# biod/sambamba

Measured on NVIDIA H100. Metric: bam_gb_per_s_depth_base, higher is better.
Workload: dtype u32

## Files before the change

include/bdepth.h:

```cpp
#ifndef BDEPTH_H
#define BDEPTH_H

#include <stddef.h>
#include <stdint.h>

#ifdef __cplusplus
extern "C" {
#endif

typedef struct bdepth bdepth_t;

typedef enum {
    BDEPTH_OK = 0,
    BDEPTH_ERR_IO = -1,
    BDEPTH_ERR_FORMAT = -2,
    BDEPTH_ERR_UNSORTED = -3,
    BDEPTH_ERR_NOINDEX = -4,
    BDEPTH_ERR_CUDA = -5,
    BDEPTH_ERR_NCCL = -6,
    BDEPTH_ERR_ARG = -7,
    BDEPTH_ERR_CALLBACK = -8
} bdepth_status;

typedef struct { uint32_t ref_id, start, end; } bdepth_region;

typedef struct {
    int32_t  ref_id;
    uint32_t start;
    uint32_t len;
    uint32_t stride;
    const uint32_t* counts;
    uint32_t n_samples;
    uint32_t sample_stride;
} bdepth_tile;
enum { BDEPTH_PLANE_A = 0, BDEPTH_PLANE_C, BDEPTH_PLANE_G, BDEPTH_PLANE_T, BDEPTH_PLANE_N, BDEPTH_PLANE_DEL, BDEPTH_PLANE_REFSKIP, BDEPTH_N_PLANES };

typedef int (*bdepth_tile_cb)(void* user, const bdepth_tile* tile);

typedef struct {
    int32_t  ref_id;
    uint32_t start, end;
    uint32_t n_reads;
    uint32_t n_bases;
    const uint32_t* cov_ge;
    int32_t  sample_id;
} bdepth_region_stat;
typedef int (*bdepth_stat_cb)(void* user, const bdepth_region_stat* stat, uint64_t index);

typedef struct {
    uint64_t file_bytes;
    uint64_t n_blocks;
    uint64_t cdata_bytes;
    uint64_t inflated_bytes;
    uint64_t n_records;
    uint64_t n_records_pass;
    uint64_t n_cigar_ops;
    uint64_t seq_bytes;
    uint64_t positions;
    uint64_t covered_positions;
    uint64_t long_reads;
    uint64_t chain_fixups;
    uint32_t gpu_launches;
    uint32_t n_batches;
    float ms_h2d, ms_inflate, ms_scan, ms_coverage, ms_reduce, ms_d2h, ms_total_device;
    double host_wall_ms;
    float ms_span_device;
    float ms_exchange;
    uint64_t own_lo, own_hi;
    uint64_t halo_bytes_sent;
    uint64_t mate_pairs;
    uint64_t mate_pair_columns;
    uint64_t mate_groups;
    float ms_mates;
} bdepth_stats;

int  bdepth_device_count(void);
int  bdepth_open(const char* bam_path, int device, bdepth_t** out);
int  bdepth_open_lazy(const char* bam_path, int device, bdepth_t** out);
int  bdepth_open_memory(const void* bam, size_t bam_len, const void* bai, size_t bai_len, int device, bdepth_t** out);
int  bdepth_add_input(bdepth_t* h, const char* bam_path);
void bdepth_close(bdepth_t* h);
const char* bdepth_last_error(const bdepth_t* h);

int         bdepth_n_ref(const bdepth_t* h);
const char* bdepth_ref_name(const bdepth_t* h, int i);
uint32_t    bdepth_ref_length(const bdepth_t* h, int i);
const char* bdepth_header_text(const bdepth_t* h, size_t* len);
int         bdepth_is_coordinate_sorted(const bdepth_t* h);
int         bdepth_has_index(const bdepth_t* h);
int         bdepth_n_samples(const bdepth_t* h);
const char* bdepth_sample_name(const bdepth_t* h, int i);

int bdepth_set_filter(bdepth_t* h, int mapq_gt, uint32_t flag_reject_mask);
int bdepth_set_filter_query(bdepth_t* h, const char* query);
int bdepth_set_min_baseq(bdepth_t* h, uint32_t min_base_quality);
int bdepth_set_fix_mates(bdepth_t* h, int on);
int bdepth_set_combined(bdepth_t* h, int combined);
int bdepth_set_regions(bdepth_t* h, const bdepth_region* regions, size_t n);
int bdepth_set_shard(bdepth_t* h, int rank, int world, const void* nccl_unique_id);
int bdepth_nccl_unique_id(void* out128);
int bdepth_plan_shards(const char* bam_path, int world, uint64_t* out_voffsets);
long bdepth_plan_region_chunks(const char* bam_path, const bdepth_region* regions, size_t n, uint64_t* out_pairs, size_t cap);
int bdepth_set_tuning(bdepth_t* h, uint64_t batch_inflated_bytes, uint64_t chunk_blocks);

int bdepth_stage(bdepth_t* h);
int bdepth_run_resident(bdepth_t* h);
int bdepth_run_base(bdepth_t* h, bdepth_tile_cb cb, void* user);
int bdepth_run_windows(bdepth_t* h, uint32_t window, uint32_t overlap, const uint32_t* thresholds, size_t n_thresholds, bdepth_stat_cb cb, void* user);
int bdepth_run_regions(bdepth_t* h, const bdepth_region* regions, size_t n, const uint32_t* thresholds, size_t n_thresholds, bdepth_stat_cb cb, void* user);

typedef struct { double min_cov, max_cov; int annotate; } bdepth_text_opts;
typedef int (*bdepth_text_cb)(void* user, const char* text, size_t len);
int bdepth_run_base_text(bdepth_t* h, const bdepth_text_opts* opts, bdepth_text_cb cb, void* user);

int bdepth_get_stats(const bdepth_t* h, bdepth_stats* out);
int bdepth_ref_has_reads(const bdepth_t* h, int ref);

int64_t bdepth_inflate_to_host(bdepth_t* h, void* dst, uint64_t cap);
int64_t bdepth_build_index(bdepth_t* h, void* dst, uint64_t cap);
typedef struct { uint64_t total[2], secondary[2], supplementary[2], duplicates[2], mapped[2], paired[2], read1[2], read2[2],
                 proper_pair[2], both_mapped[2], singletons[2], mate_diff_chr[2], mate_diff_chr_mapq5[2]; } bdepth_flagstat;
int bdepth_run_flagstat(bdepth_t* h, bdepth_flagstat* out);
enum { BDEPTH_VIEW_ALL = 0, BDEPTH_VIEW_BED = 1, BDEPTH_VIEW_POSITIONAL = 2 };
typedef struct {
    uint16_t flag_set, flag_unset;
    const char* query;
    int subsample;
    uint64_t subsample_threshold;
    uint64_t subsampling_seed;
    int regions_from;
    const bdepth_region* regions;
    size_t n_regions;
    uint32_t n_unmapped;
} bdepth_view_opts;
int bdepth_run_view_count(bdepth_t* h, const bdepth_view_opts* opts, uint64_t* count);
#define BDEPTH_VIEW_UNMAPPED 0xFFFFFFFFu
int bdepth_run_view_text(bdepth_t* h, const bdepth_view_opts* opts, bdepth_text_cb cb, void* user);
int64_t bdepth_scan_to_host(bdepth_t* h, uint64_t cap, int32_t* ref_id, int32_t* pos, uint32_t* span, uint16_t* flag, uint8_t* mapq, uint16_t* n_cigar, uint64_t* rec_off);

#ifdef __cplusplus
}
#endif
#endif
```

sambamba_b200/_lib.py:

```python
import ctypes as C
import os
import numpy as np

_HERE = os.path.dirname(os.path.abspath(__file__))


def lib_path():
    return os.path.join(_HERE, "_build", "libbdepth.so")


class BDepthError(RuntimeError):
    def __init__(self, code, msg):
        super().__init__(f"bdepth error {code}: {msg}")
        self.code = code
        self.msg = msg


class Region(C.Structure):
    _fields_ = [("ref_id", C.c_uint32), ("start", C.c_uint32), ("end", C.c_uint32)]


class Tile(C.Structure):
    _fields_ = [("ref_id", C.c_int32), ("start", C.c_uint32), ("len", C.c_uint32), ("stride", C.c_uint32),
                ("counts", C.POINTER(C.c_uint32)), ("n_samples", C.c_uint32), ("sample_stride", C.c_uint32)]


class RegionStat(C.Structure):
    _fields_ = [("ref_id", C.c_int32), ("start", C.c_uint32), ("end", C.c_uint32), ("n_reads", C.c_uint32),
                ("n_bases", C.c_uint32), ("cov_ge", C.POINTER(C.c_uint32)), ("sample_id", C.c_int32)]


class Stats(C.Structure):
    _fields_ = [(n, C.c_uint64) for n in ("file_bytes", "n_blocks", "cdata_bytes", "inflated_bytes", "n_records",
                                          "n_records_pass", "n_cigar_ops", "seq_bytes", "positions",
                                          "covered_positions", "long_reads", "chain_fixups")] + \
               [("gpu_launches", C.c_uint32), ("n_batches", C.c_uint32)] + \
               [(n, C.c_float) for n in ("ms_h2d", "ms_inflate", "ms_scan", "ms_coverage", "ms_reduce", "ms_d2h",
                                         "ms_total_device")] + [("host_wall_ms", C.c_double), ("ms_span_device", C.c_float), ("ms_exchange", C.c_float),
                                                                 ("own_lo", C.c_uint64), ("own_hi", C.c_uint64), ("halo_bytes_sent", C.c_uint64),
                                                                 ("mate_pairs", C.c_uint64), ("mate_pair_columns", C.c_uint64), ("mate_groups", C.c_uint64), ("ms_mates", C.c_float)]

    def as_dict(self):
        return {n: getattr(self, n) for n, _ in self._fields_}


FLAGSTAT_FIELDS = ("total", "secondary", "supplementary", "duplicates", "mapped", "paired", "read1", "read2", "proper_pair", "both_mapped",
                   "singletons", "mate_diff_chr", "mate_diff_chr_mapq5")


class FlagStat(C.Structure):
    _fields_ = [(n, C.c_uint64 * 2) for n in FLAGSTAT_FIELDS]

    def as_dict(self):
        return {n: (getattr(self, n)[0], getattr(self, n)[1]) for n in FLAGSTAT_FIELDS}


class ViewOpts(C.Structure):
    _fields_ = [("flag_set", C.c_uint16), ("flag_unset", C.c_uint16), ("query", C.c_char_p), ("subsample", C.c_int), ("subsample_threshold", C.c_uint64),
                ("subsampling_seed", C.c_uint64), ("regions_from", C.c_int), ("regions", C.POINTER(Region)), ("n_regions", C.c_size_t), ("n_unmapped", C.c_uint32)]


def subsample_threshold(frac):
    t = 4294967296.0 * frac
    if not t >= 0:
        raise ValueError("Conversion negative overflow")
    if t > 18446744073709551616.0:
        raise ValueError("Conversion positive overflow")
    return min(int(t), (1 << 64) - 1)


class TextOpts(C.Structure):
    _fields_ = [("min_cov", C.c_double), ("max_cov", C.c_double), ("annotate", C.c_int)]


TEXT_CB = C.CFUNCTYPE(C.c_int, C.c_void_p, C.c_void_p, C.c_size_t)
TILE_CB = C.CFUNCTYPE(C.c_int, C.c_void_p, C.POINTER(Tile))
STAT_CB = C.CFUNCTYPE(C.c_int, C.c_void_p, C.POINTER(RegionStat), C.c_uint64)

_lib = None


def load_library():
    global _lib
    if _lib is not None:
        return _lib
    p = lib_path()
    if not os.path.exists(p):
        raise ImportError(f"{p} is missing: build it with `python -c 'import __graft_entry__ as g; g.build()'` "
                          "(there is no CPU fallback)")
    L = C.CDLL(p)
    vp = C.c_void_p
    L.bdepth_device_count.restype = C.c_int
    L.bdepth_open.argtypes = [C.c_char_p, C.c_int, C.POINTER(vp)]
    L.bdepth_open_lazy.argtypes = [C.c_char_p, C.c_int, C.POINTER(vp)]
    L.bdepth_open_memory.argtypes = [vp, C.c_size_t, vp, C.c_size_t, C.c_int, C.POINTER(vp)]
    L.bdepth_add_input.argtypes = [vp, C.c_char_p]
    L.bdepth_close.argtypes = [vp]
    L.bdepth_close.restype = None
    L.bdepth_last_error.argtypes = [vp]
    L.bdepth_last_error.restype = C.c_char_p
    L.bdepth_n_ref.argtypes = [vp]
    L.bdepth_ref_name.argtypes = [vp, C.c_int]
    L.bdepth_ref_name.restype = C.c_char_p
    L.bdepth_ref_length.argtypes = [vp, C.c_int]
    L.bdepth_ref_length.restype = C.c_uint32
    L.bdepth_header_text.argtypes = [vp, C.POINTER(C.c_size_t)]
    L.bdepth_header_text.restype = C.c_char_p
    L.bdepth_is_coordinate_sorted.argtypes = [vp]
    L.bdepth_has_index.argtypes = [vp]
    L.bdepth_n_samples.argtypes = [vp]
    L.bdepth_sample_name.argtypes = [vp, C.c_int]
    L.bdepth_sample_name.restype = C.c_char_p
    L.bdepth_set_filter.argtypes = [vp, C.c_int, C.c_uint32]
    L.bdepth_set_filter_query.argtypes = [vp, C.c_char_p]
    L.bdepth_set_min_baseq.argtypes = [vp, C.c_uint32]
    L.bdepth_set_fix_mates.argtypes = [vp, C.c_int]
    L.bdepth_set_combined.argtypes = [vp, C.c_int]
    L.bdepth_set_regions.argtypes = [vp, C.POINTER(Region), C.c_size_t]
    L.bdepth_set_shard.argtypes = [vp, C.c_int, C.c_int, vp]
    L.bdepth_nccl_unique_id.argtypes = [vp]
    L.bdepth_set_tuning.argtypes = [vp, C.c_uint64, C.c_uint64]
    L.bdepth_stage.argtypes = [vp]
    L.bdepth_run_resident.argtypes = [vp]
    L.bdepth_plan_shards.argtypes = [C.c_char_p, C.c_int, C.POINTER(C.c_uint64)]
    L.bdepth_plan_region_chunks.argtypes = [C.c_char_p, C.POINTER(Region), C.c_size_t, C.POINTER(C.c_uint64), C.c_size_t]
    L.bdepth_plan_region_chunks.restype = C.c_long
    L.bdepth_run_base.argtypes = [vp, TILE_CB, vp]
    L.bdepth_run_base_text.argtypes = [vp, C.POINTER(TextOpts), TEXT_CB, vp]
    L.bdepth_run_windows.argtypes = [vp, C.c_uint32, C.c_uint32, C.POINTER(C.c_uint32), C.c_size_t, STAT_CB, vp]
    L.bdepth_run_regions.argtypes = [vp, C.POINTER(Region), C.c_size_t, C.POINTER(C.c_uint32), C.c_size_t, STAT_CB, vp]
    L.bdepth_get_stats.argtypes = [vp, C.POINTER(Stats)]
    L.bdepth_ref_has_reads.argtypes = [vp, C.c_int]
    L.bdepth_inflate_to_host.argtypes = [vp, vp, C.c_uint64]
    L.bdepth_inflate_to_host.restype = C.c_int64
    L.bdepth_scan_to_host.argtypes = [vp, C.c_uint64] + [vp] * 7
    L.bdepth_scan_to_host.restype = C.c_int64
    L.bdepth_build_index.argtypes = [vp, vp, C.c_uint64]
    L.bdepth_build_index.restype = C.c_int64
    L.bdepth_run_flagstat.argtypes = [vp, C.POINTER(FlagStat)]
    L.bdepth_run_view_count.argtypes = [vp, C.POINTER(ViewOpts), C.POINTER(C.c_uint64)]
    L.bdepth_run_view_text.argtypes = [vp, C.POINTER(ViewOpts), TEXT_CB, vp]
    _lib = L
    return L


EXPORTED_SYMBOLS = [
    "bdepth_device_count", "bdepth_open", "bdepth_open_lazy", "bdepth_open_memory", "bdepth_add_input", "bdepth_close", "bdepth_last_error", "bdepth_n_ref",
    "bdepth_ref_name", "bdepth_ref_length", "bdepth_header_text", "bdepth_is_coordinate_sorted", "bdepth_has_index",
    "bdepth_n_samples", "bdepth_sample_name", "bdepth_set_filter", "bdepth_set_filter_query", "bdepth_set_min_baseq", "bdepth_set_fix_mates", "bdepth_set_combined", "bdepth_set_regions",
    "bdepth_set_shard", "bdepth_nccl_unique_id", "bdepth_plan_shards", "bdepth_plan_region_chunks", "bdepth_set_tuning", "bdepth_stage", "bdepth_run_resident", "bdepth_run_base", "bdepth_run_base_text",
    "bdepth_run_windows", "bdepth_run_regions", "bdepth_get_stats", "bdepth_ref_has_reads", "bdepth_inflate_to_host", "bdepth_scan_to_host", "bdepth_build_index",
    "bdepth_run_flagstat", "bdepth_run_view_count", "bdepth_run_view_text",
]


def nccl_unique_id():
    L = load_library()
    buf = (C.c_char * 128)()
    rc = L.bdepth_nccl_unique_id(buf)
    if rc:
        raise BDepthError(rc, L.bdepth_last_error(None).decode())
    return bytes(buf)


def plan_shards(path, world):
    L = load_library()
    out = (C.c_uint64 * max(1, world - 1))()
    rc = L.bdepth_plan_shards(os.fsencode(path), world, out)
    if rc:
        raise BDepthError(rc, L.bdepth_last_error(None).decode())
    return list(out)[:world - 1]


def plan_region_chunks(path, regions):
    L = load_library()
    arr = (Region * max(1, len(regions)))(*[Region(*r) for r in regions])
    n = L.bdepth_plan_region_chunks(os.fsencode(path), arr, len(regions), None, 0)
    if n < 0:
        raise BDepthError(n, L.bdepth_last_error(None).decode())
    out = (C.c_uint64 * max(1, 2 * n))()
    L.bdepth_plan_region_chunks(os.fsencode(path), arr, len(regions), out, n)
    return [(out[2 * i], out[2 * i + 1]) for i in range(n)]


class BDepth:

    def __init__(self, path=None, device=0, memory=None, bai=None, lazy=False):
        self.L = load_library()
        self.h = C.c_void_p()
        if memory is not None:
            self._keep = (memory, bai)
            mp = memory.ctypes.data_as(C.c_void_p)
            bp = bai.ctypes.data_as(C.c_void_p) if bai is not None else None
# ... 245 lines not shown
```

sambamba_b200/csrc/bdepth.cu:

```cuda
#include "launch.cuh"
#include <dlfcn.h>
#include <fcntl.h>
#include <stdarg.h>
#include <stdio.h>
#include <stdlib.h>
#include <sys/mman.h>
#include <sys/stat.h>
#include <unistd.h>
#include <algorithm>
#include <chrono>
#include <map>
#include <string>
#include <vector>

#include "../../include/bdepth.h"
#include "host_bam.hpp"
#include "kernels.cuh"
#include "mates.cuh"
#include "host_filter.hpp"

using namespace bdk;

namespace {

thread_local std::string g_open_error;

struct DevBuf {
    void* p = nullptr; size_t cap = 0;
    cudaError_t ensure(size_t n) {
        if (n <= cap) return cudaSuccess;
        if (p) { cudaFree(p); p = nullptr; cap = 0; }
        size_t want = n + n / 8 + 256;
        cudaError_t e = cudaMalloc(&p, want);
        if (e == cudaSuccess) cap = want;
        return e;
    }
    void release() { if (p) cudaFree(p); p = nullptr; cap = 0; }
    template <class T> T* as() const { return (T*)p; }
};

struct HostScratch {
    uint8_t* hp = nullptr; uint8_t* dp = nullptr; size_t cap = 0, used = 0;
    cudaError_t ensure(size_t n) {
        if (n <= cap) return cudaSuccess;
        if (hp) { cudaDeviceSynchronize(); cudaFreeHost(hp); hp = nullptr; dp = nullptr; cap = 0; }
        cudaError_t e = cudaHostAlloc((void**)&hp, n + n / 4, cudaHostAllocMapped);
        if (e != cudaSuccess) return e;
        e = cudaHostGetDevicePointer((void**)&dp, hp, 0);
        if (e == cudaSuccess) cap = n + n / 4;
        used = 0;
        return e;
    }
    uint8_t* take(size_t n) { size_t a = (used + 15) & ~size_t(15); if (a + n > cap) return nullptr; used = a + n; return hp + a; }
    uint8_t* dev(const void* host) const { return dp + ((const uint8_t*)host - hp); }
    void release() { if (hp) cudaFreeHost(hp); hp = nullptr; dp = nullptr; cap = used = 0; }
};
__global__ void k_copy_words(uint32_t* __restrict__ dst, const uint32_t* __restrict__ src, size_t n) {
    for (size_t i = (size_t)blockIdx.x * blockDim.x + threadIdx.x; i < n; i += (size_t)gridDim.x * blockDim.x) dst[i] = src[i];
}

#ifdef BDEPTH_EMULATE_SHIM
constexpr unsigned COUNT_GRID = 4;
#else
constexpr unsigned COUNT_GRID = 2048;
#endif
constexpr size_t CARRY_MAX = 64ull << 20;
constexpr size_t EMIT_CHUNK = 4ull << 20;
constexpr uint32_t SHARD_EXTRA_BLOCKS = 8;
constexpr uint32_t MATE_ZONE_BLOCKS = 64;

enum RunMode { RUN_FULL = 0, RUN_INFLATE_ONLY = 1, RUN_SCAN_ONLY = 2, RUN_INDEX = 3, RUN_FLAGSTAT = 4, RUN_VIEW_COUNT = 5, RUN_VIEW_TEXT = 6 };
constexpr int RC_RETRY_WINDOW = 1;

struct NcclUid { char b[128]; };
typedef void* NcclComm;
struct NcclApi {
    bool ok = false; std::string err;
    int (*GetUniqueId)(NcclUid*) = nullptr;
    int (*CommInitRank)(NcclComm*, int, NcclUid, int) = nullptr;
    int (*CommDestroy)(NcclComm) = nullptr;
    int (*AllGather)(const void*, void*, size_t, int, NcclComm, cudaStream_t) = nullptr;
    int (*AllReduce)(const void*, void*, size_t, int, int, NcclComm, cudaStream_t) = nullptr;
    int (*Send)(const void*, size_t, int, int, NcclComm, cudaStream_t) = nullptr;
    int (*Recv)(void*, size_t, int, int, NcclComm, cudaStream_t) = nullptr;
    int (*GroupStart)() = nullptr;
    int (*GroupEnd)() = nullptr;
    const char* (*GetErrorString)(int) = nullptr;
};
constexpr int NCCL_UINT32 = 3, NCCL_UINT64 = 5, NCCL_SUM = 0;
NcclApi& nccl() {
    static NcclApi api; static bool tried = false;
    if (tried) return api;
    tried = true;
#ifdef BDEPTH_EMULATE_SHIM
    api.GetUniqueId = [](NcclUid* u) { return emu_ncclGetUniqueId(u->b); };
    api.CommInitRank = [](NcclComm* c, int w, NcclUid u, int r) { return emu_ncclCommInitRank(c, w, u.b, r); };
    api.CommDestroy = emu_ncclCommDestroy; api.AllGather = emu_ncclAllGather; api.AllReduce = emu_ncclAllReduce; api.Send = emu_ncclSend; api.Recv = emu_ncclRecv;
    api.GroupStart = emu_ncclGroupStart; api.GroupEnd = emu_ncclGroupEnd; api.GetErrorString = emu_ncclGetErrorString; api.ok = true;
    return api;
#endif
    void* lib = dlopen("libnccl.so.2", RTLD_NOW | RTLD_GLOBAL);
    if (!lib) lib = dlopen("libnccl.so", RTLD_NOW | RTLD_GLOBAL);
    if (!lib) { api.err = std::string("cannot load libnccl.so.2: ") + dlerror(); return api; }
    bool all = true;
    auto sym = [&](const char* n) { void* p = dlsym(lib, n); if (!p) { all = false; api.err = std::string("missing NCCL symbol ") + n; } return p; };
    api.GetUniqueId = (int (*)(NcclUid*))sym("ncclGetUniqueId");
    api.CommInitRank = (int (*)(NcclComm*, int, NcclUid, int))sym("ncclCommInitRank");
    api.CommDestroy = (int (*)(NcclComm))sym("ncclCommDestroy");
    api.AllGather = (int (*)(const void*, void*, size_t, int, NcclComm, cudaStream_t))sym("ncclAllGather");
    api.AllReduce = (int (*)(const void*, void*, size_t, int, int, NcclComm, cudaStream_t))sym("ncclAllReduce");
    api.Send = (int (*)(const void*, size_t, int, int, NcclComm, cudaStream_t))sym("ncclSend");
    api.Recv = (int (*)(void*, size_t, int, int, NcclComm, cudaStream_t))sym("ncclRecv");
    api.GroupStart = (int (*)())sym("ncclGroupStart");
    api.GroupEnd = (int (*)())sym("ncclGroupEnd");
    api.GetErrorString = (const char* (*)(int))sym("ncclGetErrorString");
    api.ok = all;
    return api;
}

}

struct bdepth {
    const uint8_t* file = nullptr; size_t file_len = 0; bool mapped = false; int fd = -1;
    std::vector<HostBlock> blocks; uint64_t total_u = 0;
    bool lazy = false, framed_all = true; size_t framed_off = 0;
    BamHeader hdr; BaiIndex bai; bool has_index = false;
    int device = 0; int n_sm = 0;
    int mapq_gt = 0; uint32_t flag_reject = 0x600; uint32_t minq = 0;
    std::vector<bdepth_region> regions;
    int rank = 0, world = 1;
    NcclComm comm = nullptr; bool have_uid = false; NcclUid uid{};
    uint64_t own_lo = 0, own_hi = 0;
    bool bai_window_ok = true;
    bool combined = false;
    bool fix_mates = false;
    bool k1lz_v12 = false;
    bool k1lz_flat = false;
    int k1h_variant = -1;
    bool k1_onephase = false;
    bool k3_pre = false;
    bool k3_tile = true;
    bool has_fprog = false; FilterProg fprog; DevBuf fprog_d;
    DevBuf m_hash, m_flag, m_flt, m_ctl;
    uint32_t S = 1;
    DevBuf rg_ids, rg_offs, rg_samp;
    DevBuf text[2], text_tiles, text_offs, text_zero, text_samp, present;
    int coll_pending = 0;
    bool want_presence = false;
    uint64_t batch_u = 6ull << 30;
    uint64_t chunk_blocks = 13 * 32 * 16;
    bool shard_ready = false;
    size_t blk_lo = 0, blk_hi = 0; int64_t entry0 = 0; uint64_t limit_abs_u = 0;
    uint64_t zone_lin_lo = UINT64_MAX;
    uint64_t own_lo_abs_u = 0;
    bool sparse_ok = true;
    bool sparse_on = false;
    std::vector<HostBlock> vblocks; std::vector<int32_t> seg_entry ; std::vector<uint32_t> seg_limit ;
    DevBuf anchors_idx, anchors_val, chunk_limit;
    cudaStream_t s_main = nullptr, s_copy = nullptr, s_d2h = nullptr;
    cudaEvent_t ev[32] = {};
    DevBuf comp2[2];
    cudaStream_t s_k1[16] = {};
    std::vector<cudaEvent_t> chunk_ev[2], k1_ev;
    std::vector<size_t> chunk_end[2];
    bool staged = false; uint64_t staged_file_off = 0;
    DevBuf tok, lits, aux, segi, littab;
    DevBuf comp, descs, status, ubuf, chunk_start, entry, exitb, count, slot_base, slots, rec_base, walk_list;
    DevBuf soa_start, soa_span, soa_meta, soa_off, soa_ncl, soa_lseq, long_list, tile_first, tile_lo, counts, ref_len_d, ref_lin0_d, scan_stats, ref_has, ref_has_all, flt_d, lead_list, misc;
    uint64_t cnt_base = 0, win_len = 0;
    void* pinned = nullptr; size_t pinned_cap = 0;
    HostScratch hs;
    std::vector<uint32_t> ref_has_host;
    struct SegSet { bool on = false; uint32_t n = 0; bool has_min = false, has_u = false; uint64_t ext_max = 0; DevBuf s, e, pmax, id, reads, minstart, bases_reads, mbases, ustart, da, dac, db, dthr, dbases, dcov, dscr; } seg;
    struct IndexSet { DevBuf lin, lin_len, lin_base, lin_cap, n_mapped, n_unmapped, carry, ctl, runs, excs; std::vector<uint32_t> base, cap; std::vector<IndexRun> h_runs; std::vector<IndexExc> h_excs; uint64_t n_lin = 0; } ix;
    std::vector<uint8_t> built_bai;
    DevBuf fs; uint64_t fs_host[FS_WORDS + 1] = {};
    ViewSel vsel{}; DevBuf vc, vc_reg, vc_prog; uint64_t vc_host[2] = {};
    struct ViewText {
        bdepth_text_cb cb = nullptr; void* user = nullptr;
        DevBuf names, len, off, tiles, ctl, cut_r, cut_o, slot[2];
        char* host = nullptr; size_t cap = 0;
        bool pend[2] = {false, false}; size_t pend_len[2] = {0, 0}; int next = 0;
        uint64_t issued = 0;
        float ms_fmt = 0, ms_d2h = 0;
        SamTab tab{};
    } vt;
    std::vector<bdepth*> extra;
    bool accum = false;
    bool force_window = false;
    bdepth_stats st{}; std::string err;
};

namespace {

int fail(bdepth* h, int code, const char* fmt, ...) {
    char buf[1024]; va_list ap; va_start(ap, fmt); vsnprintf(buf, sizeof buf, fmt, ap); va_end(ap);
    if (h) h->err = buf; else g_open_error = buf;
    return code;
}
#define NK(call) do { int r__ = (call); if (r__ != 0) return fail(h, BDEPTH_ERR_NCCL, "NCCL error at %s:%d: %s", __FILE__, __LINE__, nccl().GetErrorString ? nccl().GetErrorString(r__) : "?"); } while (0)
#define CK(call) do { cudaError_t e__ = (call); if (e__ != cudaSuccess) return fail(h, BDEPTH_ERR_CUDA, "CUDA error %s at %s:%d: %s", cudaGetErrorName(e__), __FILE__, __LINE__, cudaGetErrorString(e__)); } while (0)

int ensure_pinned(bdepth* h, size_t n) {
    if (n <= h->pinned_cap) return 0;
    if (h->pinned) cudaFreeHost(h->pinned);
    h->hs.release();
    h->pinned = nullptr; h->pinned_cap = 0;
    CK(cudaMallocHost(&h->pinned, n));
    h->pinned_cap = n;
    return 0;
}

int init_device(bdepth* h) {
    int n = 0; cudaError_t e = cudaGetDeviceCount(&n);
    if (e != cudaSuccess || n <= 0) return fail(h, BDEPTH_ERR_CUDA, "no CUDA device available (%s); libbdepth has no CPU fallback", cudaGetErrorString(e));
    if (h->device < 0 || h->device >= n) return fail(h, BDEPTH_ERR_ARG, "device %d out of range (%d devices)", h->device, n);
    CK(cudaSetDevice(h->device));
    CK(cudaDeviceGetAttribute(&h->n_sm, cudaDevAttrMultiProcessorCount, h->device));
    if (!h->s_main) { CK(cudaStreamCreateWithFlags(&h->s_main, cudaStreamNonBlocking)); CK(cudaStreamCreateWithFlags(&h->s_copy, cudaStreamNonBlocking)); CK(cudaStreamCreateWithFlags(&h->s_d2h, cudaStreamNonBlocking)); for (auto& ks : h->s_k1) CK(cudaStreamCreateWithFlags(&ks, cudaStreamNonBlocking)); for (auto& e2 : h->ev) CK(cudaEventCreate(&e2)); }
    CK(cudaFuncSetAttribute(k1_inflate, cudaFuncAttributeMaxDynamicSharedMemorySize, K1_SMEM));
    CK(cudaFuncSetAttribute(k1_fallback, cudaFuncAttributeMaxDynamicSharedMemorySize, K1_SMEM));
    CK(cudaFuncSetAttribute(k1_huff<false, 4>, cudaFuncAttributePreferredSharedMemoryCarveout, cudaSharedmemCarveoutMaxShared)); CK(cudaFuncSetAttribute(k1_huff<false, 6>, cudaFuncAttributePreferredSharedMemoryCarveout, cudaSharedmemCarveoutMaxShared));
    CK(cudaFuncSetAttribute(k1_huff<true, 5>, cudaFuncAttributePreferredSharedMemoryCarveout, cudaSharedmemCarveoutMaxShared)); CK(cudaFuncSetAttribute(k1_huff<true, 4>, cudaFuncAttributePreferredSharedMemoryCarveout, cudaSharedmemCarveoutMaxShared));
    { const char* e = getenv("BDEPTH_K1H_VARIANT"); h->k1h_variant = e ? atoi(e) : -1; }
    { const char* e = getenv("BDEPTH_K3"); h->k3_tile = !(e && !strcmp(e, "gather")); }
    CK(cudaFuncSetAttribute(k3_tile<false>, cudaFuncAttributeMaxDynamicSharedMemorySize, (int)K3T_SMEM)); CK(cudaFuncSetAttribute(k3_tile<true>, cudaFuncAttributeMaxDynamicSharedMemorySize, (int)K3T_SMEM));
    { const char* e = getenv("BDEPTH_K1LZ"); h->k1lz_flat = e && !strcmp(e, "flat"); h->k1lz_v12 = e && !strcmp(e, "v12"); }
    { const char* e = getenv("BDEPTH_K1_ONEPHASE"); h->k1_onephase = e && atoi(e) == 1; }
    { const char* e = getenv("BDEPTH_K3_PREFETCH"); h->k3_pre = !e || atoi(e) != 0; }
    return 0;
}

int inflate_blocks_to_host(bdepth* h, size_t b0, size_t b1, std::vector<uint8_t>& out) {
    size_t nb = b1 - b0; if (!nb) { out.clear(); return 0; }
    uint64_t f0 = h->blocks[b0].coff & ~3ull, f1 = h->blocks[b1 - 1].coff + h->blocks[b1 - 1].bsize;
    uint64_t ulen = h->blocks[b1 - 1].uoff + h->blocks[b1 - 1].isize - h->blocks[b0].uoff;
    CK(h->comp.ensure(f1 - f0 + 256)); CK(h->descs.ensure(nb * sizeof(BlockDesc))); CK(h->status.ensure(nb * sizeof(int))); CK(h->ubuf.ensure(CARRY_MAX + ulen + 256));
    std::vector<BlockDesc> d(nb);
    for (size_t i = 0; i < nb; i++) { const HostBlock& b = h->blocks[b0 + i]; d[i] = BlockDesc{b.coff + b.cdata_off - f0, b.uoff - h->blocks[b0].uoff, b.csize, b.isize}; }
    CK(cudaMemcpyAsync(h->comp.p, h->file + f0, f1 - f0, cudaMemcpyHostToDevice, h->s_main));
    CK(cudaMemsetAsync((uint8_t*)h->comp.p + (f1 - f0), 0, 128, h->s_main));
    CK(cudaMemcpyAsync(h->descs.p, d.data(), nb * sizeof(BlockDesc), cudaMemcpyHostToDevice, h->s_main));
    BD_LAUNCH((unsigned)((nb + 32 * K1_WARPS - 1) / (32 * K1_WARPS)), 32 * K1_WARPS, K1_SMEM, h->s_main, k1_inflate)(h->comp.as<uint32_t>(), h->descs.as<BlockDesc>(), (uint32_t)nb, h->ubuf.as<uint8_t>() + CARRY_MAX, h->status.as<int>());
    CK(cudaGetLastError());
    std::vector<int> stt(nb); out.resize(ulen);
    CK(cudaMemcpyAsync(stt.data(), h->status.p, nb * sizeof(int), cudaMemcpyDeviceToHost, h->s_main));
    CK(cudaMemcpyAsync(out.data(), h->ubuf.as<uint8_t>() + CARRY_MAX, ulen, cudaMemcpyDeviceToHost, h->s_main));
    CK(cudaStreamSynchronize(h->s_main));
    h->st.gpu_launches += 1;
    for (size_t i = 0; i < nb; i++) if (stt[i]) return fail(h, BDEPTH_ERR_FORMAT, "DEFLATE error %d in BGZF block at offset %llu", stt[i], (unsigned long long)h->blocks[b0 + i].coff);
    return 0;
}

int frame_more(bdepth* h, size_t more) {
    if (h->framed_all) return 0;
    bool eof = false;
    std::string e = frame_bgzf(h->file, h->file_len, &h->framed_off, &h->total_u, more, UINT64_MAX, h->blocks, &eof);
    if (!e.empty()) return fail(h, BDEPTH_ERR_FORMAT, "%s", e.c_str());
    if (eof) h->framed_all = true;
    return 0;
}
int ensure_all_blocks(bdepth* h) { return frame_more(h, SIZE_MAX); }

int finish_open(bdepth* h) {
    h->blocks.clear(); h->total_u = 0; h->framed_off = 0; h->framed_all = false;
    { int rcf = frame_more(h, h->lazy ? 4 : SIZE_MAX); if (rcf) return rcf; }
    if (h->blocks.empty()) return fail(h, BDEPTH_ERR_FORMAT, "Invalid file format: expected BAM\\1");
    int rc = init_device(h); if (rc) return rc;
    size_t nb = std::min<size_t>(4, h->blocks.size());
    for (;;) {
        std::vector<uint8_t> u; rc = inflate_blocks_to_host(h, 0, nb, u); if (rc) return rc;
        std::string perr; int pr = parse_bam_header(u.data(), u.size(), h->hdr, perr);
        if (pr == 0) break;
        if (pr < 0) return fail(h, BDEPTH_ERR_FORMAT, "%s", perr.c_str());
        if (nb == h->blocks.size() && !h->framed_all) { rc = frame_more(h, nb * 3); if (rc) return rc; }
        if (nb == h->blocks.size()) return fail(h, BDEPTH_ERR_FORMAT, "truncated BAM header");
        nb = std::min(h->blocks.size(), nb * 4);
    }
    size_t nref = h->hdr.ref_len.size();
    CK(h->ref_len_d.ensure((nref + 1) * 4)); CK(h->ref_lin0_d.ensure((nref + 1) * 8));
    if (nref) { CK(cudaMemcpy(h->ref_len_d.p, h->hdr.ref_len.data(), nref * 4, cudaMemcpyHostToDevice)); CK(cudaMemcpy(h->ref_lin0_d.p, h->hdr.ref_lin0.data(), nref * 8, cudaMemcpyHostToDevice)); }
    return 0;
}

std::vector<uint64_t> shard_candidates(const BaiIndex& bai) {
    std::vector<uint64_t> vos;
    for (auto& v : bai.ioffsets) for (uint64_t x : v) if (x) vos.push_back(x);
    std::sort(vos.begin(), vos.end()); vos.erase(std::unique(vos.begin(), vos.end()), vos.end());
    return vos;
}
uint64_t shard_cut_voffset(const std::vector<uint64_t>& vos, uint64_t file_len, int k, int world) {
    uint64_t target = (uint64_t)((__uint128_t)file_len * (unsigned)k / (unsigned)world);
    auto it = std::lower_bound(vos.begin(), vos.end(), target << 16);
    return it == vos.end() ? UINT64_MAX : *it;
}

int prepare_shard(bdepth* h) {
    if (h->shard_ready) return 0;
    { int rcf = ensure_all_blocks(h); if (rcf) return rcf; }
    const auto& B = h->blocks;
    auto block_of_u = [&](uint64_t u) { size_t lo = 0, hi = B.size(); while (lo + 1 < hi) { size_t m = (lo + hi) / 2; if (B[m].uoff <= u) lo = m; else hi = m; } return lo; };
    auto block_of_c = [&](uint64_t c) { size_t lo = 0, hi = B.size(); while (lo + 1 < hi) { size_t m = (lo + hi) / 2; if (B[m].coff <= c) lo = m; else hi = m; } return lo; };
    uint64_t start_u = h->hdr.first_rec_off, end_u = h->total_u;
    if (h->world > 1) {
        if (!h->bai.valid) return fail(h, BDEPTH_ERR_NOINDEX, "sharding needs the BAI linear index");
        std::vector<uint64_t> vos = shard_candidates(h->bai);
        auto cut = [&](int k) -> uint64_t {
            if (k <= 0) return h->hdr.first_rec_off;
            if (k >= h->world) return h->total_u;
            uint64_t vo = shard_cut_voffset(vos, h->file_len, k, h->world);
            if (vo == UINT64_MAX) return h->total_u;
            size_t b = block_of_c(vo >> 16);
            if (B[b].coff != (vo >> 16)) return h->total_u;
            uint64_t u = B[b].uoff + (vo & 0xFFFF);
            return u < h->hdr.first_rec_off ? h->hdr.first_rec_off : u;
        };
        start_u = cut(h->rank); end_u = cut(h->rank + 1);
        if (end_u < start_u) end_u = start_u;
    }
    if (start_u >= h->total_u) { h->blk_lo = h->blk_hi = B.size(); h->entry0 = 0; h->limit_abs_u = h->total_u; h->shard_ready = true; return 0; }
    h->blk_lo = block_of_u(start_u); h->entry0 = (int64_t)(start_u - B[h->blk_lo].uoff);
    h->limit_abs_u = end_u; h->own_lo_abs_u = start_u;
    if (end_u >= h->total_u) h->blk_hi = B.size();
    else h->blk_hi = std::min(B.size(), block_of_u(end_u) + 1 + (h->fix_mates ? MATE_ZONE_BLOCKS : SHARD_EXTRA_BLOCKS));
    h->zone_lin_lo = UINT64_MAX;
    if (h->world > 1 && h->rank > 0) {
        std::vector<uint8_t> u; int rc = inflate_blocks_to_host(h, h->blk_lo, std::min(B.size(), h->blk_lo + 2), u); if (rc) return rc;
        const uint64_t o = (uint64_t)h->entry0;
        if (o + 12 <= u.size()) {
            int32_t ref = (int32_t)h_rd32(u.data() + o + 4), pos = (int32_t)h_rd32(u.data() + o + 8);
            if (ref >= 0 && (size_t)ref < h->bai.ioffsets.size() && pos >= 0) {
                const auto& lin = h->bai.ioffsets[ref]; size_t w = (size_t)pos >> 14;
                uint64_t vo = w < lin.size() ? lin[w] : 0;
                if (vo) {
                    size_t b = block_of_c(vo >> 16);
                    if (B[b].coff != (vo >> 16)) return fail(h, BDEPTH_ERR_FORMAT, "fix-mate-overlaps on several ranks: the linear index does not match the file");
                    uint64_t zu = B[b].uoff + (vo & 0xFFFF);
                    if (zu < h->hdr.first_rec_off) zu = h->hdr.first_rec_off;
                    if (zu < start_u) { h->blk_lo = block_of_u(zu); h->entry0 = (int64_t)(zu - B[h->blk_lo].uoff); }
                    h->zone_lin_lo = h->hdr.ref_lin0[ref] + ((uint64_t)w << 14);
                }
            }
        }
    }
    h->shard_ready = true;
    return 0;
}

struct Emitter {
    bdepth* h; bdepth_tile_cb cb; void* user;
    struct Range { uint64_t a, b; };
    std::vector<Range> ranges; size_t ri = 0; uint64_t pos = 0; bool started = false;
    uint64_t lo_clip = 0, hi_clip = UINT64_MAX;
    struct Slot { uint64_t a = 0, b = 0; } slot[2];
    int head = 0, inflight = 0;
    uint64_t d2h_bytes = 0;
    size_t chunk() const { return EMIT_CHUNK / h->S; }
    int issue(int si, uint64_t a, uint64_t b) {
        const int NP = N_PLANES * (int)h->S; const size_t CH = chunk();
        uint32_t* dst = (uint32_t*)h->pinned + (size_t)si * EMIT_CHUNK * N_PLANES;
        uint64_t wa = std::max(a, h->cnt_base), wb = std::min(b, h->cnt_base + h->win_len);
        if (wa >= wb || wa > a || wb < b) for (int pl = 0; pl < NP; pl++) memset(dst + (size_t)pl * CH, 0, (b - a) * 4);
        if (wa < wb) for (int pl = 0; pl < NP; pl++) CK(cudaMemcpyAsync(dst + (size_t)pl * CH + (wa - a), h->counts.as<uint32_t>() + (uint64_t)pl * h->win_len + (wa - h->cnt_base), (wb - wa) * 4, cudaMemcpyDeviceToHost, h->s_d2h));
        CK(cudaEventRecord(h->ev[8 + si], h->s_d2h));
        slot[si].a = a; slot[si].b = b; d2h_bytes += (b - a) * NP * 4;
        return 0;
    }
    int deliver_oldest() {
        int si = (head + 2 - inflight) & 1;
        CK(cudaEventSynchronize(h->ev[8 + si]));
        inflight--;
        if (!cb) return 0;
        const uint32_t* src = (const uint32_t*)h->pinned + (size_t)si * EMIT_CHUNK * N_PLANES;
        uint64_t a = slot[si].a, bnd = slot[si].b; const size_t nref = h->hdr.ref_len.size();
        size_t ref = std::upper_bound(h->hdr.ref_lin0.begin(), h->hdr.ref_lin0.end(), a) - h->hdr.ref_lin0.begin() - 1;
        while (a < bnd && ref < nref) {
            uint64_t rend = h->hdr.ref_lin0[ref] + h->hdr.ref_len[ref];
            if (a >= rend) { ref++; continue; }
            uint64_t e = std::min(bnd, rend);
// ... 191 lines not shown
    uint32_t i = blockIdx.x * blockDim.x + threadIdx.x; if (i < n) dst[idx[i]] = val[i];
}

struct RunOut {
    uint8_t* inflate_dst = nullptr; uint64_t inflate_cap = 0; uint64_t inflate_len = 0;
    uint64_t scan_cap = 0; uint64_t scan_n = 0;
    int32_t* ref_id = nullptr; int32_t* pos = nullptr; uint32_t* span = nullptr; uint16_t* flag = nullptr; uint8_t* mapq = nullptr; uint16_t* n_cigar = nullptr; uint64_t* rec_off = nullptr;
};

__global__ void k_fill_u32(uint32_t* p, uint32_t v, uint64_t n) { uint64_t i = (uint64_t)blockIdx.x * blockDim.x + threadIdx.x; if (i < n) p[i] = v; }

constexpr uint64_t VIEW_TEXT_PIECE = 64ull << 20;
const char* sam_err_msg(unsigned long long c) {
    switch (c) {
        case SAM_ERR_REF: return "a record's reference ID lies outside [-1, n_ref): no RNAME to print (the reference indexes its reference list out of bounds)";
        case SAM_ERR_MATE_REF: return "a record's mate reference ID lies outside [-1, n_ref): no RNEXT to print (the reference indexes its reference list out of bounds)";
        case SAM_ERR_TAG_TYPE: return "unknown tag type in a record's auxiliary data (UnknownTagTypeException)";
        case SAM_ERR_B_TYPE: return "unknown element type of a B array in a record's auxiliary data (UnknownTagTypeException)";
        case SAM_ERR_NO_NUL: return "a Z or H tag value without its terminating NUL";
        default: return "a record's fields, a tag or a B array run past the record's block_size";
    }
}
int view_text_deliver(bdepth* h, int slot) {
    auto& V = h->vt;
    if (!V.pend[slot]) return 0;
    CK(cudaEventSynchronize(h->ev[26 + slot])); V.pend[slot] = false;
    float t = 0; CK(cudaEventElapsedTime(&t, h->ev[28 + slot], h->ev[24 + slot])); V.ms_fmt += t;
    CK(cudaEventElapsedTime(&t, h->ev[24 + slot], h->ev[26 + slot])); V.ms_d2h += t;
    if (V.cb && V.pend_len[slot] && V.cb(V.user, V.host + (size_t)slot * V.cap, V.pend_len[slot])) return fail(h, BDEPTH_ERR_CALLBACK, "text callback aborted");
    return 0;
}
int view_text_flush(bdepth* h) { int rc = view_text_deliver(h, h->vt.next); if (!rc) rc = view_text_deliver(h, h->vt.next ^ 1); return rc; }
int view_text_sub(bdepth* h, const RecordSoA& soa, const uint8_t* u0, uint32_t R, int64_t own_from) {
    auto& V = h->vt; cudaStream_t sm = h->s_main;
    const uint32_t n_tiles = (R + SAM_SCAN_TILE - 1) / SAM_SCAN_TILE;
    const size_t toff_at = ((size_t)n_tiles * 4 + 7) / 8 * 8;
    CK(V.len.ensure((size_t)R * 4)); CK(V.off.ensure((size_t)R * 8)); CK(V.tiles.ensure(toff_at + (size_t)n_tiles * 8)); CK(V.ctl.ensure(32));
    uint32_t* len = V.len.as<uint32_t>(); unsigned long long* off = V.off.as<unsigned long long>();
    uint32_t* tsum = V.tiles.as<uint32_t>(); unsigned long long* toff = (unsigned long long*)(V.tiles.as<uint8_t>() + toff_at);
    SamTab t = V.tab; t.ctl = V.ctl.as<unsigned long long>();
    CK(cudaMemsetAsync(t.ctl, 0, 24, sm));
    CK(cudaEventRecord(h->ev[30], sm));
    BD_LAUNCH((unsigned)std::min<uint64_t>((R + 7) / 8, 8192), 256, 0, sm, k_sam_len)(soa, u0, R, own_from, h->vsel, t, len);
    BD_LAUNCH(n_tiles, 256, 0, sm, k_sam_tile_sum)(len, R, tsum);
    BD_LAUNCH(1, 1024, 0, sm, k_text_scan)(tsum, n_tiles, toff, t.ctl);
    BD_LAUNCH(n_tiles, 256, 0, sm, k_sam_scan_apply)(len, R, toff, off);
    CK(cudaGetLastError()); h->st.gpu_launches += 4;
    CK(cudaEventRecord(h->ev[31], sm));
    unsigned long long c[3]; CK(cudaMemcpyAsync(c, t.ctl, 24, cudaMemcpyDeviceToHost, sm)); CK(cudaStreamSynchronize(sm));
    { float tm = 0; CK(cudaEventElapsedTime(&tm, h->ev[30], h->ev[31])); V.ms_fmt += tm; }
    if (c[2]) return fail(h, BDEPTH_ERR_FORMAT, "%s", sam_err_msg(c[2]));
    const uint64_t total = c[0];
    if (!total) return 0;
    const uint64_t piece = std::max<uint64_t>(1, std::min<uint64_t>(VIEW_TEXT_PIECE, h->batch_u));
    if (piece + c[1] > V.cap) {
        int rc = view_text_flush(h); if (rc) return rc;
        if (V.host) { cudaFreeHost(V.host); V.host = nullptr; }
        V.cap = 0;
        const size_t need = piece + std::max<uint64_t>(c[1], piece);
        CK(cudaMallocHost((void**)&V.host, 2 * need)); CK(V.slot[0].ensure(need)); CK(V.slot[1].ensure(need));
        V.cap = need;
    }
    const uint32_t n_cuts = (uint32_t)((total + piece - 1) / piece) + 1;
    CK(V.cut_r.ensure((size_t)n_cuts * 4)); CK(V.cut_o.ensure((size_t)n_cuts * 8));
    BD_LAUNCH((n_cuts + 255) / 256, 256, 0, sm, k_sam_cut)(off, R, total, piece, n_cuts, V.cut_r.as<uint32_t>(), V.cut_o.as<unsigned long long>());
    CK(cudaGetLastError()); h->st.gpu_launches++;
    std::vector<uint32_t> cr(n_cuts); std::vector<unsigned long long> co(n_cuts);
    CK(cudaMemcpyAsync(cr.data(), V.cut_r.p, (size_t)n_cuts * 4, cudaMemcpyDeviceToHost, sm)); CK(cudaMemcpyAsync(co.data(), V.cut_o.p, (size_t)n_cuts * 8, cudaMemcpyDeviceToHost, sm));
    CK(cudaStreamSynchronize(sm));
    for (uint32_t j = 0; j + 1 < n_cuts; j++) {
        const uint32_t r0 = cr[j], r1 = j + 2 == n_cuts ? R : cr[j + 1];
        const uint64_t bytes = (j + 2 == n_cuts ? total : co[j + 1]) - co[j];
        if (!bytes) continue;
        const int s = V.next;
        int rc = view_text_deliver(h, s); if (rc) return rc;
        CK(cudaEventRecord(h->ev[28 + s], sm));
        BD_LAUNCH((unsigned)std::min<uint64_t>((r1 - r0 + 7) / 8, 8192), 256, 0, sm, k_sam_write)(soa.off, u0, r0, r1, len, off, t, V.slot[s].as<char>());
        CK(cudaGetLastError()); h->st.gpu_launches++;
        CK(cudaEventRecord(h->ev[24 + s], sm));
        CK(cudaStreamWaitEvent(h->s_d2h, h->ev[24 + s], 0));
        CK(cudaMemcpyAsync(V.host + (size_t)s * V.cap, V.slot[s].p, bytes, cudaMemcpyDeviceToHost, h->s_d2h));
        CK(cudaEventRecord(h->ev[26 + s], h->s_d2h));
        V.pend[s] = true; V.pend_len[s] = bytes; V.issued += bytes; V.next = s ^ 1;
        rc = view_text_deliver(h, s ^ 1); if (rc) return rc;
    }
    return 0;
}

int run_pipeline_body(bdepth* h, RunMode mode, RunOut* ro, Emitter* em);
int run_pipeline(bdepth* h, RunMode mode, RunOut* ro, Emitter* em = nullptr) {
    const int rc = run_pipeline_body(h, mode, ro, em);
    if (rc && rc != RC_RETRY_WINDOW) abort_collectives(h);
    return rc;
}
int run_pipeline_body(bdepth* h, RunMode mode, RunOut* ro, Emitter* em) {
    h->coll_pending = 0;
    int rc = init_device(h); if (rc) return rc;
    auto t_host0 = std::chrono::steady_clock::now();
    bdepth_stats& st = h->st; uint32_t launches0 = 0;
    st = bdepth_stats{}; st.gpu_launches = launches0;
    const bool view = mode == RUN_VIEW_COUNT || mode == RUN_VIEW_TEXT;
    if (mode == RUN_VIEW_TEXT) { h->vt.issued = 0; h->vt.ms_fmt = h->vt.ms_d2h = 0; }
    const bool sparse = (mode == RUN_FULL || view) && plan_sparse(h);
    h->coll_pending = (mode == RUN_FULL && h->world > 1 && h->comm) ? (sparse ? 2 : 1) : (mode == RUN_FLAGSTAT && h->world > 1 && h->comm) ? 3 : (view && h->world > 1 && h->comm) ? (sparse ? 2 : 4) : 0;
    if (!sparse) { rc = prepare_shard(h); if (rc) return rc; }
    const bool fix = mode == RUN_FULL && h->fix_mates;
    bool flt_uploaded = false;
    if (fix && h->world > 1 && !h->comm) return fail(h, BDEPTH_ERR_ARG, "fix-mate-overlaps on several ranks needs the boundary exchange (bdepth_set_shard with a NCCL id)");
    const uint64_t eff_batch_u = h->batch_u;
    size_t ghost_b = 0; int64_t ghost_entry = 0; uint64_t ghost_below_abs = 0, prev_s_last = 0, covered_from = 0;
    const std::vector<HostBlock>& B = sparse ? h->vblocks : h->blocks;
    const size_t blk_lo = sparse ? 0 : h->blk_lo, blk_hi = sparse ? B.size() : h->blk_hi;
    const size_t nref = h->hdr.ref_len.size();
    cudaStream_t sm = h->s_main;

    if (mode == RUN_FULL && h->accum) {
    } else if (mode == RUN_FULL) {
        uint64_t lo = 0, hi = h->hdr.total_len;
        if (h->force_window) { lo = h->cnt_base; hi = h->cnt_base + h->win_len; }
        else
        if (h->bai.valid && h->bai_window_ok && h->bai.ioffsets.size() == nref && h->world > 1 && !sparse && !fix && blk_hi > blk_lo) {
            const uint64_t vo_end = blk_hi < B.size() ? (B[blk_hi].coff << 16) : (h->file_len << 16);
            lo = h->rank == 0 ? UINT64_MAX : h->zone_lin_lo; hi = 0;
            for (size_t r = 0; r < nref; r++) {
                const auto& v = h->bai.ioffsets[r];
                for (size_t k = 0; k < v.size(); k++) if (v[k] && v[k] < vo_end) {
                    const uint64_t a = h->hdr.ref_lin0[r] + std::min<uint64_t>((uint64_t)k << 14, h->hdr.ref_len[r]), e = h->hdr.ref_lin0[r] + std::min<uint64_t>((uint64_t)(k + 1) << 14, h->hdr.ref_len[r]);
                    if (h->rank == 0) lo = std::min(lo, a);
                    if (e > hi) hi = e;
                }
            }
            if (lo == UINT64_MAX || lo >= hi) { lo = 0; hi = h->hdr.total_len; }
        } else if (h->bai.valid && h->bai_window_ok && h->bai.ioffsets.size() == nref && h->world == 1) {
            lo = UINT64_MAX; hi = 0;
            for (size_t r = 0; r < nref; r++) {
                const auto& v = h->bai.ioffsets[r]; if (v.empty()) continue;
                size_t k = 0; while (k < v.size() && v[k] == 0) k++;
                if (k == v.size()) continue;
                lo = std::min<uint64_t>(lo, h->hdr.ref_lin0[r] + std::min<uint64_t>((uint64_t)k << 14, h->hdr.ref_len[r]));
                hi = std::max<uint64_t>(hi, h->hdr.ref_lin0[r] + std::min<uint64_t>((uint64_t)v.size() << 14, h->hdr.ref_len[r]));
            }
            if (lo >= hi) { lo = 0; hi = h->hdr.total_len; }
        }
        if (!h->force_window) {
            h->cnt_base = lo / TILE_POS * TILE_POS;
            h->win_len = ((hi - h->cnt_base + TILE_POS - 1) / TILE_POS + 1) * TILE_POS;
        }
        h->S = (h->combined || h->hdr.sample_names.size() <= 1) ? 1u : (uint32_t)h->hdr.sample_names.size();
        if (h->S > 64) return fail(h, BDEPTH_ERR_ARG, "%u samples: per-sample output supports at most 64 (use --combined)", h->S);
        size_t need = (size_t)h->win_len * N_PLANES * 4 * h->S;
        size_t free_b = 0, tot_b = 0; CK(cudaMemGetInfo(&free_b, &tot_b));
        if (need > h->counts.cap && need > free_b + h->counts.cap) return fail(h, BDEPTH_ERR_CUDA, "counter window needs %zu bytes of HBM, %zu free", need, free_b);
        CK(h->counts.ensure(need));
        CK(cudaMemsetAsync(h->counts.p, 0, need, sm));
        if (h->want_presence) { CK(h->present.ensure((h->win_len / 32 + 2) * 4)); CK(cudaMemsetAsync(h->present.p, 0, (h->win_len / 32 + 2) * 4, sm)); }
        CK(h->ref_has.ensure((nref / 32 + 2) * 4)); CK(cudaMemsetAsync(h->ref_has.p, 0, (nref / 32 + 2) * 4, sm));
    }
    CK(h->scan_stats.ensure(sizeof(ScanStats)));
    const FilterProg* d_fprog = nullptr;
    if (h->has_fprog && mode != RUN_FLAGSTAT && !view) { CK(h->fprog_d.ensure(sizeof(FilterProg))); CK(cudaMemcpyAsync(h->fprog_d.p, &h->fprog, sizeof(FilterProg), cudaMemcpyHostToDevice, sm)); CK(cudaStreamSynchronize(sm)); d_fprog = h->fprog_d.as<FilterProg>(); }
    RgTable rgt{nullptr, nullptr, nullptr, 0};
    if (mode == RUN_FULL && (h->S > 1 || (fix && h->hdr.sample_names.size() > 1))) {
        std::vector<uint8_t> ids; std::vector<uint32_t> offs; std::vector<uint8_t> samp;
        for (size_t g = 0; g < h->hdr.rg_ids.size(); g++) { offs.push_back((uint32_t)ids.size()); ids.insert(ids.end(), h->hdr.rg_ids[g].begin(), h->hdr.rg_ids[g].end()); ids.push_back(0); samp.push_back((uint8_t)h->hdr.rg_sample[g]); }
        CK(h->rg_ids.ensure(ids.size() + 8)); CK(h->rg_offs.ensure(offs.size() * 4 + 8)); CK(h->rg_samp.ensure(samp.size() + 8));
        CK(cudaMemcpyAsync(h->rg_ids.p, ids.data(), ids.size(), cudaMemcpyHostToDevice, sm)); CK(cudaMemcpyAsync(h->rg_offs.p, offs.data(), offs.size() * 4, cudaMemcpyHostToDevice, sm)); CK(cudaMemcpyAsync(h->rg_samp.p, samp.data(), samp.size(), cudaMemcpyHostToDevice, sm));
        CK(cudaStreamSynchronize(sm));
        rgt = RgTable{h->rg_ids.as<uint8_t>(), h->rg_offs.as<uint32_t>(), h->rg_samp.as<uint8_t>(), (uint32_t)offs.size()};
    }
    { uint64_t shard_u = blk_hi > blk_lo ? B[blk_hi - 1].uoff + B[blk_hi - 1].isize - B[blk_lo].uoff : 0; CK(h->ubuf.ensure(CARRY_MAX + std::min<uint64_t>(eff_batch_u + 65536, shard_u) + 256)); }
    CK(h->misc.ensure(64));
    HostScratch& hs = h->hs;
    auto up = [&](void* dst_dev, const void* src, size_t bytes) -> int {
        if (!bytes) return 0;
        uint8_t* m = hs.take(bytes); if (!m) return fail(h, BDEPTH_ERR_CUDA, "internal: host scratch exhausted");
        memcpy(m, src, bytes);
        BD_LAUNCH((unsigned)std::min<size_t>((bytes / 4 + 255) / 256, 512), 256, 0, sm, k_copy_words)((uint32_t*)dst_dev, (const uint32_t*)hs.dev(m), bytes / 4);
        st.gpu_launches++;
        return 0;
    };
    auto down = [&](const void* src_dev, size_t bytes) -> uint8_t* {
        uint8_t* m = hs.take(bytes ? bytes : 4); if (!m) return nullptr;
        if (bytes) { BD_LAUNCH((unsigned)std::min<size_t>((bytes / 4 + 255) / 256, 512), 256, 0, sm, k_copy_words)((uint32_t*)hs.dev(m), (const uint32_t*)src_dev, bytes / 4); st.gpu_launches++; }
        return m;
    };
#define UP(dst, src, bytes) do { int rcu_ = up((dst), (src), (bytes)); if (rcu_) return rcu_; } while (0)
#define DOWN(var, type, src, bytes) type* var = (type*)down((src), (bytes)); if (!var) return fail(h, BDEPTH_ERR_CUDA, "internal: host scratch exhausted")

    float ms_h2d = 0, ms_k1 = 0, ms_k2 = 0, ms_k3 = 0;
    uint64_t carry_len = 0; bool first_batch = true;
    bool sparse_bad = false;
    uint64_t shard_min = UINT64_MAX, shard_max = 0;
    if (mode == RUN_INDEX) {
        auto& X = h->ix; X.base.assign(nref + 1, 0); X.cap.assign(nref + 1, 0); uint64_t acc = 0;
        for (size_t r = 0; r < nref; r++) { X.base[r] = (uint32_t)acc; X.cap[r] = (uint32_t)std::min<uint64_t>(32769, ((uint64_t)h->hdr.ref_len[r] >> 14) + 2); acc += X.cap[r]; if (acc > 0xFFFFFFF0ull) return fail(h, BDEPTH_ERR_ARG, "too many references for the linear index tables"); }
        X.n_lin = acc; X.h_runs.clear(); X.h_excs.clear();
        CK(X.lin.ensure((acc + 1) * 8)); CK(X.lin_len.ensure((nref + 1) * 4)); CK(X.lin_base.ensure((nref + 1) * 4)); CK(X.lin_cap.ensure((nref + 1) * 4));
        CK(X.n_mapped.ensure((nref + 1) * 8)); CK(X.n_unmapped.ensure((nref + 1) * 8)); CK(X.carry.ensure(sizeof(IndexCarry))); CK(X.ctl.ensure(sizeof(IndexCtl)));
        CK(cudaMemsetAsync(X.lin.p, 0xFF, (acc + 1) * 8, sm)); CK(cudaMemsetAsync(X.lin_len.p, 0, (nref + 1) * 4, sm)); CK(cudaMemsetAsync(X.n_mapped.p, 0, (nref + 1) * 8, sm)); CK(cudaMemsetAsync(X.n_unmapped.p, 0, (nref + 1) * 8, sm));
        CK(cudaMemsetAsync(X.carry.p, 0, sizeof(IndexCarry), sm));
        CK(cudaMemcpyAsync(X.lin_base.p, X.base.data(), (nref + 1) * 4, cudaMemcpyHostToDevice, sm)); CK(cudaMemcpyAsync(X.lin_cap.p, X.cap.data(), (nref + 1) * 4, cudaMemcpyHostToDevice, sm));
        IndexCtl c0{0, 0, 0, ~0ull, ~0ull, 0, ~0ull, 0};
        CK(cudaMemcpyAsync(X.ctl.p, &c0, sizeof c0, cudaMemcpyHostToDevice, sm)); CK(cudaStreamSynchronize(sm));
    }
    float ms_census = 0;
    if (mode == RUN_FLAGSTAT) { CK(h->fs.ensure((FS_WORDS + 1) * 8)); CK(cudaMemsetAsync(h->fs.p, 0, (FS_WORDS + 1) * 8, sm)); }
    if (view) { CK(h->vc.ensure(16)); CK(cudaMemsetAsync(h->vc.p, 0, 16, sm)); }
    CK(cudaEventRecord(h->ev[10], sm));
    size_t b = blk_lo;
    if (ro) { ro->inflate_len = 0; ro->scan_n = 0; }
    if (!h->staged) {
        uint64_t mx = 0;
        for (size_t bb = blk_lo; bb < blk_hi;) {
            size_t e = bb; uint64_t u = 0, cb = 0; while (e < blk_hi && (e == bb || u + B[e].isize <= eff_batch_u)) { u += B[e].isize; cb += B[e].bsize; e++; }
            mx = std::max<uint64_t>(mx, sparse ? cb + 8 : B[e - 1].coff + B[e - 1].bsize - (B[bb].coff & ~3ull)); bb = e;
        }
        CK(h->comp2[0].ensure(mx + 256)); CK(h->comp2[1].ensure(mx + 256));
    }
    size_t batch_no = 0;
    auto batch_end = [&](size_t bb) { size_t e = bb; uint64_t u = 0; while (e < blk_hi && (e == bb || u + B[e].isize <= eff_batch_u)) { u += B[e].isize; e++; } return e; };
    const size_t H2D_CHUNK_BLOCKS = h->chunk_blocks;
    std::vector<uint64_t> dco[2];
    auto issue_h2d = [&](size_t no, size_t bb, size_t be) -> int {
        int slot = (int)(no & 1);
        uint64_t g0 = B[bb].coff & ~3ull;
        if (no >= 2) CK(cudaStreamWaitEvent(h->s_copy, h->ev[16 + slot], 0));
        CK(cudaEventRecord(h->ev[18 + slot], h->s_copy));
        h->chunk_end[slot].clear();
        dco[slot].resize(be - bb);
        { uint64_t acc = 0; for (size_t i = bb; i < be; i++) { dco[slot][i - bb] = sparse ? acc : B[i].coff - g0; acc += B[i].bsize; } }
        size_t nch = 0;
        for (size_t c0 = bb; c0 < be; c0 += H2D_CHUNK_BLOCKS, nch++) {
            size_t c1 = std::min(be, c0 + H2D_CHUNK_BLOCKS);
            uint64_t dev_end;
            if (!sparse) {
                uint64_t a = c0 == bb ? g0 : B[c0].coff, e = B[c1 - 1].coff + B[c1 - 1].bsize;
                CK(cudaMemcpyAsync((uint8_t*)h->comp2[slot].p + (a - g0), h->file + a, e - a, cudaMemcpyHostToDevice, h->s_copy));
                dev_end = e - g0;
            } else {
                for (size_t r0 = c0; r0 < c1;) {
                    size_t r1 = r0 + 1; while (r1 < c1 && B[r1].coff == B[r1 - 1].coff + B[r1 - 1].bsize) r1++;
                    CK(cudaMemcpyAsync((uint8_t*)h->comp2[slot].p + dco[slot][r0 - bb], h->file + B[r0].coff, B[r1 - 1].coff + B[r1 - 1].bsize - B[r0].coff, cudaMemcpyHostToDevice, h->s_copy));
                    r0 = r1;
                }
                dev_end = dco[slot][c1 - 1 - bb] + B[c1 - 1].bsize;
            }
            if (c1 == be) CK(cudaMemsetAsync((uint8_t*)h->comp2[slot].p + dev_end, 0, 128, h->s_copy));
            if (h->chunk_ev[slot].size() <= nch) { cudaEvent_t ne; CK(cudaEventCreateWithFlags(&ne, cudaEventDisableTiming)); h->chunk_ev[slot].push_back(ne); }
            CK(cudaEventRecord(h->chunk_ev[slot][nch], h->s_copy));
            h->chunk_end[slot].push_back(c1);
        }
        CK(cudaEventRecord(h->ev[14 + slot], h->s_copy));
        return 0;
    };
    while (b < blk_hi) {
        size_t b1 = b; uint64_t ub_new = 0;
        while (b1 < blk_hi && (b1 == b || ub_new + B[b1].isize <= eff_batch_u)) { ub_new += B[b1].isize; b1++; }
        const bool last_batch = b1 == blk_hi;
        st.n_batches++; st.n_blocks += b1 - b; st.inflated_bytes += ub_new;
        const size_t new_b = b;
        const size_t stream_b = (fix && batch_no > 0) ? std::min(ghost_b, b) : b;
        {
        const size_t b = stream_b;
        const size_t nb = b1 - b;
        const uint64_t batch_u0 = B[b].uoff;
        const uint64_t ub = B[b1 - 1].uoff + B[b1 - 1].isize - batch_u0;
        const uint32_t* d_comp;
        cudaEvent_t e0 = h->ev[0], e1 = h->ev[1], e2 = h->ev[2], e3 = h->ev[3], e4 = h->ev[4];
        CK(cudaEventRecord(e0, sm));
        if (h->staged) d_comp = h->comp.as<uint32_t>();
        else {
            if (fix) {
                uint64_t need = 8; if (sparse) for (size_t i = b; i < b1; i++) need += B[i].bsize; else need = B[b1 - 1].coff + B[b1 - 1].bsize - (B[b].coff & ~3ull);
                CK(h->comp2[batch_no & 1].ensure(need + 256));
                int rcp = issue_h2d(batch_no, b, b1); if (rcp) return rcp;
            } else if (batch_no == 0) { int rcp = issue_h2d(0, b, b1); if (rcp) return rcp; }
            d_comp = h->comp2[batch_no & 1].as<uint32_t>();
        }
        std::vector<BlockDesc> d(nb); uint64_t csum = 0, tok_words = 0;
        for (size_t i = 0; i < nb; i++) {
            const HostBlock& hb = B[b + i];
            uint64_t dev_off = h->staged ? hb.coff - h->staged_file_off : dco[batch_no & 1][i];
            d[i] = BlockDesc{dev_off + hb.cdata_off, hb.uoff - batch_u0, hb.csize, hb.isize, tok_words};
            tok_words += tok_cap_of(hb.isize);
            if (b + i >= new_b) { csum += hb.csize; st.file_bytes += hb.bsize; }
        }
        st.cdata_bytes += csum;
        CK(h->descs.ensure(nb * sizeof(BlockDesc))); CK(h->status.ensure(nb * sizeof(int))); CK(h->ubuf.ensure(CARRY_MAX + ub + 256));
        if (!h->k1_onephase) { CK(h->tok.ensure(tok_words * 4 + 64)); CK(h->lits.ensure(ub + 16 * nb + 64)); CK(h->aux.ensure(nb * sizeof(BlockAux))); CK(h->segi.ensure(nb * MAX_SEG * 4)); CK(h->littab.ensure(nb * (size_t)MAX_SEG * 256)); }
        CK(hs.ensure(nb * (sizeof(BlockDesc) + 192) + 16384)); hs.used = 0;
        UP(h->descs.p, d.data(), nb * sizeof(BlockDesc));
        uint8_t* u0 = h->ubuf.as<uint8_t>() + CARRY_MAX;
        CK(cudaEventRecord(e1, sm));
        struct Sub { size_t s0, s1; int ev_lo, ev_hi; };
        std::vector<Sub> subs;
        auto launch_k1 = [&](cudaStream_t ks, size_t c0, uint32_t n) -> int {
            const BlockDesc* dd = h->descs.as<BlockDesc>() + (c0 - b); int* stp = h->status.as<int>() + (c0 - b);
            if (h->k1_onephase) {
                BD_LAUNCH((n + 32 * K1_WARPS - 1) / (32 * K1_WARPS), 32 * K1_WARPS, K1_SMEM, ks, k1_inflate)(d_comp, dd, n, u0, stp);
                CK(cudaGetLastError()); st.gpu_launches++;
                return 0;
            }
            BlockAux* ax = h->aux.as<BlockAux>() + (c0 - b); uint32_t* sgi = h->segi.as<uint32_t>() + (c0 - b) * MAX_SEG; uint8_t* ltb = h->littab.as<uint8_t>() + (c0 - b) * (size_t)MAX_SEG * 256;
            const unsigned hg = (n + 32 * K1H_WARPS - 1) / (32 * K1H_WARPS); const uint32_t blk0 = (uint32_t)(c0 - b);
#define K1H(LIMS, MINB) BD_LAUNCH(hg, 32 * K1H_WARPS, k1h_smem<LIMS>(), ks, k1_huff<LIMS, MINB>)(d_comp, dd, n, blk0, stp, h->tok.as<uint32_t>(), h->lits.as<uint8_t>(), ax, sgi, ltb)
            const int variant = h->k1h_variant >= 0 ? h->k1h_variant : (n > (uint32_t)h->n_sm * 16u * 32u ? 2 : 0);
            switch (variant) { case 1: K1H(false, 6); break; case 2: K1H(true, 5); break; case 3: K1H(true, 4); break; default: K1H(false, 4); }
// ... 84 lines not shown
        int walk_err = *werr;
        for (size_t i = 0; i < nb; i++) if (stt[i]) return fail(h, BDEPTH_ERR_FORMAT, "DEFLATE error %d in BGZF block at offset %llu", stt[i], (unsigned long long)B[b + i].coff);
        int64_t cur = anchor; int64_t tail = (int64_t)ub;
        for (size_t i = 0; i < nb; i++) {
            if (sparse && i && h->seg_entry[b + i] >= 0) cur = cstart[i] + h->seg_entry[b + i];
            int64_t true_e = (cur < cstart[i + 1]) ? cur : ENTRY_NONE;
            if (true_e != ENTRY_NONE && true_e < cstart[i]) return fail(h, BDEPTH_ERR_FORMAT, "internal: record chain went backwards");
            if (ent[i] != true_e) {
                st.chain_fixups++;
                uint32_t ci = (uint32_t)i;
                UP((int64_t*)h->entry.p + i, &true_e, 8);
                UP(h->walk_list.p, &ci, 4);
                BD_LAUNCH(1, 32, 0, sm, k2_walk)(spw, h->chunk_start.as<int64_t>(), (uint32_t)nb, h->entry.as<int64_t>(), h->slot_base.as<uint32_t>(), h->slots.as<uint16_t>(), h->count.as<uint32_t>(), h->exitb.as<int64_t>(), (int*)h->misc.p, h->walk_list.as<uint32_t>(), 1, d_limit);
                CK(cudaGetLastError()); st.gpu_launches++;
                DOWN(fx_ext, int64_t, (int64_t*)h->exitb.p + i, 8); DOWN(fx_cnt, uint32_t, (uint32_t*)h->count.p + i, 4); DOWN(fx_err, int, h->misc.p, 4);
                CK(cudaStreamSynchronize(sm));
                ext[i] = *fx_ext; cnt[i] = *fx_cnt; walk_err = *fx_err;
                ent[i] = true_e;
            }
            if (true_e != ENTRY_NONE) {
                cur = ext[i];
                if (sparse && h->seg_limit[b + i] != UINT32_MAX) {
                    if (ext[i] != (i ? cstart[i] : 0) + (int64_t)h->seg_limit[b + i]) {
                        if (h->world == 1) { if (mode == RUN_VIEW_TEXT && h->vt.issued) return fail(h, BDEPTH_ERR_FORMAT, "the index does not describe this file (a region chunk does not end at a record), found after SAM lines were delivered"); h->sparse_ok = false; CK(cudaDeviceSynchronize()); return run_pipeline(h, mode, ro, em); }
                        sparse_bad = true; break;
                    }
                    cur = INT64_MAX / 2;
                    continue;
                }
                if (ext[i] < cstart[i + 1]) {
                    for (size_t j = i + 1; j < nb; j++) cnt[j] = 0;
                    break;
                }
            }
        }
        if (sparse_bad) break;
        if (walk_err) return fail(h, BDEPTH_ERR_FORMAT, "corrupt BAM record chain (block_size < 32)");
        tail = cur < (int64_t)ub ? cur : (int64_t)ub;
        std::vector<uint32_t> rbase(nb + 1); uint64_t R = 0;
        bool limited = u_limit < (int64_t)ub && !fix;
        std::vector<uint16_t> tmp_slots;
        for (size_t i = 0; i < nb; i++) {
            if (limited && cnt[i]) {
                if (cstart[i] >= u_limit) cnt[i] = 0;
                else if (cstart[i + 1] > u_limit) {
                    tmp_slots.resize(cnt[i]);
                    CK(cudaMemcpy(tmp_slots.data(), (uint16_t*)h->slots.p + sbase[i], cnt[i] * 2, cudaMemcpyDeviceToHost));
                    uint32_t k = 0; while (k < cnt[i] && ((k == 0 || cstart[i] > 0) ? cstart[i] : 0) + tmp_slots[k] < u_limit) k++;
                    cnt[i] = k;
                }
            }
            rbase[i] = (uint32_t)R; R += cnt[i];
        }
        rbase[nb] = (uint32_t)R;
        if (R > 0xFFFFFFF0ull) return fail(h, BDEPTH_ERR_ARG, "batch too large");
        UP(h->count.p, cnt, nb * 4);
        if (limited && last_batch && tail < u_limit && tail < (int64_t)ub && b1 < B.size()) return fail(h, BDEPTH_ERR_FORMAT, "record at the shard boundary spans more than %u BGZF blocks", SHARD_EXTRA_BLOCKS);
        UP(h->rec_base.p, rbase.data(), (nb + 1) * 4);
        st.n_records += R;
        size_t Rc = R ? R : 1;
        CK(h->soa_start.ensure(Rc * 8)); CK(h->soa_span.ensure(Rc * 4)); CK(h->soa_meta.ensure(Rc * 4)); CK(h->soa_off.ensure(Rc * 8)); CK(h->soa_ncl.ensure(Rc * 4)); CK(h->soa_lseq.ensure(Rc * 4)); CK(h->long_list.ensure(Rc * 4));
        RecordSoA soa{h->soa_start.as<uint64_t>(), h->soa_span.as<uint32_t>(), h->soa_meta.as<uint32_t>(), h->soa_off.as<int64_t>(), h->soa_ncl.as<uint32_t>(), h->soa_lseq.as<int32_t>()};
        ScanStats zs{0, 0, 0, 0, ~0ull, 0, 0, ~0ull, 0, 0, ~0ull, 0, ~0ull, ~0ull, 0};
        const int64_t ghost_below = (fix && batch_no > 0) ? (int64_t)ghost_below_abs - (int64_t)batch_u0 : INT64_MIN;
        const int64_t own_lo = (fix && h->world > 1) ? (int64_t)h->own_lo_abs_u - (int64_t)batch_u0 : INT64_MIN;
        const int64_t own_hi = (fix && h->world > 1 && h->limit_abs_u < h->total_u) ? (int64_t)h->limit_abs_u - (int64_t)batch_u0 : INT64_MAX;
        const int64_t zone_below = (!fix && !sparse && h->world > 1) ? (int64_t)h->own_lo_abs_u - (int64_t)batch_u0 : INT64_MIN;
        UP(h->scan_stats.p, &zs, sizeof zs);
        if ((mode == RUN_SCAN_ONLY || mode == RUN_INDEX || mode == RUN_FLAGSTAT || view) && !h->ref_has.p) { CK(h->ref_has.ensure((nref / 32 + 2) * 4)); CK(cudaMemsetAsync(h->ref_has.p, 0, (nref / 32 + 2) * 4, sm)); }
        uint32_t* has_dst = h->ref_has.as<uint32_t>();
        const uint32_t n_flt_k2 = mode == RUN_FULL ? (uint32_t)h->regions.size() : 0u;
        if (n_flt_k2) {
            if (!flt_uploaded) {
                std::vector<uint64_t> fl; fl.reserve(2 * (size_t)n_flt_k2);
                for (auto& g : h->regions) fl.push_back(h->hdr.ref_lin0[g.ref_id] + g.start);
                for (auto& g : h->regions) fl.push_back(h->hdr.ref_lin0[g.ref_id] + g.end);
                CK(h->flt_d.ensure(fl.size() * 8)); CK(cudaMemcpyAsync(h->flt_d.p, fl.data(), fl.size() * 8, cudaMemcpyHostToDevice, sm)); CK(cudaStreamSynchronize(sm));
                CK(h->ref_has_all.ensure((nref / 32 + 2) * 4)); CK(cudaMemsetAsync(h->ref_has_all.p, 0, (nref / 32 + 2) * 4, sm));
                flt_uploaded = true;
            }
            has_dst = h->ref_has_all.as<uint32_t>();
        }
#define K2_DECODE(F, G) BD_LAUNCH((unsigned)((nb * 32 + 255) / 256), 256, 0, sm, k2_decode<F, G>)(sp, h->chunk_start.as<int64_t>(), (uint32_t)nb, h->slot_base.as<uint32_t>(), h->slots.as<uint16_t>(), h->count.as<uint32_t>(), h->rec_base.as<uint32_t>(), soa, h->mapq_gt, h->flag_reject, h->scan_stats.as<ScanStats>(), h->long_list.as<uint32_t>(), has_dst, rgt, d_fprog, ghost_below, own_lo, own_hi, zone_below)
        if (fix) { if (d_fprog) K2_DECODE(true, true); else K2_DECODE(false, true); }
        else if (d_fprog) K2_DECODE(true, false);
        else K2_DECODE(false, false);
#undef K2_DECODE
        CK(cudaGetLastError()); st.gpu_launches++;
        if (R && mode != RUN_INDEX && mode != RUN_SCAN_ONLY && mode != RUN_FLAGSTAT && !view) {
            const bool lead_n_regions = h->seg.on && h->seg.n && !h->seg.has_u && !h->seg.has_min && !fix && h->world == 1;
            LeadNSegs lsg{nullptr, nullptr, nullptr, nullptr, 0u, nullptr, nullptr, 1u, h->minq};
            if (lead_n_regions) lsg = LeadNSegs{h->seg.s.as<uint64_t>(), h->seg.e.as<uint64_t>(), h->seg.pmax.as<uint64_t>(), h->seg.id.as<uint32_t>(), h->seg.n, h->seg.reads.as<uint32_t>(), h->seg.mbases.as<uint32_t>(),
                                                (uint32_t)((h->combined || h->hdr.sample_names.size() <= 1) ? 1 : h->hdr.sample_names.size()), h->minq};
            CK(h->lead_list.ensure(Rc * 4));
            BD_LAUNCH((unsigned)((R + 255) / 256), 256, 0, sm, k2_lead_n_find)(soa, u0, (uint32_t)R, h->lead_list.as<uint32_t>(), h->scan_stats.as<ScanStats>());
            BD_LAUNCH(32, 128, 0, sm, k2_lead_n_fix)(soa, u0, h->lead_list.as<uint32_t>(), h->scan_stats.as<ScanStats>(), (h->seg.on && !lead_n_regions) ? 1 : 0,
                                                    n_flt_k2 ? h->flt_d.as<uint64_t>() : nullptr, n_flt_k2 ? h->flt_d.as<uint64_t>() + n_flt_k2 : nullptr, n_flt_k2, lsg);
            CK(cudaGetLastError()); st.gpu_launches += 2;
        }
        if (n_flt_k2 && R) {
            BD_LAUNCH((unsigned)((R + 255) / 256), 256, 0, sm, k_ref_seen)(soa, (uint32_t)R, h->flt_d.as<uint64_t>(), h->flt_d.as<uint64_t>() + n_flt_k2, n_flt_k2, h->ref_lin0_d.as<uint64_t>(), (uint32_t)nref, h->ref_has.as<uint32_t>());
            CK(cudaGetLastError()); st.gpu_launches++;
        }
        DOWN(ssp, ScanStats, h->scan_stats.p, sizeof(ScanStats));
        CK(cudaEventRecord(e3, sm));
        CK(cudaStreamSynchronize(sm));
        const ScanStats ss = *ssp;
        st.n_records -= ss.n_ghost + ss.n_ghost_right;
        if (ss.bad_rec != ~0ull) return fail(h, BDEPTH_ERR_FORMAT, "corrupt BAM record (#%llu of the batch): its name, CIGAR, sequence and qualities do not fit its block_size", ss.bad_rec);
        if (ss.lead_n != ~0ull) return fail(h, BDEPTH_ERR_FORMAT, "read #%llu of the batch: its CIGAR begins with N%s (pileup.d:180-189): there is no result to reproduce", ss.lead_n,
                                             h->seg.on ? " -- the reference computes region / window statistics of such a read partly from its CIGAR as written and partly from a cursor that skips the leading N" : " and ends in a match -- the reference's pileup cursor runs past the read's sequence on such a read");
        if (ss.rg_err != ~0ull) return fail(h, BDEPTH_ERR_FORMAT, "error in read #%llu of the batch: its read group is not present in the header", ss.rg_err);
        st.n_records_pass += ss.n_pass; st.n_cigar_ops += ss.n_cigar; st.seq_bytes += ss.seq_bytes; st.long_reads += ss.n_long;
        if (ss.n_pass) { shard_min = std::min<uint64_t>(shard_min, ss.min_start); shard_max = std::max<uint64_t>(shard_max, ss.max_end); }
        if (mode == RUN_SCAN_ONLY) {
            if (ro && R) {
                uint64_t n = std::min<uint64_t>(R, ro->scan_cap > ro->scan_n ? ro->scan_cap - ro->scan_n : 0);
                std::vector<uint64_t> hs(n), ho(n); std::vector<uint32_t> hsp(n), hm(n), hn(n);
                CK(cudaMemcpy(hs.data(), soa.start, n * 8, cudaMemcpyDeviceToHost)); CK(cudaMemcpy(ho.data(), soa.off, n * 8, cudaMemcpyDeviceToHost));
                CK(cudaMemcpy(hsp.data(), soa.span, n * 4, cudaMemcpyDeviceToHost)); CK(cudaMemcpy(hm.data(), soa.meta, n * 4, cudaMemcpyDeviceToHost)); CK(cudaMemcpy(hn.data(), soa.ncl, n * 4, cudaMemcpyDeviceToHost));
                for (uint64_t i = 0; i < n; i++) {
                    uint64_t k = ro->scan_n + i; int32_t rid = -1, p = -1;
                    if (hs[i] != START_UNPLACED) { size_t lo = 0, hi = nref; while (lo + 1 < hi) { size_t m = (lo + hi) / 2; if (h->hdr.ref_lin0[m] <= hs[i]) lo = m; else hi = m; } while (lo + 1 < nref && h->hdr.ref_lin0[lo + 1] <= hs[i] && h->hdr.ref_len[lo] == 0) lo++; rid = (int32_t)lo; p = (int32_t)(hs[i] - h->hdr.ref_lin0[lo]); }
                    if (ro->ref_id) ro->ref_id[k] = rid; if (ro->pos) ro->pos[k] = p; if (ro->span) ro->span[k] = hsp[i];
                    if (ro->flag) ro->flag[k] = (uint16_t)(hm[i] >> 16); if (ro->mapq) ro->mapq[k] = (uint8_t)(hm[i] >> 8); if (ro->n_cigar) ro->n_cigar[k] = (uint16_t)(hn[i] >> 8);
                    if (ro->rec_off) ro->rec_off[k] = batch_u0 + ho[i] - 4;
                }
            }
            if (ro) ro->scan_n += R;
        }
        if (mode == RUN_INDEX && R) {
            auto& X = h->ix;
            CK(X.runs.ensure(R * sizeof(IndexRun))); CK(X.excs.ensure(R * sizeof(IndexExc)));
            BD_LAUNCH((unsigned)((R + 255) / 256), 256, 0, sm, k_index_scan)(soa, u0, (uint32_t)R, (unsigned long long)batch_u0, (int)nref, X.lin_base.as<uint32_t>(), X.lin_cap.as<uint32_t>(), X.lin.as<unsigned long long>(), X.lin_len.as<uint32_t>(),
                                                                               X.n_mapped.as<unsigned long long>(), X.n_unmapped.as<unsigned long long>(), X.carry.as<IndexCarry>(), X.runs.as<IndexRun>(), X.excs.as<IndexExc>(), X.ctl.as<IndexCtl>());
            BD_LAUNCH(1, 32, 0, sm, k_index_carry)(soa, u0, (unsigned long long)batch_u0, X.carry.as<IndexCarry>(), X.ctl.as<IndexCtl>());
            CK(cudaGetLastError()); st.gpu_launches += 2;
            DOWN(icp, IndexCtl, X.ctl.p, sizeof(IndexCtl));
            CK(cudaStreamSynchronize(sm));
            const IndexCtl ic = *icp;
            if (ic.bad_ref != ~0ull) return fail(h, BDEPTH_ERR_FORMAT, "record #%llu of the batch names a reference the header does not have", ic.bad_ref);
            if (ic.unsorted != ~0ull) return fail(h, BDEPTH_ERR_FORMAT, "BAM file is not coordinate-sorted (record #%llu of the batch lies before the read in front of it)", ic.unsorted);
            if (ic.past_end) return fail(h, BDEPTH_ERR_FORMAT, "%llu reads reach more than 16 kbp past the end of their reference: no index is built for such a file", ic.past_end);
            if (ic.n_runs) { size_t o = X.h_runs.size(); X.h_runs.resize(o + ic.n_runs); CK(cudaMemcpy(X.h_runs.data() + o, X.runs.p, ic.n_runs * sizeof(IndexRun), cudaMemcpyDeviceToHost)); std::sort(X.h_runs.begin() + o, X.h_runs.end(), [](const IndexRun& a, const IndexRun& b) { return a.start_abs < b.start_abs; }); }
            if (ic.n_exc) { size_t o = X.h_excs.size(); X.h_excs.resize(o + ic.n_exc); CK(cudaMemcpy(X.h_excs.data() + o, X.excs.p, ic.n_exc * sizeof(IndexExc), cudaMemcpyDeviceToHost)); std::sort(X.h_excs.begin() + o, X.h_excs.end(), [](const IndexExc& a, const IndexExc& b) { return a.start_abs < b.start_abs; }); }
            CK(cudaMemsetAsync(X.ctl.p, 0, 16, sm));
        }
        if (mode == RUN_FULL && h->seg.on && h->seg.n && ss.n_pass) {
            if (h->minq) BD_LAUNCH((unsigned)((R + 127) / 128), 128, 0, sm, k_read_segments<true>)(soa, u0, (uint32_t)R, h->seg.s.as<uint64_t>(), h->seg.e.as<uint64_t>(), h->seg.pmax.as<uint64_t>(), h->seg.id.as<uint32_t>(), h->seg.has_min ? h->seg.minstart.as<uint64_t>() : nullptr, h->seg.n, h->seg.reads.as<uint32_t>(), h->minq, h->S, h->seg.has_min ? h->seg.bases_reads.as<uint32_t>() : nullptr);
            else BD_LAUNCH((unsigned)((R + 127) / 128), 128, 0, sm, k_read_segments<false>)(soa, u0, (uint32_t)R, h->seg.s.as<uint64_t>(), h->seg.e.as<uint64_t>(), h->seg.pmax.as<uint64_t>(), h->seg.id.as<uint32_t>(), h->seg.has_min ? h->seg.minstart.as<uint64_t>() : nullptr, h->seg.n, h->seg.reads.as<uint32_t>(), 0, h->S, h->seg.has_min ? h->seg.bases_reads.as<uint32_t>() : nullptr);
            CK(cudaGetLastError()); st.gpu_launches++;
        }
        uint64_t idx_tiles_base = 0; uint32_t idx_n_tiles = 0;
        uint64_t gmin = std::min<uint64_t>(ss.min_start, ss.min_start_all), gmax = ss.max_end;
        if (ss.n_zone_pass && gmin < h->cnt_base) gmin = h->cnt_base;
        if (mode == RUN_FULL && (ss.n_pass || ss.n_zone_pass) && gmax > gmin) {
            if (gmin < h->cnt_base || gmax > h->cnt_base + h->win_len) {
                if (!h->bai_window_ok) return fail(h, BDEPTH_ERR_FORMAT, "read extends past the end of the reference space");
                h->bai_window_ok = false; CK(cudaDeviceSynchronize());
                if (h->force_window || h->accum) return RC_RETRY_WINDOW;
                return run_pipeline(h, mode, ro, em);
            }
            uint64_t t_lo = (gmin - h->cnt_base) / TILE_POS, t_hi = (gmax - h->cnt_base + TILE_POS - 1) / TILE_POS;
            uint64_t n_tiles = t_hi - t_lo; uint64_t tiles_base = h->cnt_base + t_lo * TILE_POS;
            idx_tiles_base = tiles_base; idx_n_tiles = (uint32_t)n_tiles;
            if (t_hi * TILE_POS > h->win_len) return fail(h, BDEPTH_ERR_FORMAT, "read extends past the end of the reference space");
            CK(h->tile_first.ensure((n_tiles + 2) * 4)); CK(h->tile_lo.ensure((n_tiles + 2) * 4));
            BD_LAUNCH((unsigned)((n_tiles + 2 + 255) / 256), 256, 0, sm, k_fill_u32)(h->tile_first.as<uint32_t>(), (uint32_t)R, n_tiles + 2);
            CK(cudaMemsetAsync(h->tile_lo.p, 0xFF, (n_tiles + 2) * 4, sm));
            if (h->want_presence) { BD_LAUNCH((unsigned)((R + 255) / 256), 256, 0, sm, k_presence)(soa, (uint32_t)R, h->cnt_base, h->win_len, h->present.as<uint32_t>()); st.gpu_launches++; }
            BD_LAUNCH((unsigned)((R + 255) / 256), 256, 0, sm, k3_tile_index)(soa, (uint32_t)R, tiles_base, (uint32_t)n_tiles, h->tile_first.as<uint32_t>(), h->tile_lo.as<uint32_t>());
            CK(cudaGetLastError()); st.gpu_launches += 2;
            for (uint32_t si = 0; si < h->S; si++) {
                uint32_t* cnt = h->counts.as<uint32_t>() + (uint64_t)si * N_PLANES * h->win_len; int sel = h->S > 1 ? (int)si : -1;
                if (ss.n_long) {
                    if (h->minq) BD_LAUNCH((unsigned)((ss.n_long * 32 + 255) / 256), 256, 0, sm, k3_scatter_long<true>)(soa, u0, h->long_list.as<uint32_t>(), (uint32_t)ss.n_long, h->cnt_base, h->win_len, cnt, h->minq, sel);
                    else BD_LAUNCH((unsigned)((ss.n_long * 32 + 255) / 256), 256, 0, sm, k3_scatter_long<false>)(soa, u0, h->long_list.as<uint32_t>(), (uint32_t)ss.n_long, h->cnt_base, h->win_len, cnt, 0, sel);
                    CK(cudaGetLastError()); st.gpu_launches++;
                }
                if (h->k3_tile) {
                    if (h->minq) BD_LAUNCH((unsigned)n_tiles, 256, K3T_SMEM, sm, k3_tile<true>)(soa, u0, (int64_t)ub, (uint32_t)R, tiles_base, h->cnt_base, h->win_len, h->tile_first.as<uint32_t>(), h->tile_lo.as<uint32_t>(), cnt, h->minq, sel);
                    else BD_LAUNCH((unsigned)n_tiles, 256, K3T_SMEM, sm, k3_tile<false>)(soa, u0, (int64_t)ub, (uint32_t)R, tiles_base, h->cnt_base, h->win_len, h->tile_first.as<uint32_t>(), h->tile_lo.as<uint32_t>(), cnt, 0, sel);
                } else if (h->k3_pre) {
                    if (h->minq) BD_LAUNCH((unsigned)n_tiles, 256, 0, sm, k3_gather<true, true>)(soa, u0, tiles_base, h->cnt_base, h->win_len, h->tile_first.as<uint32_t>(), h->tile_lo.as<uint32_t>(), cnt, h->minq, sel);
                    else BD_LAUNCH((unsigned)n_tiles, 256, 0, sm, k3_gather<false, true>)(soa, u0, tiles_base, h->cnt_base, h->win_len, h->tile_first.as<uint32_t>(), h->tile_lo.as<uint32_t>(), cnt, 0, sel);
                } else if (h->minq) BD_LAUNCH((unsigned)n_tiles, 256, 0, sm, k3_gather<true, false>)(soa, u0, tiles_base, h->cnt_base, h->win_len, h->tile_first.as<uint32_t>(), h->tile_lo.as<uint32_t>(), cnt, h->minq, sel);
                else BD_LAUNCH((unsigned)n_tiles, 256, 0, sm, k3_gather<false, false>)(soa, u0, tiles_base, h->cnt_base, h->win_len, h->tile_first.as<uint32_t>(), h->tile_lo.as<uint32_t>(), cnt, 0, sel);
                CK(cudaGetLastError()); st.gpu_launches++;
            }
        }
        if (fix) {
            const uint64_t tail_abs = batch_u0 + (uint64_t)tail; size_t lo = 0, hi = B.size(); while (lo + 1 < hi) { size_t m2 = (lo + hi) / 2; if (B[m2].uoff <= tail_abs) lo = m2; else hi = m2; }
            ghost_b = lo; ghost_entry = (int64_t)(tail_abs - B[lo].uoff); ghost_below_abs = tail_abs;
        }
        if (fix && R && (ss.n_pass || ss.n_ghost || ss.n_ghost_right)) {
            if (subs.size() != 1) return fail(h, BDEPTH_ERR_ARG, "internal: fix-mate-overlaps scans a batch as a whole");
            uint64_t s_last = 0;
            CK(cudaMemcpyAsync(&s_last, soa.start + (R - 1), 8, cudaMemcpyDeviceToHost, sm)); CK(cudaStreamSynchronize(sm));
            cudaEvent_t em0 = h->ev[20], em1 = h->ev[21];
            CK(cudaEventRecord(em0, sm));
            CK(h->m_hash.ensure(Rc * 8)); CK(h->m_flag.ensure(Rc * 4)); CK(h->m_ctl.ensure(64));
            std::vector<uint64_t> fl;
            for (auto& g : h->regions) fl.push_back(h->hdr.ref_lin0[g.ref_id] + g.start);
            for (auto& g : h->regions) fl.push_back(h->hdr.ref_lin0[g.ref_id] + g.end);
            const uint32_t n_flt = (uint32_t)h->regions.size();
            CK(h->m_flt.ensure(fl.size() * 8 + 16));
            if (n_flt) CK(cudaMemcpyAsync(h->m_flt.p, fl.data(), fl.size() * 8, cudaMemcpyHostToDevice, sm));
            CK(cudaMemsetAsync(h->m_ctl.p, 0, 64, sm)); CK(cudaMemsetAsync((uint8_t*)h->m_ctl.p + 48, 0xFF, 16, sm));
            const bool segm = h->seg.on && h->seg.n;
            MateParams mp{soa.start, soa.span, soa.meta, soa.off, soa.ncl, soa.lseq, u0, (uint32_t)R, h->m_hash.as<uint64_t>(), h->m_flag.as<uint32_t>(),
                          h->m_flt.as<uint64_t>(), h->m_flt.as<uint64_t>() + n_flt, n_flt, h->counts.as<uint32_t>(), h->cnt_base, h->win_len, h->S, h->minq,
                          segm ? h->seg.s.as<uint64_t>() : nullptr, segm ? h->seg.e.as<uint64_t>() : nullptr, segm ? h->seg.pmax.as<uint64_t>() : nullptr, segm ? h->seg.id.as<uint32_t>() : nullptr,
                          segm ? h->seg.n : 0u, segm ? h->seg.reads.as<uint32_t>() : nullptr, segm ? h->seg.mbases.as<uint32_t>() : nullptr, h->S,
                          segm && h->seg.has_u ? h->seg.ustart.as<uint64_t>() : nullptr, segm && h->seg.has_u && h->seg.has_min ? h->seg.minstart.as<uint64_t>() : nullptr, segm && h->seg.has_u ? h->seg.ext_max : 0ull,
                          h->tile_lo.as<uint32_t>(), idx_tiles_base, idx_n_tiles, h->long_list.as<uint32_t>(), (uint32_t)ss.n_long,
                          (uint32_t)ss.n_ghost, s_last, prev_s_last, covered_from, last_batch ? 1 : 0, (unsigned long long*)((uint8_t*)h->m_ctl.p + 48), (unsigned long long*)((uint8_t*)h->m_ctl.p + 56),
                          (last_batch && blk_hi < B.size()) ? 1 : 0, (unsigned long long*)((uint8_t*)h->m_ctl.p + 40), (uint32_t)ss.n_ghost_right, ghost_below == INT64_MIN ? INT64_MIN : ghost_below + 4, 0,
                          (int*)h->m_ctl.p, (unsigned long long*)((uint8_t*)h->m_ctl.p + 16)};
            const unsigned mg = (unsigned)((R + 127) / 128);
            BD_LAUNCH(mg, 128, 0, sm, km_hash)(mp); BD_LAUNCH(mg, 128, 0, sm, km_link)(mp); BD_LAUNCH(mg, 128, 0, sm, km_fix)(mp);
            if (!last_batch) { BD_LAUNCH(mg, 128, 0, sm, km_cover)(mp); st.gpu_launches++; }
            CK(cudaGetLastError()); st.gpu_launches += 3;
            CK(cudaEventRecord(em1, sm));
            struct { int err[4]; unsigned long long stat[3]; unsigned long long fix_max_end; unsigned long long open_off, open_start; } ctl;
            CK(cudaMemcpyAsync(&ctl, h->m_ctl.p, sizeof ctl, cudaMemcpyDeviceToHost, sm));
            CK(cudaStreamSynchronize(sm));
            if (ctl.err[0] == MATE_ERR_TOO_MANY) return fail(h, BDEPTH_ERR_ARG, "fix-mate-overlaps: more than %d reads of one name cover one position (record #%d of the batch)", MATE_MAX_MEMBERS, ctl.err[1]);
            if (ctl.err[0] == MATE_ERR_CROSS) return fail(h, BDEPTH_ERR_ARG, "fix-mate-overlaps: four or more overlapping reads of one name next to a batch boundary (record #%d of the batch): not reproduced there, use larger batches", ctl.err[1]);
            st.mate_pairs += ctl.stat[0]; st.mate_pair_columns += ctl.stat[1]; st.mate_groups += ctl.stat[2];
            if (!last_batch && ctl.open_off != ~0ull && batch_u0 + (ctl.open_off - 4) < ghost_below_abs) {
                const uint64_t g_abs = batch_u0 + (ctl.open_off - 4); size_t lo = 0, hi = B.size(); while (lo + 1 < hi) { size_t m2 = (lo + hi) / 2; if (B[m2].uoff <= g_abs) lo = m2; else hi = m2; }
                ghost_b = lo; ghost_entry = (int64_t)(g_abs - B[lo].uoff);
            }
            if (ctl.err[0] == MATE_ERR_ZONE) return fail(h, BDEPTH_ERR_ARG, "fix-mate-overlaps on several ranks: overlapping reads of one name reach more than %u BGZF blocks past a shard boundary (record #%d of the batch)", MATE_ZONE_BLOCKS, ctl.err[1]);
            if (ctl.fix_max_end > shard_max && shard_min != UINT64_MAX) shard_max = ctl.fix_max_end;
            prev_s_last = s_last; covered_from = ctl.open_start;
            { float t = 0; CK(cudaEventElapsedTime(&t, em0, em1)); st.ms_mates += t; }
        }
        CK(cudaEventRecord(e4, sm));
        if (mode == RUN_FLAGSTAT && R) {
            const int64_t own_from = h->world > 1 ? (int64_t)h->own_lo_abs_u - (int64_t)batch_u0 : INT64_MIN;
            CK(cudaEventRecord(h->ev[22], sm));
            BD_LAUNCH((unsigned)((R + 255) / 256), 256, 0, sm, k_flagstat)(soa, u0, (uint32_t)R, own_from, h->fs.as<unsigned long long>());
            CK(cudaGetLastError()); st.gpu_launches++;
            CK(cudaEventRecord(h->ev[23], sm));
        }
        if (mode == RUN_VIEW_COUNT && R) {
            const int64_t own_from = (h->world > 1 && !sparse) ? (int64_t)h->own_lo_abs_u - (int64_t)batch_u0 : INT64_MIN;
            CK(cudaEventRecord(h->ev[22], sm));
            BD_LAUNCH((unsigned)((R + 255) / 256), 256, 0, sm, k_view_count)(soa, u0, (uint32_t)R, own_from, h->vsel, h->vc.as<unsigned long long>());
            CK(cudaGetLastError()); st.gpu_launches++;
            CK(cudaEventRecord(h->ev[23], sm));
        }
        if (mode == RUN_VIEW_TEXT && R) {
            const int64_t own_from = (h->world > 1 && !sparse) ? (int64_t)h->own_lo_abs_u - (int64_t)batch_u0 : INT64_MIN;
            rc = view_text_sub(h, soa, u0, (uint32_t)R, own_from); if (rc) return rc;
        }
        const bool zone_mode = h->world > 1 && h->comm && !fix && !sparse;
        if (em && zone_mode && h->rank > 0 && shard_min != UINT64_MAX) em->lo_clip = shard_min;
        if (em && mode == RUN_FULL && (h->world == 1 || (zone_mode && (h->rank == 0 || shard_min != UINT64_MAX))) && !fix && !last_batch && ss.n_pass) { int rce = em->advance(ss.max_start / TILE_POS * TILE_POS, e4); if (rce) return rce; }
        uint64_t new_carry = (uint64_t)((int64_t)ub - tail);
        if (last_batch && last_sub && !sparse && !limited && b1 == B.size() && new_carry >= 4) return fail(h, BDEPTH_ERR_FORMAT, "truncated BAM record at the end of the file (not enough data in stream)");
        if (!last_batch && last_sub && new_carry && !fix) {
            if (new_carry > CARRY_MAX) return fail(h, BDEPTH_ERR_FORMAT, "BAM record larger than %zu bytes", CARRY_MAX);
            CK(cudaMemcpyAsync(m_u0 - new_carry, u0 + tail, new_carry, cudaMemcpyDeviceToDevice, sm));
        }
        CK(cudaStreamSynchronize(sm));
        if ((mode == RUN_FLAGSTAT || mode == RUN_VIEW_COUNT) && R) { float t; CK(cudaEventElapsedTime(&t, h->ev[22], h->ev[23])); ms_census += t; }
        { float t; if (!h->staged && last_sub) { CK(cudaEventElapsedTime(&t, h->ev[18 + (batch_no & 1)], h->ev[14 + (batch_no & 1)])); ms_h2d += t; } if (last_sub) { CK(cudaEventElapsedTime(&t, e1, e2)); ms_k1 += t; } CK(cudaEventElapsedTime(&t, e2, e3)); ms_k2 += t; CK(cudaEventElapsedTime(&t, e3, e4)); ms_k3 += t; }
        carry_len = (last_batch || fix) ? 0 : new_carry; first_batch = false;
        hs.used = 0;
        }
        if (sparse_bad) break;
        }
        b = b1; batch_no++;
    }
    if (sparse && h->world > 1) {
        if (h->comm) {
            uint32_t flag = sparse_bad ? 1u : 0u;
            CK(cudaMemcpyAsync(h->misc.p, &flag, 4, cudaMemcpyHostToDevice, sm));
            NK(nccl().AllReduce(h->misc.p, h->misc.p, 1, NCCL_UINT32, NCCL_SUM, h->comm, sm));
            h->coll_pending = view ? 4 : 1;
            CK(cudaMemcpyAsync(&flag, h->misc.p, 4, cudaMemcpyDeviceToHost, sm)); CK(cudaStreamSynchronize(sm));
            if (flag >= SPARSE_PEER_FAILED) { h->coll_pending = 0; return fail(h, BDEPTH_ERR_NCCL, "another rank of the run stopped with an error (its own message says why): no result"); }
            sparse_bad = flag != 0;
        } else if (sparse_bad) return fail(h, BDEPTH_ERR_FORMAT, "the index does not describe this file (a region chunk does not end at a record); several ranks without a NCCL id cannot fall back together");
        if (sparse_bad && mode == RUN_VIEW_TEXT) { h->coll_pending = 4; return fail(h, BDEPTH_ERR_FORMAT, "the index does not describe this file (a region chunk does not end at a record), found after SAM lines were delivered"); }
        if (sparse_bad) { h->sparse_ok = false; CK(cudaDeviceSynchronize()); return run_pipeline(h, mode, ro, em); }
    }
    st.ms_h2d = ms_h2d; st.ms_inflate = ms_k1; st.ms_scan = ms_k2; st.ms_coverage = ms_k3;
    if (mode == RUN_FLAGSTAT) {
        if (h->world > 1 && h->comm) { NK(nccl().AllReduce(h->fs.p, h->fs.p, FS_WORDS + 1, NCCL_UINT64, NCCL_SUM, h->comm, sm)); h->coll_pending = 0; }
        CK(hs.ensure(16384)); hs.used = 0;
        DOWN(fsp, uint64_t, h->fs.p, (FS_WORDS + 1) * 8);
        CK(cudaStreamSynchronize(sm));
        memcpy(h->fs_host, fsp, sizeof h->fs_host);
        if (h->fs_host[FS_WORDS]) return fail(h, BDEPTH_ERR_NCCL, "another rank of the run stopped with an error (its own message says why): no result");
        st.ms_reduce = ms_census;
    }
    if (mode == RUN_VIEW_TEXT) { rc = view_text_flush(h); if (rc) return rc; st.ms_d2h = h->vt.ms_d2h; }
    if (view) {
        if (h->world > 1 && h->comm) { NK(nccl().AllReduce(h->vc.p, h->vc.p, 2, NCCL_UINT64, NCCL_SUM, h->comm, sm)); h->coll_pending = 0; }
        CK(hs.ensure(16384)); hs.used = 0;
        DOWN(vcp, uint64_t, h->vc.p, 16);
        CK(cudaStreamSynchronize(sm));
        memcpy(h->vc_host, vcp, sizeof h->vc_host);
        if (h->vc_host[1]) return fail(h, BDEPTH_ERR_NCCL, "another rank of the run stopped with an error (its own message says why): no result");
        st.ms_reduce = mode == RUN_VIEW_TEXT ? h->vt.ms_fmt : ms_census;
    }
    st.positions = mode == RUN_FULL ? h->hdr.total_len : 0;
    h->own_lo = 0; h->own_hi = h->hdr.total_len;
    if (mode == RUN_FULL) {
        if (h->world > 1 && h->comm) { rc = exchange_boundaries(h, shard_min, shard_max, sparse || fix); if (rc) return rc; }
        h->ref_has_host.assign(nref / 32 + 2, 0);
        CK(cudaMemcpyAsync(h->ref_has_host.data(), h->ref_has.p, (nref / 32 + 2) * 4, cudaMemcpyDeviceToHost, sm));
    }
    CK(cudaEventRecord(h->ev[11], sm));
    CK(cudaStreamSynchronize(sm));
    { float t = 0; CK(cudaEventElapsedTime(&t, h->ev[10], h->ev[11])); st.ms_span_device = t; }
    st.own_lo = h->own_lo; st.own_hi = h->own_hi;
    st.host_wall_ms = std::chrono::duration<double, std::milli>(std::chrono::steady_clock::now() - t_host0).count();
    return 0;
}

void swap_inputs(bdepth* a, bdepth* b) {
    std::swap(a->file, b->file); std::swap(a->file_len, b->file_len); std::swap(a->mapped, b->mapped); std::swap(a->fd, b->fd);
    std::swap(a->blocks, b->blocks); std::swap(a->total_u, b->total_u); std::swap(a->lazy, b->lazy); std::swap(a->framed_all, b->framed_all); std::swap(a->framed_off, b->framed_off);
    std::swap(a->hdr, b->hdr); std::swap(a->bai, b->bai); std::swap(a->has_index, b->has_index); std::swap(a->bai_window_ok, b->bai_window_ok);
    std::swap(a->shard_ready, b->shard_ready); std::swap(a->blk_lo, b->blk_lo); std::swap(a->blk_hi, b->blk_hi); std::swap(a->entry0, b->entry0);
    std::swap(a->limit_abs_u, b->limit_abs_u); std::swap(a->own_lo_abs_u, b->own_lo_abs_u); std::swap(a->zone_lin_lo, b->zone_lin_lo);
    std::swap(a->sparse_ok, b->sparse_ok); std::swap(a->sparse_on, b->sparse_on); std::swap(a->vblocks, b->vblocks); std::swap(a->seg_entry, b->seg_entry); std::swap(a->seg_limit, b->seg_limit);
}
void index_extent(const bdepth* h, uint64_t& lo, uint64_t& hi) {
    const size_t nref = h->hdr.ref_len.size();
    lo = 0; hi = h->hdr.total_len;
    if (!(h->bai.valid && h->bai_window_ok && h->bai.ioffsets.size() == nref)) return;
    uint64_t a = UINT64_MAX, b = 0;
    for (size_t r = 0; r < nref; r++) {
        const auto& v = h->bai.ioffsets[r]; if (v.empty()) continue;
        size_t k = 0; while (k < v.size() && v[k] == 0) k++;
        if (k == v.size()) continue;
        a = std::min<uint64_t>(a, h->hdr.ref_lin0[r] + std::min<uint64_t>((uint64_t)k << 14, h->hdr.ref_len[r]));
        b = std::max<uint64_t>(b, h->hdr.ref_lin0[r] + std::min<uint64_t>((uint64_t)v.size() << 14, h->hdr.ref_len[r]));
    }
    if (a < b) { lo = a; hi = b; }
}
void add_stats(bdepth_stats& t, const bdepth_stats& s) {
    t.file_bytes += s.file_bytes; t.n_blocks += s.n_blocks; t.cdata_bytes += s.cdata_bytes; t.inflated_bytes += s.inflated_bytes; t.n_records += s.n_records; t.n_records_pass += s.n_records_pass;
    t.n_cigar_ops += s.n_cigar_ops; t.seq_bytes += s.seq_bytes; t.long_reads += s.long_reads; t.chain_fixups += s.chain_fixups; t.gpu_launches += s.gpu_launches; t.n_batches += s.n_batches;
    t.ms_h2d += s.ms_h2d; t.ms_inflate += s.ms_inflate; t.ms_scan += s.ms_scan; t.ms_coverage += s.ms_coverage; t.ms_span_device += s.ms_span_device; t.host_wall_ms += s.host_wall_ms;
}
int run_all_inputs(bdepth* h, Emitter* em = nullptr) {
    if (h->extra.empty()) return run_pipeline(h, RUN_FULL, nullptr, em);
    if (h->fix_mates) return fail(h, BDEPTH_ERR_ARG, "fix-mate-overlaps with several BAM files: not available (mates are paired within one file's stream)");
    if (h->world > 1) return fail(h, BDEPTH_ERR_ARG, "several BAM files on several ranks: not available");
    h->staged = false;
    for (int attempt = 0; attempt < 2; attempt++) {
        uint64_t lo = UINT64_MAX, hi = 0;
        for (size_t i = 0; i <= h->extra.size(); i++) {
            if (i) swap_inputs(h, h->extra[i - 1]);
            uint64_t a, b; index_extent(h, a, b); if (attempt) { a = 0; b = h->hdr.total_len; }
            lo = std::min(lo, a); hi = std::max(hi, b);
            if (i) swap_inputs(h, h->extra[i - 1]);
        }
        h->cnt_base = lo / TILE_POS * TILE_POS; h->win_len = ((hi - h->cnt_base + TILE_POS - 1) / TILE_POS + 1) * TILE_POS;
        h->force_window = true;
        bdepth_stats total{}; int rc = 0;
        for (size_t i = 0; i <= h->extra.size() && !rc; i++) {
            if (i) swap_inputs(h, h->extra[i - 1]);
            h->accum = i > 0;
            rc = run_pipeline(h, RUN_FULL, nullptr, nullptr);
            add_stats(total, h->st);
            if (i) swap_inputs(h, h->extra[i - 1]);
        }
        h->accum = false; h->force_window = false;
        if (rc == RC_RETRY_WINDOW) { if (attempt) return fail(h, BDEPTH_ERR_FORMAT, "read extends past the end of the reference space"); continue; }
        if (rc) return rc;
        total.positions = h->hdr.total_len; total.own_lo = h->own_lo; total.own_hi = h->own_hi;
        h->st = total;
        return 0;
    }
    return fail(h, BDEPTH_ERR_FORMAT, "internal: counter window");
}

void normalize_regions(const bdepth* h, const bdepth_region* r, size_t n, std::vector<bdepth_region>& out) {
    out.clear();
    for (size_t i = 0; i < n; i++) {
        if (r[i].ref_id >= h->hdr.ref_len.size() || r[i].start >= r[i].end) continue;
        bdepth_region g = r[i]; if (g.end > h->hdr.ref_len[g.ref_id]) g.end = h->hdr.ref_len[g.ref_id]; if (g.start >= g.end) continue;
        out.push_back(g);
    }
    std::sort(out.begin(), out.end(), [](const bdepth_region& a, const bdepth_region& b) { return a.ref_id != b.ref_id ? a.ref_id < b.ref_id : a.start != b.start ? a.start < b.start : a.end < b.end; });
    size_t m = 0;
    for (size_t i = 0; i < out.size(); i++) { if (m && out[m - 1].ref_id == out[i].ref_id && out[m - 1].end >= out[i].start) out[m - 1].end = std::max(out[m - 1].end, out[i].end); else out[m++] = out[i]; }
    out.resize(m);
}

}

extern "C" {

int bdepth_device_count(void) { int n = 0; if (cudaGetDeviceCount(&n) != cudaSuccess) return 0; return n; }

static int open_common(bdepth* h, bdepth_t** out) {
    int rc = finish_open(h);
    if (rc) { g_open_error = h->err; bdepth_close(h); return rc; }
    *out = h; return 0;
}

static int open_path(const char* bam_path, int device, bool lazy, bdepth_t** out);
int bdepth_open(const char* bam_path, int device, bdepth_t** out) { return open_path(bam_path, device, false, out); }
int bdepth_open_lazy(const char* bam_path, int device, bdepth_t** out) { return open_path(bam_path, device, true, out); }
static int open_path(const char* bam_path, int device, bool lazy, bdepth_t** out) {
    if (!bam_path || !out) return fail(nullptr, BDEPTH_ERR_ARG, "null argument");
    bdepth* h = new bdepth(); h->device = device; h->lazy = lazy;
    h->fd = open(bam_path, O_RDONLY);
    if (h->fd < 0) { delete h; return fail(nullptr, BDEPTH_ERR_IO, "Cannot open file `%s' in mode `rb' (No such file or directory)", bam_path); }
    struct stat sb; if (fstat(h->fd, &sb) != 0 || sb.st_size == 0) { close(h->fd); delete h; return fail(nullptr, BDEPTH_ERR_IO, "cannot stat `%s' or file is empty", bam_path); }
    h->file_len = (size_t)sb.st_size;
    void* m = mmap(nullptr, h->file_len, PROT_READ, MAP_PRIVATE, h->fd, 0);
    if (m == MAP_FAILED) { close(h->fd); delete h; return fail(nullptr, BDEPTH_ERR_IO, "cannot mmap `%s'", bam_path); }
    madvise(m, h->file_len, MADV_SEQUENTIAL);
    h->file = (const uint8_t*)m; h->mapped = true;
    std::string p1 = std::string(bam_path) + ".bai", p2; { std::string s(bam_path); size_t dot = s.rfind('.'); p2 = (dot == std::string::npos ? s + "." : s.substr(0, dot + 1)) + "bai"; }
    for (const std::string& bp : {p1, p2}) {
        FILE* f = fopen(bp.c_str(), "rb"); if (!f) continue;
        fseek(f, 0, SEEK_END); long n = ftell(f); fseek(f, 0, SEEK_SET);
        std::vector<uint8_t> buf(n > 0 ? n : 0); if (n > 0 && fread(buf.data(), 1, n, f) != (size_t)n) { fclose(f); continue; }
        fclose(f); h->has_index = true; parse_bai(buf.data(), buf.size(), h->bai); break;
    }
    return open_common(h, out);
}

int bdepth_open_memory(const void* bam, size_t bam_len, const void* bai, size_t bai_len, int device, bdepth_t** out) {
    if (!bam || !bam_len || !out) return fail(nullptr, BDEPTH_ERR_ARG, "null argument");
    bdepth* h = new bdepth(); h->device = device; h->file = (const uint8_t*)bam; h->file_len = bam_len;
    if (bai && bai_len) { h->has_index = true; parse_bai((const uint8_t*)bai, bai_len, h->bai); }
    return open_common(h, out);
}

int bdepth_add_input(bdepth_t* h, const char* bam_path) {
    if (!h || !bam_path) return fail(h, BDEPTH_ERR_ARG, "null argument");
    bdepth* x = nullptr;
    int rc = open_path(bam_path, h->device, h->lazy, &x);
    if (rc) { h->err = g_open_error; return rc; }
    if (x->hdr.ref_names != h->hdr.ref_names || x->hdr.ref_len != h->hdr.ref_len) { bdepth_close(x); return fail(h, BDEPTH_ERR_ARG, "%s: its reference sequences differ from the first file's (only identical sequence dictionaries can be merged)", bam_path); }
    const bool first_has_rg = !h->hdr.rg_ids.empty(), this_has_rg = !x->hdr.rg_ids.empty();
    std::vector<std::string> merged = first_has_rg ? h->hdr.sample_names : std::vector<std::string>();
    std::vector<int> remap(x->hdr.sample_names.size(), 0);
    if (this_has_rg) for (size_t i = 0; i < x->hdr.sample_names.size(); i++) {
        int id = -1; for (size_t k = 0; k < merged.size(); k++) if (merged[k] == x->hdr.sample_names[i]) id = (int)k;
        if (id < 0) { id = (int)merged.size(); merged.push_back(x->hdr.sample_names[i]); }
        remap[i] = id;
    }
    if (merged.empty()) merged.push_back("*");
    for (auto& sid : x->hdr.rg_sample) sid = remap[sid];
    x->hdr.sample_names = merged; h->hdr.sample_names = merged;
    for (bdepth* e : h->extra) e->hdr.sample_names = merged;
    x->comp.release(); x->descs.release(); x->status.release(); x->ubuf.release();
    h->extra.push_back(x);
    h->staged = false;
    return 0;
}

void bdepth_close(bdepth_t* h) {
    if (!h) return;
    for (bdepth* e : h->extra) bdepth_close(e);
    h->extra.clear();
    cudaSetDevice(h->device);
    h->anchors_idx.release(); h->anchors_val.release(); h->chunk_limit.release(); h->tok.release(); h->lits.release(); h->aux.release(); h->segi.release(); h->littab.release();
    DevBuf* bufs[] = {&h->comp, &h->descs, &h->status, &h->ubuf, &h->chunk_start, &h->entry, &h->exitb, &h->count, &h->slot_base, &h->slots, &h->rec_base, &h->walk_list, &h->soa_start, &h->soa_span, &h->soa_meta, &h->soa_off, &h->soa_ncl, &h->soa_lseq, &h->long_list, &h->tile_first, &h->tile_lo, &h->counts, &h->ref_len_d, &h->ref_lin0_d, &h->scan_stats, &h->ref_has, &h->ref_has_all, &h->flt_d, &h->lead_list, &h->misc};
    for (DevBuf* b : bufs) b->release();
    h->rg_ids.release(); h->rg_offs.release(); h->rg_samp.release();
    h->text[0].release(); h->text[1].release(); h->text_tiles.release(); h->text_offs.release(); h->text_zero.release(); h->text_samp.release(); h->present.release();
    h->seg.s.release(); h->seg.e.release(); h->seg.pmax.release(); h->seg.id.release(); h->seg.reads.release(); h->seg.minstart.release(); h->seg.bases_reads.release(); h->seg.mbases.release(); h->seg.ustart.release(); h->seg.dscr.release(); h->seg.da.release(); h->seg.dac.release(); h->seg.db.release(); h->seg.dthr.release(); h->seg.dbases.release(); h->seg.dcov.release();
    { auto& X = h->ix; X.lin.release(); X.lin_len.release(); X.lin_base.release(); X.lin_cap.release(); X.n_mapped.release(); X.n_unmapped.release(); X.carry.release(); X.ctl.release(); X.runs.release(); X.excs.release(); }
    h->m_hash.release(); h->m_flag.release(); h->m_flt.release(); h->m_ctl.release(); h->fprog_d.release();
    h->vc.release(); h->vc_reg.release(); h->vc_prog.release();
    { auto& V = h->vt; V.names.release(); V.len.release(); V.off.release(); V.tiles.release(); V.ctl.release(); V.cut_r.release(); V.cut_o.release(); V.slot[0].release(); V.slot[1].release(); if (V.host) cudaFreeHost(V.host); V.host = nullptr; V.cap = 0; }
    if (h->comm) { nccl().CommDestroy(h->comm); h->comm = nullptr; }
    if (h->pinned) cudaFreeHost(h->pinned);
    h->hs.release();
    if (h->s_main) { cudaStreamDestroy(h->s_main); cudaStreamDestroy(h->s_copy); cudaStreamDestroy(h->s_d2h); for (auto& ks : h->s_k1) cudaStreamDestroy(ks); for (auto& e : h->ev) cudaEventDestroy(e); for (int q = 0; q < 2; q++) for (auto& e : h->chunk_ev[q]) cudaEventDestroy(e); for (auto& e : h->k1_ev) cudaEventDestroy(e); }
    h->comp2[0].release(); h->comp2[1].release();
    if (h->mapped) munmap((void*)h->file, h->file_len);
    if (h->fd >= 0) close(h->fd);
    delete h;
}

const char* bdepth_last_error(const bdepth_t* h) { return h ? h->err.c_str() : g_open_error.c_str(); }

int bdepth_n_ref(const bdepth_t* h) { return (int)h->hdr.ref_len.size(); }
const char* bdepth_ref_name(const bdepth_t* h, int i) { return (i >= 0 && (size_t)i < h->hdr.ref_names.size()) ? h->hdr.ref_names[i].c_str() : nullptr; }
uint32_t bdepth_ref_length(const bdepth_t* h, int i) { return (i >= 0 && (size_t)i < h->hdr.ref_len.size()) ? h->hdr.ref_len[i] : 0; }
const char* bdepth_header_text(const bdepth_t* h, size_t* len) { if (len) *len = h->hdr.text.size(); return h->hdr.text.c_str(); }
int bdepth_is_coordinate_sorted(const bdepth_t* h) { for (const bdepth* e : h->extra) if (!e->hdr.so_coordinate) return 0; return h->hdr.so_coordinate ? 1 : 0; }
int bdepth_has_index(const bdepth_t* h) { for (const bdepth* e : h->extra) if (!e->has_index) return 0; return h->has_index ? 1 : 0; }
int bdepth_n_samples(const bdepth_t* h) { return (int)h->hdr.sample_names.size(); }
const char* bdepth_sample_name(const bdepth_t* h, int i) { return (i >= 0 && (size_t)i < h->hdr.sample_names.size()) ? h->hdr.sample_names[i].c_str() : nullptr; }

int bdepth_set_filter(bdepth_t* h, int mapq_gt, uint32_t flag_reject_mask) { h->mapq_gt = mapq_gt; h->flag_reject = flag_reject_mask; h->has_fprog = false; return 0; }
int bdepth_set_filter_query(bdepth_t* h, const char* query) {
    if (!query) return fail(h, BDEPTH_ERR_ARG, "null filter");
// ... 630 lines not shown
```

sambamba_b200/csrc/kernels.cuh:

```cuda
#pragma once
#include "launch.cuh"
#include <stdint.h>
#include "inflate_core.cuh"
#include "inflate2_core.cuh"
#include "filter.cuh"

namespace bdk {

constexpr int TILE_POS = 1024;
constexpr uint32_t SPAN_SHORT = 1024;
constexpr int N_PLANES = 7;
constexpr int64_t ENTRY_NONE = (int64_t)0x8080808080808080ull;
constexpr int ENTRY_NONE_BYTE = 0x80;

struct BlockDesc {
    uint64_t coff;
    uint64_t uoff;
    uint32_t csize;
    uint32_t isize;
    uint64_t tok_off;
};
BD_HD uint32_t tok_cap_of(uint32_t isize) { return isize / 4u + 16u; }
struct BlockAux { uint32_t n_tok, n_seg, n_lit, pad; };
BD_HD uint64_t lit_off_of(uint64_t uoff, uint64_t block_index) { return (uoff & ~15ull) + 16ull * block_index; }
// ... 349 lines not shown
    uint32_t* ncl;
    int32_t*  lseq;
};
struct ScanStats {
    unsigned long long n_pass, n_cigar, seq_bytes, max_end, min_start, n_long, max_start, rg_err;
    unsigned long long n_ghost;
    unsigned long long n_ghost_right;
    unsigned long long bad_rec;
    unsigned long long n_zone_pass, min_start_all;
    unsigned long long lead_n;
    unsigned long long n_lead;
};
constexpr uint64_t START_UNPLACED = 0xFFFFFFFFFFFFFFFEull;
constexpr uint32_t NCL_GHOST = 1u << 31;
constexpr uint32_t NCL_FOREIGN = 1u << 30;
struct RgTable { const uint8_t* ids; const uint32_t* offs; const uint8_t* sample_of; uint32_t n_rg; };

__device__ __forceinline__ int sample_of_record(const RgTable& rg, const uint8_t* aux, const uint8_t* end) {
    while (aux + 3 <= end) {
        uint8_t t0 = aux[0], t1 = aux[1], ty = aux[2];
        const uint8_t* v = aux + 3;
        if (t0 == 'R' && t1 == 'G' && ty == 'Z') {
            for (uint32_t g = 0; g < rg.n_rg; g++) {
                const uint8_t* id = rg.ids + rg.offs[g]; const uint8_t* q = v; bool eq = true;
                while (q < end && *q) { if (*id != *q) { eq = false; break; } id++; q++; }
                if (eq && *id == 0) return rg.sample_of[g];
            }
            return -1;
        }
        size_t n;
        switch (ty) {
        case 'A': case 'c': case 'C': n = 1; break;
        case 's': case 'S': n = 2; break;
        case 'i': case 'I': case 'f': n = 4; break;
        case 'Z': case 'H': { const uint8_t* q = v; while (q < end && *q) q++; n = (size_t)(q - v) + 1; break; }
        case 'B': { if (v + 5 > end) return 0; uint8_t st = v[0]; uint32_t cnt = ldu32(v + 1); size_t es = (st == 'c' || st == 'C') ? 1 : (st == 's' || st == 'S') ? 2 : 4; n = 5 + es * cnt; break; }
        default: return 0;
        }
        aux = v + n;
    }
    return 0;
}

__device__ __forceinline__ bool cig_rcons(uint32_t op) { return op == 0 || op == 2 || op == 3 || op == 7 || op == 8; }
__device__ __forceinline__ bool cig_qcons(uint32_t op) { return op == 0 || op == 1 || op == 4 || op == 7 || op == 8; }
__device__ __forceinline__ bool cig_match(uint32_t op) { return op == 0 || op == 7 || op == 8; }

__device__ BD_NOINLINE bool filter_eval_cold(const FilterProg* fp, const uint8_t* rec, uint32_t rec_size) { return filter_eval(*fp, rec, rec_size); }

template <bool FILTER, bool GHOST>
__global__ void k2_decode(ScanParams sp, const int64_t* __restrict__ chunk_start, uint32_t n_chunks, const uint32_t* __restrict__ slot_base,
                          const uint16_t* __restrict__ slots, const uint32_t* __restrict__ count, const uint32_t* __restrict__ rec_base,
                          RecordSoA soa, int mapq_gt, uint32_t flag_reject, ScanStats* __restrict__ st, uint32_t* __restrict__ long_list,
                          uint32_t* __restrict__ ref_has_reads, RgTable rg, const FilterProg* __restrict__ fprog ,
                          int64_t ghost_below, int64_t own_lo, int64_t own_hi, int64_t zone_below ) {
    uint32_t warp = (blockIdx.x * blockDim.x + threadIdx.x) >> 5, lane = threadIdx.x & 31;
    if (warp >= n_chunks) return;
    uint32_t n = count[warp];
    int64_t c0 = chunk_start[warp];
    const uint16_t* sl = slots + slot_base[warp];
    uint32_t rb = rec_base[warp];
    unsigned long long loc_pass = 0, loc_cig = 0, loc_seq = 0, loc_maxend = 0, loc_minstart = ~0ull, loc_maxstart = 0;
    uint32_t has_word = 0xFFFFFFFFu, has_bits = 0;
    unsigned long long loc_ghost = 0, loc_ghost_r = 0, loc_zone = 0, loc_minall = ~0ull;
    for (uint32_t k = lane; k < n; k += 32) {
        int64_t o = ((k == 0 || c0 > 0) ? c0 : 0) + sl[k];
        const uint8_t* p = sp.u + o + 4;
        uintptr_t pa = reinterpret_cast<uintptr_t>(p);
        const uint32_t* pw = reinterpret_cast<const uint32_t*>(pa & ~uintptr_t(3)); uint32_t psh = (uint32_t)(pa & 3) * 8;
        uint32_t h0 = __ldg(pw), h1 = __ldg(pw + 1), h2 = __ldg(pw + 2), h3 = __ldg(pw + 3), h4 = __ldg(pw + 4), h5 = __ldg(pw + 5);
        int32_t ref = (int32_t)__funnelshift_r(h0, h1, psh), pos = (int32_t)__funnelshift_r(h1, h2, psh);
        uint32_t bmn = __funnelshift_r(h2, h3, psh), fnc = __funnelshift_r(h3, h4, psh);
        int32_t l_seq = (int32_t)__funnelshift_r(h4, h5, psh);
        uint32_t l_name = bmn & 0xFF, mapq = (bmn >> 8) & 0xFF, flag = fnc >> 16, n_cigar = fnc & 0xFFFF;
        const uint8_t* cg = p + 32 + l_name;
        uint64_t span = 0;
        {
            const uint32_t bs = __funnelshift_r(__ldg(pw - 1), h0, psh);
            const uint64_t need = 32ull + l_name + 4ull * n_cigar + (l_seq > 0 ? ((uint64_t)(uint32_t)l_seq + 1) / 2 + (uint32_t)l_seq : 0ull);
            if (l_seq < 0 || need > bs) { atomicMin(&st->bad_rec, (unsigned long long)(rb + k) + 1); n_cigar = 0; l_seq = 0; ref = -1; }
        }
        for (uint32_t i = 0; i < n_cigar; i++) { uint32_t c = ldu32(cg + 4 * i); if (cig_rcons(c & 15)) span += c >> 4; }
        bool placed = ref >= 0 && ref < sp.n_ref && pos >= 0;
        bool pass = placed && !(flag & 4u) && span > 0;
        if (pass) { if (FILTER) pass = filter_eval_cold(fprog, p, ldu32(sp.u + o)); else pass = ((int)mapq > mapq_gt) && !(flag & flag_reject); }
        uint64_t start = placed ? sp.ref_lin0[ref] + (uint64_t)pos : START_UNPLACED;
        uint32_t span_eff = 0;
        if (pass) {
            uint64_t room = (uint32_t)pos < sp.ref_len[ref] ? (uint64_t)sp.ref_len[ref] - (uint32_t)pos : 0;
            span_eff = (uint32_t)(span < room ? span : room);
            if (span_eff == 0) pass = false;
        }
        bool is_long = pass && span_eff > SPAN_SHORT;
        uint32_t r = rb + k;
        uint32_t sample = 0;
        if (rg.n_rg && pass) {
            uint32_t bs = ldu32(sp.u + o);
            int sid = sample_of_record(rg, cg + 4u * n_cigar + ((uint32_t)l_seq + 1) / 2 + (uint32_t)l_seq, p + bs);
            if (sid < 0) { atomicMin(&st->rg_err, (unsigned long long)r + 1); sid = 0; }
            sample = (uint32_t)sid & 63u;
        }
        uint32_t ghost_bit = 0;
        if (GHOST) {
            const bool foreign = o < own_lo || o >= own_hi;
            if (foreign || o < ghost_below) { if (o >= own_hi) loc_ghost_r++; else loc_ghost++; if (pass) ghost_bit = NCL_GHOST | (foreign ? NCL_FOREIGN : 0u); pass = false; is_long = false; }
        }
        const bool zone = !GHOST && o < zone_below;
        if (zone) { loc_ghost++; if (pass) ghost_bit = NCL_FOREIGN; }
        soa.start[r] = start; soa.span[r] = span_eff;
        soa.meta[r] = (flag << 16) | (mapq << 8) | (sample << 2) | (pass ? 1u : 0u) | (is_long ? 2u : 0u);
        soa.off[r] = o + 4; soa.ncl[r] = (n_cigar << 8) | l_name | ghost_bit; soa.lseq[r] = l_seq;
        if (!zone) loc_cig += n_cigar;
        if (pass && zone) {
            loc_zone++;
            if (start < loc_minall) loc_minall = start;
            if (start + span_eff > loc_maxend) loc_maxend = start + span_eff;
            if (is_long) { uint32_t idx = (uint32_t)atomicAdd(&st->n_long, 1ull); long_list[idx] = r; }
        } else if (pass) {
            loc_pass++; loc_seq += ((uint64_t)l_seq + 1) / 2;
            if (start + span_eff > loc_maxend) loc_maxend = start + span_eff;
            if (start < loc_minstart) loc_minstart = start;
            if (start > loc_maxstart) loc_maxstart = start;
            if ((uint32_t)(ref >> 5) != has_word) { if (has_bits) atomicOr(&ref_has_reads[has_word], has_bits); has_word = (uint32_t)(ref >> 5); has_bits = 0; }
            has_bits |= 1u << (ref & 31);
            if (is_long) { uint32_t idx = (uint32_t)atomicAdd(&st->n_long, 1ull); long_list[idx] = r; }
        }
    }
    if (loc_zone) { atomicAdd(&st->n_zone_pass, loc_zone); atomicMin(&st->min_start_all, loc_minall); }
    if (loc_ghost) atomicAdd(&st->n_ghost, loc_ghost);
    if (GHOST && loc_ghost_r) atomicAdd(&st->n_ghost_right, loc_ghost_r);
    {
        uint32_t w0 = __shfl_sync(0xFFFFFFFFu, has_word, 0);
        bool same = __all_sync(0xFFFFFFFFu, has_word == w0 || has_bits == 0);
        if (same) { uint32_t allb = __reduce_or_sync(0xFFFFFFFFu, has_bits); uint32_t ww = __reduce_min_sync(0xFFFFFFFFu, has_bits ? has_word : 0xFFFFFFFFu); if (lane == 0 && allb) atomicOr(&ref_has_reads[ww], allb); }
        else if (has_bits) atomicOr(&ref_has_reads[has_word], has_bits);
    }
    for (int s = 16; s; s >>= 1) {
        loc_pass += __shfl_xor_sync(0xFFFFFFFFu, loc_pass, s); loc_cig += __shfl_xor_sync(0xFFFFFFFFu, loc_cig, s); loc_seq += __shfl_xor_sync(0xFFFFFFFFu, loc_seq, s);
        unsigned long long m = __shfl_xor_sync(0xFFFFFFFFu, loc_maxend, s); if (m > loc_maxend) loc_maxend = m;
        m = __shfl_xor_sync(0xFFFFFFFFu, loc_minstart, s); if (m < loc_minstart) loc_minstart = m;
        m = __shfl_xor_sync(0xFFFFFFFFu, loc_maxstart, s); if (m > loc_maxstart) loc_maxstart = m;
    }
    if (lane == 0) {
        if (loc_pass) atomicAdd(&st->n_pass, loc_pass);
        if (loc_cig) atomicAdd(&st->n_cigar, loc_cig);
        if (loc_seq) atomicAdd(&st->seq_bytes, loc_seq);
        if (loc_maxend) atomicMax(&st->max_end, loc_maxend);
        if (loc_minstart != ~0ull) atomicMin(&st->min_start, loc_minstart);
        if (loc_maxstart) atomicMax(&st->max_start, loc_maxstart);
    }
}

__global__ void k3_tile_index(RecordSoA soa, uint32_t R, uint64_t win_base, uint32_t n_tiles, uint32_t* __restrict__ tile_first, uint32_t* __restrict__ tile_lo) {
    uint32_t r = blockIdx.x * blockDim.x + threadIdx.x;
    if (r >= R) return;
    uint64_t s = soa.start[r];
    if (s == START_UNPLACED) return;
    int64_t t_hi = s >= win_base ? (int64_t)((s - win_base) / TILE_POS) : -1;
    int64_t t_lo;
    uint32_t q = r; while (q > 0 && soa.start[q - 1] == START_UNPLACED) q--;
    if (q == 0) t_lo = 0;
    else { uint64_t ps = soa.start[q - 1]; t_lo = ps >= win_base ? (int64_t)((ps - win_base) / TILE_POS) + 1 : 0; }
    if (t_hi > (int64_t)n_tiles) t_hi = n_tiles;
    for (int64_t t = t_lo; t <= t_hi; t++) tile_first[t] = r;
    uint32_t m = soa.meta[r];
    if ((m & 3u) == 1u) {
        uint64_t e = s + soa.span[r] - 1;
        if (e >= win_base) {
            uint64_t ta = s >= win_base ? (s - win_base) / TILE_POS : 0, tb = (e - win_base) / TILE_POS;
            for (uint64_t t = ta; t <= tb && t < n_tiles; t++) atomicMin(&tile_lo[t], r);
        }
    }
}

__device__ __forceinline__ uint32_t ldg8(const uint8_t* p) { return (uint32_t)__ldg(p); }

struct GatherAcc {
    uint32_t packed[4];
    uint32_t wide[4][4];
    uint32_t nN[4], del[4], skip[4];
};

template <bool MINQ>
__device__ __forceinline__ void add_base(GatherAcc& a, int j, const uint8_t* seq, const uint8_t* qual, uint32_t q, uint32_t lseq, uint32_t minq) {
    if (q >= lseq) return;
    if (MINQ) { if (ldg8(qual + q) < minq) return; }
    uint32_t b = ldg8(seq + (q >> 1));
    uint32_t nib = (q & 1) ? (b & 15u) : (b >> 4);
    if (__popc(nib) == 1) a.packed[j] += 1u << ((31 - __clz(nib)) * 8);
    else a.nN[j]++;
}

template <bool MINQ, bool PRE>
__global__ void __launch_bounds__(256) k3_gather(RecordSoA soa, const uint8_t* __restrict__ u, uint64_t tiles_base, uint64_t cnt_base, uint64_t win_len,
                                                  const uint32_t* __restrict__ tile_first, const uint32_t* __restrict__ tile_lo,
                                                  uint32_t* __restrict__ counts, uint32_t minq, int sample_sel) {
    uint32_t tile = blockIdx.x;
    uint32_t lo = tile_lo[tile];
    if (lo == 0xFFFFFFFFu) return;
    uint32_t hi = tile_first[tile + 1];
    uint32_t lane = threadIdx.x & 31, warp = threadIdx.x >> 5;
    uint64_t w0 = tiles_base + (uint64_t)tile * TILE_POS + warp * 128u, w1 = w0 + 128;
    uint64_t p0 = w0 + 4u * lane;
    GatherAcc a;
#pragma unroll
    for (int j = 0; j < 4; j++) { a.packed[j] = 0; a.nN[j] = a.del[j] = a.skip[j] = 0; for (int c = 0; c < 4; c++) a.wide[j][c] = 0; }
    uint32_t since_flush = 0;
    for (uint32_t base = lo; base < hi; base += 32) {
        uint32_t r = base + lane;
        uint64_t s = 0; uint32_t sp = 0; bool ov = false;
        int64_t off_l = 0; uint32_t ncl_l = 0, lseq_l = 0, c0_l = 0;
        if (r < hi) {
            s = soa.start[r]; sp = soa.span[r];
            uint32_t mt = soa.meta[r];
            ov = (mt & 3u) == 1u && (sample_sel < 0 || (int)((mt >> 2) & 63u) == sample_sel) && s < w1 && s + sp > w0;
            if (PRE && ov) { off_l = soa.off[r]; ncl_l = soa.ncl[r]; lseq_l = (uint32_t)max(soa.lseq[r], 0); c0_l = ldu32(u + off_l + 32 + (ncl_l & 0xFF)); }
        }
        unsigned placed_m = __ballot_sync(0xFFFFFFFFu, r < hi && s != START_UNPLACED);
        if (placed_m) { uint64_t s_first = __shfl_sync(0xFFFFFFFFu, s, __ffs(placed_m) - 1); if (s_first >= w1) break; }
        unsigned m = __ballot_sync(0xFFFFFFFFu, ov);
        while (m) {
            int bsel = __ffs(m) - 1; m &= m - 1;
            uint32_t rr = base + bsel;
            uint64_t rs = __shfl_sync(0xFFFFFFFFu, s, bsel);
            uint32_t rspan = __shfl_sync(0xFFFFFFFFu, sp, bsel);
            int64_t off; uint32_t ncl, lseq;
            if (PRE) { off = __shfl_sync(0xFFFFFFFFu, off_l, bsel); ncl = __shfl_sync(0xFFFFFFFFu, ncl_l, bsel); lseq = __shfl_sync(0xFFFFFFFFu, lseq_l, bsel); }
            else { off = soa.off[rr]; ncl = soa.ncl[rr]; lseq = (uint32_t)max(soa.lseq[rr], 0); }
            uint32_t n_cigar = (ncl >> 8) & 0xFFFFu, l_name = ncl & 0xFF;
            const uint8_t* rec = u + off;
            const uint8_t* cg = rec + 32 + l_name;
            const uint8_t* seq = cg + 4u * n_cigar;
            const uint8_t* qual = seq + (lseq + 1) / 2;
            const int32_t rp = (int32_t)((int64_t)p0 - (int64_t)rs);
            const uint32_t c0 = PRE ? __shfl_sync(0xFFFFFFFFu, c0_l, bsel) : ldu32(cg);
            if (n_cigar == 1 && cig_match(c0 & 15)) {
                uint32_t L = min(min(c0 >> 4, rspan), lseq);
                if (rp + 3 >= 0 && rp < (int32_t)L) {
                    uint32_t xb = rp > 0 ? (uint32_t)rp : 0u, bq = xb >> 1;
                    uint32_t w = ldu32(seq + bq), wq = 0;
                    if (MINQ) wq = ldu32(qual + xb);
#pragma unroll
                    for (int j = 0; j < 4; j++) {
                        int32_t x = rp + j;
                        if (x >= 0 && x < (int32_t)L) {
                            bool okq = true;
                            if (MINQ) okq = ((wq >> (8 * ((uint32_t)x - xb))) & 0xFFu) >= minq;
                            uint32_t n = (uint32_t)x - 2 * bq;
                            uint32_t nib = (w >> (8 * (n >> 1) + ((n & 1) ? 0 : 4))) & 15u;
                            if (okq) { if (__popc(nib) == 1) a.packed[j] += 1u << ((31 - __clz(nib)) * 8); else a.nN[j]++; }
                        }
                    }
                }
            } else {
                uint32_t rpos = 0, qpos = 0;
                for (uint32_t i = 0; i < n_cigar; i++) {
                    uint32_t c = i == 0 ? c0 : ldu32(cg + 4 * i), len = c >> 4, op = c & 15;
                    if (cig_match(op)) {
#pragma unroll
                        for (int j = 0; j < 4; j++) {
                            int32_t x = rp + j - (int32_t)rpos;
                            if (x >= 0 && x < (int32_t)len && (uint32_t)(rp + j) < rspan) add_base<MINQ>(a, j, seq, qual, qpos + (uint32_t)x, lseq, minq);
                        }
                        rpos += len; qpos += len;
                    } else if (op == 2 || op == 3) {
#pragma unroll
                        for (int j = 0; j < 4; j++) {
                            int32_t x = rp + j - (int32_t)rpos;
                            if (x >= 0 && x < (int32_t)len && (uint32_t)(rp + j) < rspan) { if (op == 2) a.del[j]++; else a.skip[j]++; }
                        }
                        rpos += len;
                    } else if (cig_qcons(op)) qpos += len;
                    if ((int32_t)rpos > rp + 3) break;
                }
            }
            if (++since_flush == 255) {
                since_flush = 0;
#pragma unroll
                for (int j = 0; j < 4; j++) { for (int c = 0; c < 4; c++) a.wide[j][c] += (a.packed[j] >> (8 * c)) & 255u; a.packed[j] = 0; }
            }
        }
    }
#pragma unroll
    for (int j = 0; j < 4; j++) for (int c = 0; c < 4; c++) a.wide[j][c] += (a.packed[j] >> (8 * c)) & 255u;
    uint64_t idx = p0 - cnt_base;
    if (idx + 4 > win_len) return;
    uint32_t any = 0;
#pragma unroll
    for (int j = 0; j < 4; j++) any |= a.wide[j][0] | a.wide[j][1] | a.wide[j][2] | a.wide[j][3] | a.nN[j] | a.del[j] | a.skip[j];
    if (!any) return;
#pragma unroll
    for (int pl = 0; pl < N_PLANES; pl++) {
        uint32_t v[4];
#pragma unroll
        for (int j = 0; j < 4; j++) v[j] = pl < 4 ? a.wide[j][pl] : pl == 4 ? a.nN[j] : pl == 5 ? a.del[j] : a.skip[j];
        if (!(v[0] | v[1] | v[2] | v[3])) continue;
        uint4* dst = reinterpret_cast<uint4*>(counts + (uint64_t)pl * win_len + idx);
        uint4 cur = *dst;
        cur.x += v[0]; cur.y += v[1]; cur.z += v[2]; cur.w += v[3];
        *dst = cur;
    }
}

constexpr uint32_t K3T_STAGE = 40 * 1024;
constexpr uint32_t K3T_SMEM = N_PLANES * TILE_POS * 4 + K3T_STAGE + 64;
#ifndef BDEPTH_EMULATE_SHIM
__device__ __forceinline__ void mbar_init(uint32_t mbar_sa, uint32_t count) { asm volatile("mbarrier.init.shared::cta.b64 [%0], %1;" :: "r"(mbar_sa), "r"(count) : "memory"); asm volatile("fence.mbarrier_init.release.cluster;" ::: "memory"); }
__device__ __forceinline__ void bulk_g2s(uint32_t dst_sa, const void* src, uint32_t bytes, uint32_t mbar_sa) {
    asm volatile("mbarrier.arrive.expect_tx.shared::cta.b64 _, [%0], %1;" :: "r"(mbar_sa), "r"(bytes) : "memory");
    asm volatile("cp.async.bulk.shared::cluster.global.mbarrier::complete_tx::bytes [%0], [%1], %2, [%3];" :: "r"(dst_sa), "l"(src), "r"(bytes), "r"(mbar_sa) : "memory");
}
__device__ __forceinline__ void mbar_wait(uint32_t mbar_sa, uint32_t parity) {
    asm volatile("{\n.reg .pred p;\nWAIT_%=:\nmbarrier.try_wait.parity.shared::cta.b64 p, [%0], %1;\n@p bra DONE_%=;\nbra WAIT_%=;\nDONE_%=:\n}" :: "r"(mbar_sa), "r"(parity) : "memory");
}
#endif
template <bool MINQ>
__global__ void __launch_bounds__(256) k3_tile(RecordSoA soa, const uint8_t* __restrict__ u, int64_t u_end, uint32_t R, uint64_t tiles_base, uint64_t cnt_base, uint64_t win_len,
                                               const uint32_t* __restrict__ tile_first, const uint32_t* __restrict__ tile_lo, uint32_t* __restrict__ counts, uint32_t minq, int sample_sel) {
    BD_DYN_SMEM(uint8_t, smem_raw);
    uint32_t* cnt = reinterpret_cast<uint32_t*>(smem_raw);
    uint8_t* stage = smem_raw + N_PLANES * TILE_POS * 4;
    __shared__ unsigned long long s_mbar; __shared__ uint32_t s_r1;
    const uint32_t tile = blockIdx.x, tid = threadIdx.x, lane = tid & 31, warp = tid >> 5;
    const uint32_t lo = tile_lo[tile];
    if (lo == 0xFFFFFFFFu) return;
    const uint32_t hi = tile_first[tile + 1];
    const uint64_t t0 = tiles_base + (uint64_t)tile * TILE_POS;
    for (uint32_t i = tid; i < N_PLANES * TILE_POS; i += 256) cnt[i] = 0;
#ifndef BDEPTH_EMULATE_SHIM
    const uint32_t mbar_sa = (uint32_t)__cvta_generic_to_shared(&s_mbar);
    if (tid == 0) mbar_init(mbar_sa, 1);
#endif
    __syncthreads();
    uint32_t parity = 0;
    for (uint32_t r0 = lo; r0 < hi;) {
        const int64_t c0 = (int64_t)((reinterpret_cast<uintptr_t>(u) + (uintptr_t)(soa.off[r0] - 4)) & ~uintptr_t(15)) - (int64_t)reinterpret_cast<uintptr_t>(u);
        if (warp == 0) {
            uint32_t a = r0 + 1, b = hi;
            while (a < b) { uint32_t m = (a + b + 1) >> 1; int64_t e = m < R ? soa.off[m] - 4 : u_end; if (e - c0 <= (int64_t)K3T_STAGE) a = m; else b = m - 1; }
            if (lane == 0) s_r1 = a;
        }
        __syncthreads();
        const uint32_t r1 = s_r1;
        const int64_t c1 = r1 < R ? soa.off[r1] - 4 : u_end;
        const bool staged = c1 - c0 <= (int64_t)K3T_STAGE;
        if (staged) {
            const uint32_t bytes = (uint32_t)((c1 - c0 + 15) & ~int64_t(15));
#ifndef BDEPTH_EMULATE_SHIM
            if (tid == 0) bulk_g2s((uint32_t)__cvta_generic_to_shared(stage), u + c0, bytes, mbar_sa);
            mbar_wait(mbar_sa, parity); parity ^= 1;
#else
            for (uint32_t i = tid; i < bytes; i += 256) stage[i] = u[c0 + i];
            __syncthreads();
#endif
        }
        const uint8_t* const rb = staged ? stage - c0 : u;
        const uint32_t per_warp = (r1 - r0 + 7) / 8, wa = r0 + warp * per_warp, wb = min(r1, wa + per_warp);
        for (uint32_t rb0 = wa; rb0 < wb; rb0 += 32) {
            const uint32_t rl = rb0 + lane;
            uint32_t mt_l = 0, span_l = 0, ncl_l = 0, lseq_l = 0; uint64_t rs_l = 0; int64_t off_l = 0; bool want = false;
            if (rl < wb) {
                mt_l = soa.meta[rl]; rs_l = soa.start[rl]; span_l = soa.span[rl];
                want = (mt_l & 3u) == 1u && (sample_sel < 0 || (int)((mt_l >> 2) & 63u) == sample_sel) && rs_l < t0 + TILE_POS && rs_l + span_l > t0;
                if (want) { off_l = soa.off[rl]; ncl_l = soa.ncl[rl]; lseq_l = (uint32_t)max(soa.lseq[rl], 0); }
            }
            unsigned todo = __ballot_sync(0xFFFFFFFFu, want);
            while (todo) {
            const int src = __ffs(todo) - 1; todo &= todo - 1;
            const uint64_t rs = __shfl_sync(0xFFFFFFFFu, rs_l, src); const uint32_t rspan = __shfl_sync(0xFFFFFFFFu, span_l, src);
            const int64_t off = __shfl_sync(0xFFFFFFFFu, off_l, src); const uint32_t ncl = __shfl_sync(0xFFFFFFFFu, ncl_l, src), lseq = __shfl_sync(0xFFFFFFFFu, lseq_l, src);
            const uint32_t n_cigar = (ncl >> 8) & 0xFFFFu, l_name = ncl & 0xFF;
            const uint8_t* cg = rb + off + 32 + l_name; const uint8_t* seq = cg + 4u * n_cigar; const uint8_t* qual = seq + (lseq + 1) / 2;
            const uint32_t w_lo = rs < t0 ? (uint32_t)(t0 - rs) : 0u;
            const uint32_t w_hi = (uint32_t)min((uint64_t)rspan, t0 + TILE_POS - rs);
            const uint32_t pbase = (uint32_t)(rs - t0);
            uint32_t rpos = 0, qpos = 0;
            for (uint32_t i = 0; i < n_cigar && rpos < w_hi; i++) {
                const uint32_t c = ld_u32_any(cg + 4 * i), len = c >> 4, op = c & 15;
                if (cig_match(op)) {
                    const uint32_t xa = rpos < w_lo ? w_lo - rpos : 0u, xb = min(len, w_hi - rpos);
                    for (uint32_t x = xa + lane; x < xb; x += 32) {
                        const uint32_t q = qpos + x;
                        if (q >= lseq) break;
                        if (MINQ) { if ((uint32_t)qual[q] < minq) continue; }
                        const uint32_t b = seq[q >> 1], nib = (q & 1) ? (b & 15u) : (b >> 4);
                        const uint32_t pl = (__popc(nib) == 1) ? (31 - __clz(nib)) : 4;
                        atomicAdd(&cnt[pl * TILE_POS + (pbase + rpos + x)], 1u);
                    }
                    rpos += len; qpos += len;
                } else if (op == 2 || op == 3) {
                    const uint32_t xa = rpos < w_lo ? w_lo - rpos : 0u, xb = min(len, w_hi - rpos);
                    const uint32_t pl = op == 2 ? 5u : 6u;
                    for (uint32_t x = xa + lane; x < xb; x += 32) atomicAdd(&cnt[pl * TILE_POS + (pbase + rpos + x)], 1u);
                    rpos += len;
                } else if (cig_qcons(op)) qpos += len;
            }
            }
        }
        __syncthreads();
        r0 = r1;
    }
    const uint64_t idx0 = t0 - cnt_base;
    if (idx0 + TILE_POS > win_len) return;
    for (uint32_t i = tid; i < N_PLANES * TILE_POS / 4; i += 256) {
        const uint4 v = reinterpret_cast<const uint4*>(cnt)[i];
        if (!(v.x | v.y | v.z | v.w)) continue;
        const uint32_t pl = i / (TILE_POS / 4), p4 = i % (TILE_POS / 4);
        uint4* dst = reinterpret_cast<uint4*>(counts + (uint64_t)pl * win_len + idx0) + p4;
        uint4 cur = *dst; cur.x += v.x; cur.y += v.y; cur.z += v.z; cur.w += v.w; *dst = cur;
    }
}

template <bool MINQ>
__global__ void k3_scatter_long(RecordSoA soa, const uint8_t* __restrict__ u, const uint32_t* __restrict__ long_list, uint32_t n_long,
                                uint64_t win_base, uint64_t win_len, uint32_t* __restrict__ counts, uint32_t minq, int sample_sel) {
    uint32_t warp = (blockIdx.x * blockDim.x + threadIdx.x) >> 5, lane = threadIdx.x & 31;
    if (warp >= n_long) return;
    uint32_t rr = long_list[warp];
    if (sample_sel >= 0 && (int)((soa.meta[rr] >> 2) & 63u) != sample_sel) return;
    uint64_t rs = soa.start[rr]; uint32_t rspan = soa.span[rr];
    int64_t off = soa.off[rr]; uint32_t ncl = soa.ncl[rr]; uint32_t lseq = (uint32_t)max(soa.lseq[rr], 0);
    uint32_t n_cigar = (ncl >> 8) & 0xFFFFu, l_name = ncl & 0xFF;
    const uint8_t* rec = u + off; const uint8_t* cg = rec + 32 + l_name; const uint8_t* seq = cg + 4u * n_cigar; const uint8_t* qual = seq + (lseq + 1) / 2;
    uint32_t rpos = 0, qpos = 0;
    for (uint32_t i = 0; i < n_cigar; i++) {
        uint32_t c = ldu32(cg + 4 * i), len = c >> 4, op = c & 15;
        if (cig_match(op)) {
            for (uint32_t x = lane; x < len; x += 32) {
                uint32_t rp = rpos + x, q = qpos + x;
                if (rp >= rspan || q >= lseq) continue;
                uint64_t g = rs + rp; if (g < win_base || g - win_base >= win_len) continue;
                if (MINQ) { if (ldg8(qual + q) < minq) continue; }
                uint32_t b = ldg8(seq + (q >> 1)); uint32_t nib = (q & 1) ? (b & 15u) : (b >> 4);
                uint32_t pl = (__popc(nib) == 1) ? (31 - __clz(nib)) : 4;
                atomicAdd(counts + (uint64_t)pl * win_len + (g - win_base), 1u);
            }
            rpos += len; qpos += len;
        } else if (op == 2 || op == 3) {
            uint32_t pl = op == 2 ? 5 : 6;
            for (uint32_t x = lane; x < len; x += 32) {
                uint32_t rp = rpos + x; if (rp >= rspan) continue;
                uint64_t g = rs + rp; if (g < win_base || g - win_base >= win_len) continue;
                atomicAdd(counts + (uint64_t)pl * win_len + (g - win_base), 1u);
            }
            rpos += len;
        } else if (cig_qcons(op)) qpos += len;
    }
}

struct IndexCarry { unsigned long long has, key, end_abs; int ref, pos; };
struct IndexRun { unsigned long long start_abs, prev_end_abs; int ref; uint32_t bin; };
struct IndexExc { unsigned long long start_abs, end_abs; int ref; uint32_t unmapped; };
struct IndexCtl {
    unsigned long long n_runs, n_exc, last_valid , first_placed_abs, unsorted , past_end, bad_ref, no_coord;
};
struct IndexRec { int ref, pos; uint32_t bin, unmapped; int64_t end_pos ; unsigned long long abs_s, abs_e; };

__device__ __forceinline__ IndexRec index_rec(const RecordSoA& soa, const uint8_t* u, uint32_t r, unsigned long long batch_u0) {
    const int64_t o = soa.off[r];
    const uint8_t* p = u + o;
    IndexRec x;
    x.ref = (int)ldu32(p); x.pos = (int)ldu32(p + 4);
    const uint32_t bmn = ldu32(p + 8), fnc = ldu32(p + 12), bs = ldu32(p - 4);
    x.bin = bmn >> 16; x.unmapped = (fnc >> 16) & 4u ? 1u : 0u;
    const uint32_t l_name = bmn & 0xFF, n_cigar = fnc & 0xFFFF;
    int64_t bc = 0;
    if (!x.unmapped) { const uint8_t* cg = p + 32 + l_name; for (uint32_t i = 0; i < n_cigar; i++) { uint32_t c = ldu32(cg + 4 * i); if (cig_rcons(c & 15)) bc += c >> 4; } }
    x.end_pos = (int64_t)x.pos + bc;
    x.abs_s = batch_u0 + (unsigned long long)(o - 4); x.abs_e = x.abs_s + 4ull + bs;
    return x;
}

__global__ void k_index_scan(RecordSoA soa, const uint8_t* __restrict__ u, uint32_t R, unsigned long long batch_u0, int n_ref,
                             const uint32_t* __restrict__ lin_base, const uint32_t* __restrict__ lin_cap, unsigned long long* __restrict__ lin, uint32_t* __restrict__ lin_len,
                             unsigned long long* __restrict__ n_mapped, unsigned long long* __restrict__ n_unmapped,
                             const IndexCarry* __restrict__ carry, IndexRun* __restrict__ runs, IndexExc* __restrict__ excs, IndexCtl* __restrict__ ctl) {
    const uint32_t r = blockIdx.x * blockDim.x + threadIdx.x, lane = threadIdx.x & 31;
    const bool in = r < R;
    IndexRec x{-1, -1, 0, 0, 0, 0, 0};
    if (in) x = index_rec(soa, u, r, batch_u0);
    const bool valid = in && x.ref >= 0 && x.pos >= 0, placed = in && x.ref != -1;
    if (in && x.ref >= n_ref) { atomicMin(&ctl->bad_ref, (unsigned long long)r + 1); }
    const bool ok_ref = x.ref < n_ref;
    if (placed) {
        bool have = false; int pref = -1, ppos = -1; unsigned long long pkey = 0, pend = ~0ull;
        for (int64_t q = (int64_t)r - 1; q >= 0; q--) {
            IndexRec y = index_rec(soa, u, (uint32_t)q, batch_u0);
            if (y.ref >= 0 && y.pos >= 0) { have = true; pref = y.ref; ppos = y.pos; pkey = ((unsigned long long)(uint32_t)y.ref << 32) | y.bin; pend = y.abs_e; break; }
        }
        if (!have && carry->has) { have = true; pref = carry->ref; ppos = carry->pos; pkey = carry->key; pend = carry->end_abs; }
        if (have && !(pref < x.ref) && !(x.ref == pref && x.pos >= ppos)) atomicMin(&ctl->unsorted, (unsigned long long)r + 1);
        if (ctl->first_placed_abs > x.abs_s) atomicMin(&ctl->first_placed_abs, x.abs_s);
        if (valid && ok_ref) {
            const unsigned long long key = ((unsigned long long)(uint32_t)x.ref << 32) | x.bin;
            if (!have || key != pkey) { unsigned long long i = atomicAdd(&ctl->n_runs, 1ull); runs[i] = IndexRun{x.abs_s, have ? pend : ~0ull, x.ref, x.bin}; }
            const int64_t last = x.unmapped ? (int64_t)x.pos : x.end_pos - 1;
            const uint32_t w0 = (uint32_t)x.pos >> 14, w1 = last < 0 ? 0u : (uint32_t)(last >> 14);
            const uint32_t cap = lin_cap[x.ref]; unsigned long long* L = lin + lin_base[x.ref];
            for (uint32_t w = w0; w <= w1; w++) {
                if (w >= cap) { atomicAdd(&ctl->past_end, 1ull); break; }
                if (L[w] > x.abs_s) atomicMin(&L[w], x.abs_s);
            }
            if (w1 + 1 <= cap && lin_len[x.ref] < w1 + 1) atomicMax(&lin_len[x.ref], w1 + 1);
        } else if (!valid) {
            unsigned long long i = atomicAdd(&ctl->n_exc, 1ull); excs[i] = IndexExc{x.abs_s, x.abs_e, x.ref, x.unmapped};
        }
    }
    const int cref = !in ? -2 : (valid && ok_ref) ? x.ref : (x.ref == -1 ? -1 : -2);
    const int cref0 = __shfl_sync(0xFFFFFFFFu, cref, 0);
    const bool same = __all_sync(0xFFFFFFFFu, cref == cref0 || cref == -2);
    if (same) {
        const uint32_t bm = __ballot_sync(0xFFFFFFFFu, cref >= 0 && !x.unmapped), bu = __ballot_sync(0xFFFFFFFFu, cref >= 0 && x.unmapped), bn = __ballot_sync(0xFFFFFFFFu, cref == -1);
        const uint32_t any = __ballot_sync(0xFFFFFFFFu, cref >= 0); const int rr = __shfl_sync(0xFFFFFFFFu, cref, any ? (31 - __clz(any)) : 0);
        if (lane == 0) { if (bm) atomicAdd(&n_mapped[rr], (unsigned long long)__popc(bm)); if (bu) atomicAdd(&n_unmapped[rr], (unsigned long long)__popc(bu)); if (bn) atomicAdd(&ctl->no_coord, (unsigned long long)__popc(bn)); }
    } else {
        if (cref >= 0) { if (x.unmapped) atomicAdd(&n_unmapped[cref], 1ull); else atomicAdd(&n_mapped[cref], 1ull); }
        else if (cref == -1) atomicAdd(&ctl->no_coord, 1ull);
    }
    const uint32_t bv = __ballot_sync(0xFFFFFFFFu, valid && ok_ref);
    if (bv && lane == 31 - __clz(bv)) { if (ctl->last_valid < (unsigned long long)r + 1) atomicMax(&ctl->last_valid, (unsigned long long)r + 1); }
}

__global__ void k_index_carry(RecordSoA soa, const uint8_t* __restrict__ u, unsigned long long batch_u0, IndexCarry* __restrict__ carry, IndexCtl* __restrict__ ctl) {
    if (threadIdx.x || blockIdx.x) return;
    if (ctl->last_valid) {
        IndexRec y = index_rec(soa, u, (uint32_t)(ctl->last_valid - 1), batch_u0);
        carry->has = 1; carry->key = ((unsigned long long)(uint32_t)y.ref << 32) | y.bin; carry->end_abs = y.abs_e; carry->ref = y.ref; carry->pos = y.pos;
    }
    ctl->last_valid = 0;
}

__global__ void k_count_covered(const uint32_t* __restrict__ counts, uint64_t win_len, uint64_t a, uint64_t b, unsigned long long* __restrict__ out, int n_planes) {
    uint64_t i = a + (uint64_t)blockIdx.x * blockDim.x + threadIdx.x;
    uint64_t stride = (uint64_t)gridDim.x * blockDim.x;
    unsigned long long n = 0;
    for (; i < b; i += stride) {
        uint32_t s = 0;
        for (int pl = 0; pl < n_planes; pl++) s |= counts[(uint64_t)pl * win_len + i];
        n += s != 0;
    }
    for (int sft = 16; sft; sft >>= 1) n += __shfl_xor_sync(0xFFFFFFFFu, n, sft);
    if ((threadIdx.x & 31) == 0 && n) atomicAdd(out, n);
}

__global__ void k_segment_stats(const uint32_t* __restrict__ counts, uint64_t win_len, const uint64_t* __restrict__ seg_a, const uint64_t* __restrict__ seg_a_cov, const uint64_t* __restrict__ seg_b,
                                uint32_t n_seg, const uint32_t* __restrict__ thr, uint32_t n_thr, uint32_t* __restrict__ out_bases, uint32_t* __restrict__ out_cov ) {
    uint32_t warp = (blockIdx.x * blockDim.x + threadIdx.x) >> 5, lane = threadIdx.x & 31;
    if (warp >= n_seg) return;
    uint64_t a = seg_a[warp], ac = seg_a_cov[warp], b = seg_b[warp];
    uint32_t bases = 0; uint32_t cge[16];
#pragma unroll
    for (int t = 0; t < 16; t++) cge[t] = 0;
    for (uint64_t i = ac + lane; i < b; i += 32) {
        uint32_t s5 = 0, s = 0;
#pragma unroll
        for (int pl = 0; pl < N_PLANES; pl++) { uint32_t v = counts[(uint64_t)pl * win_len + i]; s += v; if (pl < 5) s5 += v; }
        if (i >= a) bases += s5;
        if (s) {
#pragma unroll
            for (int t = 0; t < 16; t++) if ((uint32_t)t < n_thr) cge[t] += s >= thr[t];
        }
    }
    for (int sft = 16; sft; sft >>= 1) {
// ... 648 lines not shown
```

Measured before the change: 45.83.

## Pipeline k3 tile staging with a producer warp and double-buffered bulk copies

Restructures the per-tile coverage kernel into a warp-specialized producer/consumer pipeline. A dedicated producer warp finds chunk boundaries with a warp-parallel search and issues bulk global-to-shared copies into two stage buffers, while eight consumer warps count bases from the other buffer, so loading overlaps compute. Tiles not yet written since the counter memset now store their counts directly instead of doing a read-modify-write. The tile-index kernel dedups atomicMin calls across adjacent lanes, and the long-read scatter now runs after the tile kernel. The old single-stage kernel is kept as an env option and per-kernel event timing stats are added, at the cost of more complexity and smaller stage buffers.

```diff
diff --git a/include/bdepth.h b/include/bdepth.h
--- a/include/bdepth.h
+++ b/include/bdepth.h
@@ -72,6 +72,8 @@
     uint64_t mate_pair_columns;
     uint64_t mate_groups;
     float ms_mates;
+    float ms_k3_index;
+    float ms_k3_tile;
 } bdepth_stats;
 
 int  bdepth_device_count(void);
diff --git a/sambamba_b200/_lib.py b/sambamba_b200/_lib.py
--- a/sambamba_b200/_lib.py
+++ b/sambamba_b200/_lib.py
@@ -38,7 +38,8 @@
                [(n, C.c_float) for n in ("ms_h2d", "ms_inflate", "ms_scan", "ms_coverage", "ms_reduce", "ms_d2h",
                                          "ms_total_device")] + [("host_wall_ms", C.c_double), ("ms_span_device", C.c_float), ("ms_exchange", C.c_float),
                                                                  ("own_lo", C.c_uint64), ("own_hi", C.c_uint64), ("halo_bytes_sent", C.c_uint64),
-                                                                 ("mate_pairs", C.c_uint64), ("mate_pair_columns", C.c_uint64), ("mate_groups", C.c_uint64), ("ms_mates", C.c_float)]
+                                                                 ("mate_pairs", C.c_uint64), ("mate_pair_columns", C.c_uint64), ("mate_groups", C.c_uint64), ("ms_mates", C.c_float),
+                                                                 ("ms_k3_index", C.c_float), ("ms_k3_tile", C.c_float)]
 
     def as_dict(self):
         return {n: getattr(self, n) for n, _ in self._fields_}
diff --git a/sambamba_b200/csrc/bdepth.cu b/sambamba_b200/csrc/bdepth.cu
--- a/sambamba_b200/csrc/bdepth.cu
+++ b/sambamba_b200/csrc/bdepth.cu
@@ -69,6 +69,7 @@
 constexpr uint32_t SHARD_EXTRA_BLOCKS = 8;
 constexpr uint32_t MATE_ZONE_BLOCKS = 64;
 
+enum K3Kernel { K3_TILE = 0, K3_TILE1 = 1, K3_GATHER = 2 };
 enum RunMode { RUN_FULL = 0, RUN_INFLATE_ONLY = 1, RUN_SCAN_ONLY = 2, RUN_INDEX = 3, RUN_FLAGSTAT = 4, RUN_VIEW_COUNT = 5, RUN_VIEW_TEXT = 6 };
 constexpr int RC_RETRY_WINDOW = 1;
 
@@ -139,7 +140,7 @@
     int k1h_variant = -1;
     bool k1_onephase = false;
     bool k3_pre = false;
-    bool k3_tile = true;
+    int k3_kernel = K3_TILE;
     bool has_fprog = false; FilterProg fprog; DevBuf fprog_d;
     DevBuf m_hash, m_flag, m_flt, m_ctl;
     uint32_t S = 1;
@@ -158,7 +159,7 @@
     std::vector<HostBlock> vblocks; std::vector<int32_t> seg_entry ; std::vector<uint32_t> seg_limit ;
     DevBuf anchors_idx, anchors_val, chunk_limit;
     cudaStream_t s_main = nullptr, s_copy = nullptr, s_d2h = nullptr;
-    cudaEvent_t ev[32] = {};
+    cudaEvent_t ev[36] = {};
     DevBuf comp2[2];
     cudaStream_t s_k1[16] = {};
     std::vector<cudaEvent_t> chunk_ev[2], k1_ev;
@@ -168,6 +169,7 @@
     DevBuf comp, descs, status, ubuf, chunk_start, entry, exitb, count, slot_base, slots, rec_base, walk_list;
     DevBuf soa_start, soa_span, soa_meta, soa_off, soa_ncl, soa_lseq, long_list, tile_first, tile_lo, counts, ref_len_d, ref_lin0_d, scan_stats, ref_has, ref_has_all, flt_d, lead_list, misc;
     uint64_t cnt_base = 0, win_len = 0;
+    uint64_t k3_fresh_from = UINT64_MAX;
     void* pinned = nullptr; size_t pinned_cap = 0;
     HostScratch hs;
     std::vector<uint32_t> ref_has_host;
@@ -223,8 +225,9 @@
     CK(cudaFuncSetAttribute(k1_huff<false, 4>, cudaFuncAttributePreferredSharedMemoryCarveout, cudaSharedmemCarveoutMaxShared)); CK(cudaFuncSetAttribute(k1_huff<false, 6>, cudaFuncAttributePreferredSharedMemoryCarveout, cudaSharedmemCarveoutMaxShared));
     CK(cudaFuncSetAttribute(k1_huff<true, 5>, cudaFuncAttributePreferredSharedMemoryCarveout, cudaSharedmemCarveoutMaxShared)); CK(cudaFuncSetAttribute(k1_huff<true, 4>, cudaFuncAttributePreferredSharedMemoryCarveout, cudaSharedmemCarveoutMaxShared));
     { const char* e = getenv("BDEPTH_K1H_VARIANT"); h->k1h_variant = e ? atoi(e) : -1; }
-    { const char* e = getenv("BDEPTH_K3"); h->k3_tile = !(e && !strcmp(e, "gather")); }
+    { const char* e = getenv("BDEPTH_K3"); h->k3_kernel = e && !strcmp(e, "gather") ? K3_GATHER : e && !strcmp(e, "tile1") ? K3_TILE1 : K3_TILE; }
     CK(cudaFuncSetAttribute(k3_tile<false>, cudaFuncAttributeMaxDynamicSharedMemorySize, (int)K3T_SMEM)); CK(cudaFuncSetAttribute(k3_tile<true>, cudaFuncAttributeMaxDynamicSharedMemorySize, (int)K3T_SMEM));
+    CK(cudaFuncSetAttribute(k3_tile1<false>, cudaFuncAttributeMaxDynamicSharedMemorySize, (int)K3T1_SMEM)); CK(cudaFuncSetAttribute(k3_tile1<true>, cudaFuncAttributeMaxDynamicSharedMemorySize, (int)K3T1_SMEM));
     { const char* e = getenv("BDEPTH_K1LZ"); h->k1lz_flat = e && !strcmp(e, "flat"); h->k1lz_v12 = e && !strcmp(e, "v12"); }
     { const char* e = getenv("BDEPTH_K1_ONEPHASE"); h->k1_onephase = e && atoi(e) == 1; }
     { const char* e = getenv("BDEPTH_K3_PREFETCH"); h->k3_pre = !e || atoi(e) != 0; }
@@ -722,7 +725,7 @@
         size_t free_b = 0, tot_b = 0; CK(cudaMemGetInfo(&free_b, &tot_b));
         if (need > h->counts.cap && need > free_b + h->counts.cap) return fail(h, BDEPTH_ERR_CUDA, "counter window needs %zu bytes of HBM, %zu free", need, free_b);
         CK(h->counts.ensure(need));
-        CK(cudaMemsetAsync(h->counts.p, 0, need, sm));
+        CK(cudaMemsetAsync(h->counts.p, 0, need, sm)); h->k3_fresh_from = h->cnt_base;
         if (h->want_presence) { CK(h->present.ensure((h->win_len / 32 + 2) * 4)); CK(cudaMemsetAsync(h->present.p, 0, (h->win_len / 32 + 2) * 4, sm)); }
         CK(h->ref_has.ensure((nref / 32 + 2) * 4)); CK(cudaMemsetAsync(h->ref_has.p, 0, (nref / 32 + 2) * 4, sm));
     }
@@ -1113,6 +1116,7 @@
             CK(cudaGetLastError()); st.gpu_launches++;
         }
         uint64_t idx_tiles_base = 0; uint32_t idx_n_tiles = 0;
+        bool k3_ran = false;
         uint64_t gmin = std::min<uint64_t>(ss.min_start, ss.min_start_all), gmax = ss.max_end;
         if (ss.n_zone_pass && gmin < h->cnt_base) gmin = h->cnt_base;
         if (mode == RUN_FULL && (ss.n_pass || ss.n_zone_pass) && gmax > gmin) {
@@ -1130,25 +1134,33 @@
             BD_LAUNCH((unsigned)((n_tiles + 2 + 255) / 256), 256, 0, sm, k_fill_u32)(h->tile_first.as<uint32_t>(), (uint32_t)R, n_tiles + 2);
             CK(cudaMemsetAsync(h->tile_lo.p, 0xFF, (n_tiles + 2) * 4, sm));
             if (h->want_presence) { BD_LAUNCH((unsigned)((R + 255) / 256), 256, 0, sm, k_presence)(soa, (uint32_t)R, h->cnt_base, h->win_len, h->present.as<uint32_t>()); st.gpu_launches++; }
+            CK(cudaEventRecord(h->ev[32], sm));
             BD_LAUNCH((unsigned)((R + 255) / 256), 256, 0, sm, k3_tile_index)(soa, (uint32_t)R, tiles_base, (uint32_t)n_tiles, h->tile_first.as<uint32_t>(), h->tile_lo.as<uint32_t>());
-            CK(cudaGetLastError()); st.gpu_launches += 2;
+            CK(cudaEventRecord(h->ev[33], sm));
+            CK(cudaGetLastError()); st.gpu_launches += 2; k3_ran = true;
             for (uint32_t si = 0; si < h->S; si++) {
                 uint32_t* cnt = h->counts.as<uint32_t>() + (uint64_t)si * N_PLANES * h->win_len; int sel = h->S > 1 ? (int)si : -1;
-                if (ss.n_long) {
-                    if (h->minq) BD_LAUNCH((unsigned)((ss.n_long * 32 + 255) / 256), 256, 0, sm, k3_scatter_long<true>)(soa, u0, h->long_list.as<uint32_t>(), (uint32_t)ss.n_long, h->cnt_base, h->win_len, cnt, h->minq, sel);
-                    else BD_LAUNCH((unsigned)((ss.n_long * 32 + 255) / 256), 256, 0, sm, k3_scatter_long<false>)(soa, u0, h->long_list.as<uint32_t>(), (uint32_t)ss.n_long, h->cnt_base, h->win_len, cnt, 0, sel);
-                    CK(cudaGetLastError()); st.gpu_launches++;
-                }
-                if (h->k3_tile) {
-                    if (h->minq) BD_LAUNCH((unsigned)n_tiles, 256, K3T_SMEM, sm, k3_tile<true>)(soa, u0, (int64_t)ub, (uint32_t)R, tiles_base, h->cnt_base, h->win_len, h->tile_first.as<uint32_t>(), h->tile_lo.as<uint32_t>(), cnt, h->minq, sel);
-                    else BD_LAUNCH((unsigned)n_tiles, 256, K3T_SMEM, sm, k3_tile<false>)(soa, u0, (int64_t)ub, (uint32_t)R, tiles_base, h->cnt_base, h->win_len, h->tile_first.as<uint32_t>(), h->tile_lo.as<uint32_t>(), cnt, 0, sel);
+                if (si == 0) CK(cudaEventRecord(h->ev[34], sm));
+                if (h->k3_kernel == K3_TILE) {
+                    if (h->minq) BD_LAUNCH((unsigned)n_tiles, K3T_THREADS, K3T_SMEM, sm, k3_tile<true>)(soa, u0, (int64_t)ub, (uint32_t)R, tiles_base, h->cnt_base, h->win_len, h->k3_fresh_from, h->tile_first.as<uint32_t>(), h->tile_lo.as<uint32_t>(), cnt, h->minq, sel);
+                    else BD_LAUNCH((unsigned)n_tiles, K3T_THREADS, K3T_SMEM, sm, k3_tile<false>)(soa, u0, (int64_t)ub, (uint32_t)R, tiles_base, h->cnt_base, h->win_len, h->k3_fresh_from, h->tile_first.as<uint32_t>(), h->tile_lo.as<uint32_t>(), cnt, 0, sel);
+                } else if (h->k3_kernel == K3_TILE1) {
+                    if (h->minq) BD_LAUNCH((unsigned)n_tiles, 256, K3T1_SMEM, sm, k3_tile1<true>)(soa, u0, (int64_t)ub, (uint32_t)R, tiles_base, h->cnt_base, h->win_len, h->tile_first.as<uint32_t>(), h->tile_lo.as<uint32_t>(), cnt, h->minq, sel);
+                    else BD_LAUNCH((unsigned)n_tiles, 256, K3T1_SMEM, sm, k3_tile1<false>)(soa, u0, (int64_t)ub, (uint32_t)R, tiles_base, h->cnt_base, h->win_len, h->tile_first.as<uint32_t>(), h->tile_lo.as<uint32_t>(), cnt, 0, sel);
                 } else if (h->k3_pre) {
                     if (h->minq) BD_LAUNCH((unsigned)n_tiles, 256, 0, sm, k3_gather<true, true>)(soa, u0, tiles_base, h->cnt_base, h->win_len, h->tile_first.as<uint32_t>(), h->tile_lo.as<uint32_t>(), cnt, h->minq, sel);
                     else BD_LAUNCH((unsigned)n_tiles, 256, 0, sm, k3_gather<false, true>)(soa, u0, tiles_base, h->cnt_base, h->win_len, h->tile_first.as<uint32_t>(), h->tile_lo.as<uint32_t>(), cnt, 0, sel);
                 } else if (h->minq) BD_LAUNCH((unsigned)n_tiles, 256, 0, sm, k3_gather<true, false>)(soa, u0, tiles_base, h->cnt_base, h->win_len, h->tile_first.as<uint32_t>(), h->tile_lo.as<uint32_t>(), cnt, h->minq, sel);
                 else BD_LAUNCH((unsigned)n_tiles, 256, 0, sm, k3_gather<false, false>)(soa, u0, tiles_base, h->cnt_base, h->win_len, h->tile_first.as<uint32_t>(), h->tile_lo.as<uint32_t>(), cnt, 0, sel);
                 CK(cudaGetLastError()); st.gpu_launches++;
+                if (ss.n_long) {
+                    if (h->minq) BD_LAUNCH((unsigned)((ss.n_long * 32 + 255) / 256), 256, 0, sm, k3_scatter_long<true>)(soa, u0, h->long_list.as<uint32_t>(), (uint32_t)ss.n_long, h->cnt_base, h->win_len, cnt, h->minq, sel);
+                    else BD_LAUNCH((unsigned)((ss.n_long * 32 + 255) / 256), 256, 0, sm, k3_scatter_long<false>)(soa, u0, h->long_list.as<uint32_t>(), (uint32_t)ss.n_long, h->cnt_base, h->win_len, cnt, 0, sel);
+                    CK(cudaGetLastError()); st.gpu_launches++;
+                }
             }
+            CK(cudaEventRecord(h->ev[35], sm));
+            h->k3_fresh_from = std::max<uint64_t>(h->k3_fresh_from, tiles_base + n_tiles * TILE_POS);
         }
         if (fix) {
             const uint64_t tail_abs = batch_u0 + (uint64_t)tail; size_t lo = 0, hi = B.size(); while (lo + 1 < hi) { size_t m2 = (lo + hi) / 2; if (B[m2].uoff <= tail_abs) lo = m2; else hi = m2; }
@@ -1229,6 +1241,7 @@
         CK(cudaStreamSynchronize(sm));
         if ((mode == RUN_FLAGSTAT || mode == RUN_VIEW_COUNT) && R) { float t; CK(cudaEventElapsedTime(&t, h->ev[22], h->ev[23])); ms_census += t; }
         { float t; if (!h->staged && last_sub) { CK(cudaEventElapsedTime(&t, h->ev[18 + (batch_no & 1)], h->ev[14 + (batch_no & 1)])); ms_h2d += t; } if (last_sub) { CK(cudaEventElapsedTime(&t, e1, e2)); ms_k1 += t; } CK(cudaEventElapsedTime(&t, e2, e3)); ms_k2 += t; CK(cudaEventElapsedTime(&t, e3, e4)); ms_k3 += t; }
+        if (k3_ran) { float t; CK(cudaEventElapsedTime(&t, h->ev[32], h->ev[33])); st.ms_k3_index += t; CK(cudaEventElapsedTime(&t, h->ev[34], h->ev[35])); st.ms_k3_tile += t; }
         carry_len = (last_batch || fix) ? 0 : new_carry; first_batch = false;
         hs.used = 0;
         }
@@ -1272,7 +1285,7 @@
     st.positions = mode == RUN_FULL ? h->hdr.total_len : 0;
     h->own_lo = 0; h->own_hi = h->hdr.total_len;
     if (mode == RUN_FULL) {
-        if (h->world > 1 && h->comm) { rc = exchange_boundaries(h, shard_min, shard_max, sparse || fix); if (rc) return rc; }
+        if (h->world > 1 && h->comm) { h->k3_fresh_from = UINT64_MAX; rc = exchange_boundaries(h, shard_min, shard_max, sparse || fix); if (rc) return rc; }
         h->ref_has_host.assign(nref / 32 + 2, 0);
         CK(cudaMemcpyAsync(h->ref_has_host.data(), h->ref_has.p, (nref / 32 + 2) * 4, cudaMemcpyDeviceToHost, sm));
     }
@@ -1309,7 +1322,7 @@
 void add_stats(bdepth_stats& t, const bdepth_stats& s) {
     t.file_bytes += s.file_bytes; t.n_blocks += s.n_blocks; t.cdata_bytes += s.cdata_bytes; t.inflated_bytes += s.inflated_bytes; t.n_records += s.n_records; t.n_records_pass += s.n_records_pass;
     t.n_cigar_ops += s.n_cigar_ops; t.seq_bytes += s.seq_bytes; t.long_reads += s.long_reads; t.chain_fixups += s.chain_fixups; t.gpu_launches += s.gpu_launches; t.n_batches += s.n_batches;
-    t.ms_h2d += s.ms_h2d; t.ms_inflate += s.ms_inflate; t.ms_scan += s.ms_scan; t.ms_coverage += s.ms_coverage; t.ms_span_device += s.ms_span_device; t.host_wall_ms += s.host_wall_ms;
+    t.ms_h2d += s.ms_h2d; t.ms_inflate += s.ms_inflate; t.ms_scan += s.ms_scan; t.ms_coverage += s.ms_coverage; t.ms_k3_index += s.ms_k3_index; t.ms_k3_tile += s.ms_k3_tile; t.ms_span_device += s.ms_span_device; t.host_wall_ms += s.host_wall_ms;
 }
 int run_all_inputs(bdepth* h, Emitter* em = nullptr) {
     if (h->extra.empty()) return run_pipeline(h, RUN_FULL, nullptr, em);
diff --git a/sambamba_b200/csrc/kernels.cuh b/sambamba_b200/csrc/kernels.cuh
--- a/sambamba_b200/csrc/kernels.cuh
+++ b/sambamba_b200/csrc/kernels.cuh
@@ -525,25 +525,31 @@
 }
 
 __global__ void k3_tile_index(RecordSoA soa, uint32_t R, uint64_t win_base, uint32_t n_tiles, uint32_t* __restrict__ tile_first, uint32_t* __restrict__ tile_lo) {
-    uint32_t r = blockIdx.x * blockDim.x + threadIdx.x;
-    if (r >= R) return;
-    uint64_t s = soa.start[r];
-    if (s == START_UNPLACED) return;
-    int64_t t_hi = s >= win_base ? (int64_t)((s - win_base) / TILE_POS) : -1;
-    int64_t t_lo;
-    uint32_t q = r; while (q > 0 && soa.start[q - 1] == START_UNPLACED) q--;
-    if (q == 0) t_lo = 0;
-    else { uint64_t ps = soa.start[q - 1]; t_lo = ps >= win_base ? (int64_t)((ps - win_base) / TILE_POS) + 1 : 0; }
-    if (t_hi > (int64_t)n_tiles) t_hi = n_tiles;
-    for (int64_t t = t_lo; t <= t_hi; t++) tile_first[t] = r;
-    uint32_t m = soa.meta[r];
-    if ((m & 3u) == 1u) {
-        uint64_t e = s + soa.span[r] - 1;
-        if (e >= win_base) {
-            uint64_t ta = s >= win_base ? (s - win_base) / TILE_POS : 0, tb = (e - win_base) / TILE_POS;
-            for (uint64_t t = ta; t <= tb && t < n_tiles; t++) atomicMin(&tile_lo[t], r);
-        }
-    }
+    const uint32_t r = blockIdx.x * blockDim.x + threadIdx.x;
+    uint32_t key0 = 0xFFFFFFFFu, key1 = 0xFFFFFFFFu;
+    const uint64_t s = r < R ? soa.start[r] : START_UNPLACED;
+    if (s != START_UNPLACED) {
+        int64_t t_hi = s >= win_base ? (int64_t)((s - win_base) / TILE_POS) : -1;
+        int64_t t_lo;
+        uint32_t q = r; while (q > 0 && soa.start[q - 1] == START_UNPLACED) q--;
+        if (q == 0) t_lo = 0;
+        else { uint64_t ps = soa.start[q - 1]; t_lo = ps >= win_base ? (int64_t)((ps - win_base) / TILE_POS) + 1 : 0; }
+        if (t_hi > (int64_t)n_tiles) t_hi = n_tiles;
+        for (int64_t t = t_lo; t <= t_hi; t++) tile_first[t] = r;
+        uint32_t m = soa.meta[r];
+        if ((m & 3u) == 1u) {
+            uint64_t e = s + soa.span[r] - 1;
+            if (e >= win_base) {
+                uint64_t ta = s >= win_base ? (s - win_base) / TILE_POS : 0, tb = (e - win_base) / TILE_POS;
+                if (ta < n_tiles) key0 = (uint32_t)ta;
+                if (tb > ta && tb < n_tiles) key1 = (uint32_t)tb;
+            }
+        }
+    }
+    const uint32_t lane = threadIdx.x & 31;
+    const uint32_t p0 = __shfl_up_sync(0xFFFFFFFFu, key0, 1), p1 = __shfl_up_sync(0xFFFFFFFFu, key1, 1);
+    if (key0 != 0xFFFFFFFFu && (lane == 0 || p0 != key0)) atomicMin(&tile_lo[key0], r);
+    if (key1 != 0xFFFFFFFFu && (lane == 0 || p1 != key1)) atomicMin(&tile_lo[key1], r);
 }
 
 __device__ __forceinline__ uint32_t ldg8(const uint8_t* p) { return (uint32_t)__ldg(p); }
@@ -675,8 +681,11 @@
     }
 }
 
-constexpr uint32_t K3T_STAGE = 40 * 1024;
-constexpr uint32_t K3T_SMEM = N_PLANES * TILE_POS * 4 + K3T_STAGE + 64;
+constexpr uint32_t K3T1_STAGE = 40 * 1024;
+constexpr uint32_t K3T1_SMEM = N_PLANES * TILE_POS * 4 + K3T1_STAGE + 64;
+constexpr uint32_t K3T_STAGES = 2, K3T_STAGE = 23 * 1024;
+constexpr uint32_t K3T_SMEM = N_PLANES * TILE_POS * 4 + K3T_STAGES * K3T_STAGE;
+constexpr uint32_t K3T_THREADS = 9 * 32;
 #ifndef BDEPTH_EMULATE_SHIM
 __device__ __forceinline__ void mbar_init(uint32_t mbar_sa, uint32_t count) { asm volatile("mbarrier.init.shared::cta.b64 [%0], %1;" :: "r"(mbar_sa), "r"(count) : "memory"); asm volatile("fence.mbarrier_init.release.cluster;" ::: "memory"); }
 __device__ __forceinline__ void bulk_g2s(uint32_t dst_sa, const void* src, uint32_t bytes, uint32_t mbar_sa) {
@@ -686,59 +695,35 @@
 __device__ __forceinline__ void mbar_wait(uint32_t mbar_sa, uint32_t parity) {
     asm volatile("{\n.reg .pred p;\nWAIT_%=:\nmbarrier.try_wait.parity.shared::cta.b64 p, [%0], %1;\n@p bra DONE_%=;\nbra WAIT_%=;\nDONE_%=:\n}" :: "r"(mbar_sa), "r"(parity) : "memory");
 }
+typedef unsigned long long K3Bar;
+__device__ __forceinline__ uint32_t smem_u32(const void* p) { return (uint32_t)__cvta_generic_to_shared(p); }
+__device__ __forceinline__ void k3bar_init(K3Bar* b, uint32_t count) { mbar_init(smem_u32(b), count); }
+__device__ __forceinline__ void k3bar_arrive(K3Bar* b) { asm volatile("mbarrier.arrive.shared::cta.b64 _, [%0];" :: "r"(smem_u32(b)) : "memory"); }
+__device__ __forceinline__ void k3bar_copy(K3Bar* b, uint8_t* dst, const uint8_t* src, uint32_t bytes) { bulk_g2s(smem_u32(dst), src, bytes, smem_u32(b)); }
+__device__ __forceinline__ void k3bar_wait(K3Bar* b, uint32_t parity) { mbar_wait(smem_u32(b), parity); }
+#else
+struct K3Bar { uint32_t phase, pending, count; int64_t tx; };
+static inline void k3bar_done(K3Bar* b) { if (b->pending == 0 && b->tx == 0) { b->phase ^= 1u; b->pending = b->count; } }
+static inline void k3bar_init(K3Bar* b, uint32_t count) { b->phase = 0; b->pending = b->count = count; b->tx = 0; }
+static inline void k3bar_arrive(K3Bar* b) { b->pending--; k3bar_done(b); }
+static inline void k3bar_copy(K3Bar* b, uint8_t* dst, const uint8_t* src, uint32_t bytes) { b->tx += bytes; b->pending--; memcpy(dst, src, bytes); b->tx -= bytes; k3bar_done(b); }
+static inline void k3bar_wait(K3Bar* b, uint32_t parity) { while (b->phase == parity) emu::yield(); }
 #endif
+
 template <bool MINQ>
-__global__ void __launch_bounds__(256) k3_tile(RecordSoA soa, const uint8_t* __restrict__ u, int64_t u_end, uint32_t R, uint64_t tiles_base, uint64_t cnt_base, uint64_t win_len,
-                                               const uint32_t* __restrict__ tile_first, const uint32_t* __restrict__ tile_lo, uint32_t* __restrict__ counts, uint32_t minq, int sample_sel) {
-    BD_DYN_SMEM(uint8_t, smem_raw);
-    uint32_t* cnt = reinterpret_cast<uint32_t*>(smem_raw);
-    uint8_t* stage = smem_raw + N_PLANES * TILE_POS * 4;
-    __shared__ unsigned long long s_mbar; __shared__ uint32_t s_r1;
-    const uint32_t tile = blockIdx.x, tid = threadIdx.x, lane = tid & 31, warp = tid >> 5;
-    const uint32_t lo = tile_lo[tile];
-    if (lo == 0xFFFFFFFFu) return;
-    const uint32_t hi = tile_first[tile + 1];
-    const uint64_t t0 = tiles_base + (uint64_t)tile * TILE_POS;
-    for (uint32_t i = tid; i < N_PLANES * TILE_POS; i += 256) cnt[i] = 0;
-#ifndef BDEPTH_EMULATE_SHIM
-    const uint32_t mbar_sa = (uint32_t)__cvta_generic_to_shared(&s_mbar);
-    if (tid == 0) mbar_init(mbar_sa, 1);
-#endif
-    __syncthreads();
-    uint32_t parity = 0;
-    for (uint32_t r0 = lo; r0 < hi;) {
-        const int64_t c0 = (int64_t)((reinterpret_cast<uintptr_t>(u) + (uintptr_t)(soa.off[r0] - 4)) & ~uintptr_t(15)) - (int64_t)reinterpret_cast<uintptr_t>(u);
-        if (warp == 0) {
-            uint32_t a = r0 + 1, b = hi;
-            while (a < b) { uint32_t m = (a + b + 1) >> 1; int64_t e = m < R ? soa.off[m] - 4 : u_end; if (e - c0 <= (int64_t)K3T_STAGE) a = m; else b = m - 1; }
-            if (lane == 0) s_r1 = a;
-        }
-        __syncthreads();
-        const uint32_t r1 = s_r1;
-        const int64_t c1 = r1 < R ? soa.off[r1] - 4 : u_end;
-        const bool staged = c1 - c0 <= (int64_t)K3T_STAGE;
-        if (staged) {
-            const uint32_t bytes = (uint32_t)((c1 - c0 + 15) & ~int64_t(15));
-#ifndef BDEPTH_EMULATE_SHIM
-            if (tid == 0) bulk_g2s((uint32_t)__cvta_generic_to_shared(stage), u + c0, bytes, mbar_sa);
-            mbar_wait(mbar_sa, parity); parity ^= 1;
-#else
-            for (uint32_t i = tid; i < bytes; i += 256) stage[i] = u[c0 + i];
-            __syncthreads();
-#endif
-        }
-        const uint8_t* const rb = staged ? stage - c0 : u;
-        const uint32_t per_warp = (r1 - r0 + 7) / 8, wa = r0 + warp * per_warp, wb = min(r1, wa + per_warp);
-        for (uint32_t rb0 = wa; rb0 < wb; rb0 += 32) {
-            const uint32_t rl = rb0 + lane;
-            uint32_t mt_l = 0, span_l = 0, ncl_l = 0, lseq_l = 0; uint64_t rs_l = 0; int64_t off_l = 0; bool want = false;
-            if (rl < wb) {
-                mt_l = soa.meta[rl]; rs_l = soa.start[rl]; span_l = soa.span[rl];
-                want = (mt_l & 3u) == 1u && (sample_sel < 0 || (int)((mt_l >> 2) & 63u) == sample_sel) && rs_l < t0 + TILE_POS && rs_l + span_l > t0;
-                if (want) { off_l = soa.off[rl]; ncl_l = soa.ncl[rl]; lseq_l = (uint32_t)max(soa.lseq[rl], 0); }
-            }
-            unsigned todo = __ballot_sync(0xFFFFFFFFu, want);
-            while (todo) {
+__device__ __forceinline__ void k3_count_chunk(const RecordSoA& soa, const uint8_t* rb, uint32_t r0, uint32_t r1, uint32_t warp, uint32_t lane, uint64_t t0,
+                                               uint32_t* cnt, uint32_t minq, int sample_sel) {
+    const uint32_t per_warp = (r1 - r0 + 7) / 8, wa = r0 + warp * per_warp, wb = min(r1, wa + per_warp);
+    for (uint32_t rb0 = wa; rb0 < wb; rb0 += 32) {
+        const uint32_t rl = rb0 + lane;
+        uint32_t mt_l = 0, span_l = 0, ncl_l = 0, lseq_l = 0; uint64_t rs_l = 0; int64_t off_l = 0; bool want = false;
+        if (rl < wb) {
+            mt_l = soa.meta[rl]; rs_l = soa.start[rl]; span_l = soa.span[rl];
+            want = (mt_l & 3u) == 1u && (sample_sel < 0 || (int)((mt_l >> 2) & 63u) == sample_sel) && rs_l < t0 + TILE_POS && rs_l + span_l > t0;
+            if (want) { off_l = soa.off[rl]; ncl_l = soa.ncl[rl]; lseq_l = (uint32_t)max(soa.lseq[rl], 0); }
+        }
+        unsigned todo = __ballot_sync(0xFFFFFFFFu, want);
+        while (todo) {
             const int src = __ffs(todo) - 1; todo &= todo - 1;
             const uint64_t rs = __shfl_sync(0xFFFFFFFFu, rs_l, src); const uint32_t rspan = __shfl_sync(0xFFFFFFFFu, span_l, src);
             const int64_t off = __shfl_sync(0xFFFFFFFFu, off_l, src); const uint32_t ncl = __shfl_sync(0xFFFFFFFFu, ncl_l, src), lseq = __shfl_sync(0xFFFFFFFFu, lseq_l, src);
@@ -768,20 +753,130 @@
                     rpos += len;
                 } else if (cig_qcons(op)) qpos += len;
             }
-            }
-        }
-        __syncthreads();
-        r0 = r1;
-    }
+        }
+    }
+}
+
+__device__ __forceinline__ void k3_flush_tile(const uint32_t* cnt, uint64_t t0, uint64_t cnt_base, uint64_t win_len, uint32_t* __restrict__ counts, uint32_t tid, uint32_t n_threads, bool fresh) {
     const uint64_t idx0 = t0 - cnt_base;
     if (idx0 + TILE_POS > win_len) return;
-    for (uint32_t i = tid; i < N_PLANES * TILE_POS / 4; i += 256) {
+    for (uint32_t i = tid; i < N_PLANES * TILE_POS / 4; i += n_threads) {
         const uint4 v = reinterpret_cast<const uint4*>(cnt)[i];
         if (!(v.x | v.y | v.z | v.w)) continue;
         const uint32_t pl = i / (TILE_POS / 4), p4 = i % (TILE_POS / 4);
         uint4* dst = reinterpret_cast<uint4*>(counts + (uint64_t)pl * win_len + idx0) + p4;
+        if (fresh) { *dst = v; continue; }
         uint4 cur = *dst; cur.x += v.x; cur.y += v.y; cur.z += v.z; cur.w += v.w; *dst = cur;
     }
+}
+
+template <bool MINQ>
+__global__ void __launch_bounds__(256) k3_tile1(RecordSoA soa, const uint8_t* __restrict__ u, int64_t u_end, uint32_t R, uint64_t tiles_base, uint64_t cnt_base, uint64_t win_len,
+                                                const uint32_t* __restrict__ tile_first, const uint32_t* __restrict__ tile_lo, uint32_t* __restrict__ counts, uint32_t minq, int sample_sel) {
+    BD_DYN_SMEM(uint8_t, smem_raw);
+    uint32_t* cnt = reinterpret_cast<uint32_t*>(smem_raw);
+    uint8_t* stage = smem_raw + N_PLANES * TILE_POS * 4;
+    __shared__ unsigned long long s_mbar; __shared__ uint32_t s_r1;
+    const uint32_t tile = blockIdx.x, tid = threadIdx.x, lane = tid & 31, warp = tid >> 5;
+    const uint32_t lo = tile_lo[tile];
+    if (lo == 0xFFFFFFFFu) return;
+    const uint32_t hi = tile_first[tile + 1];
+    const uint64_t t0 = tiles_base + (uint64_t)tile * TILE_POS;
+    for (uint32_t i = tid; i < N_PLANES * TILE_POS; i += 256) cnt[i] = 0;
+#ifndef BDEPTH_EMULATE_SHIM
+    const uint32_t mbar_sa = (uint32_t)__cvta_generic_to_shared(&s_mbar);
+    if (tid == 0) mbar_init(mbar_sa, 1);
+#endif
+    __syncthreads();
+    uint32_t parity = 0;
+    for (uint32_t r0 = lo; r0 < hi;) {
+        const int64_t c0 = (int64_t)((reinterpret_cast<uintptr_t>(u) + (uintptr_t)(soa.off[r0] - 4)) & ~uintptr_t(15)) - (int64_t)reinterpret_cast<uintptr_t>(u);
+        if (warp == 0) {
+            uint32_t a = r0 + 1, b = hi;
+            while (a < b) { uint32_t m = (a + b + 1) >> 1; int64_t e = m < R ? soa.off[m] - 4 : u_end; if (e - c0 <= (int64_t)K3T1_STAGE) a = m; else b = m - 1; }
+            if (lane == 0) s_r1 = a;
+        }
+        __syncthreads();
+        const uint32_t r1 = s_r1;
+        const int64_t c1 = r1 < R ? soa.off[r1] - 4 : u_end;
+        const bool staged = c1 - c0 <= (int64_t)K3T1_STAGE;
+        if (staged) {
+            const uint32_t bytes = (uint32_t)((c1 - c0 + 15) & ~int64_t(15));
+#ifndef BDEPTH_EMULATE_SHIM
+            if (tid == 0) bulk_g2s((uint32_t)__cvta_generic_to_shared(stage), u + c0, bytes, mbar_sa);
+            mbar_wait(mbar_sa, parity); parity ^= 1;
+#else
+            for (uint32_t i = tid; i < bytes; i += 256) stage[i] = u[c0 + i];
+            __syncthreads();
+#endif
+        }
+        k3_count_chunk<MINQ>(soa, staged ? stage - c0 : u, r0, r1, warp, lane, t0, cnt, minq, sample_sel);
+        __syncthreads();
+        r0 = r1;
+    }
+    k3_flush_tile(cnt, t0, cnt_base, win_len, counts, tid, 256, false);
+}
+
+struct K3Chunk { int64_t c0; uint32_t r0, r1, staged, pad; };
+template <bool MINQ>
+__global__ void __launch_bounds__(K3T_THREADS, 3) k3_tile(RecordSoA soa, const uint8_t* __restrict__ u, int64_t u_end, uint32_t R, uint64_t tiles_base, uint64_t cnt_base, uint64_t win_len, uint64_t fresh_from,
+                                                          const uint32_t* __restrict__ tile_first, const uint32_t* __restrict__ tile_lo, uint32_t* __restrict__ counts, uint32_t minq, int sample_sel) {
+    BD_DYN_SMEM(uint8_t, smem_raw);
+    uint32_t* cnt = reinterpret_cast<uint32_t*>(smem_raw);
+    uint8_t* stages = smem_raw + N_PLANES * TILE_POS * 4;
+    __shared__ K3Bar s_full[K3T_STAGES], s_empty[K3T_STAGES]; __shared__ K3Chunk s_chunk[K3T_STAGES];
+    const uint32_t tile = blockIdx.x, tid = threadIdx.x, lane = tid & 31, warp = tid >> 5;
+    const uint32_t lo = tile_lo[tile];
+    if (lo == 0xFFFFFFFFu) return;
+    const uint32_t hi = tile_first[tile + 1];
+    const uint64_t t0 = tiles_base + (uint64_t)tile * TILE_POS;
+    for (uint32_t i = tid; i < N_PLANES * TILE_POS; i += K3T_THREADS) cnt[i] = 0;
+    if (tid < K3T_STAGES) { k3bar_init(&s_full[tid], 1); k3bar_init(&s_empty[tid], 8); }
+    __syncthreads();
+    if (warp == 8) {
+        uint32_t r0 = lo;
+        for (uint32_t k = 0;; k++) {
+            uint32_t r1 = r0, bytes = 0; int64_t c0 = 0; bool staged = false;
+            if (r0 < hi) {
+                c0 = (int64_t)((reinterpret_cast<uintptr_t>(u) + (uintptr_t)(soa.off[r0] - 4)) & ~uintptr_t(15)) - (int64_t)reinterpret_cast<uintptr_t>(u);
+                uint32_t a = r0 + 1, b = hi;
+                while (a < b) {
+                    const uint32_t m = a + (uint32_t)(((uint64_t)(lane + 1) * (b - a) + 31) / 32);
+                    const int64_t e = m < R ? soa.off[m] - 4 : u_end;
+                    const unsigned fit = __ballot_sync(0xFFFFFFFFu, e - c0 <= (int64_t)K3T_STAGE);
+                    const int j = fit ? 31 - __clz((int)fit) : -1;
+                    const uint32_t m_j = __shfl_sync(0xFFFFFFFFu, m, j < 0 ? 0 : j), m_n = __shfl_sync(0xFFFFFFFFu, m, j < 31 ? j + 1 : 31);
+                    if (j >= 0) a = m_j;
+                    if (j < 31) b = m_n - 1;
+                }
+                r1 = a;
+                const int64_t c1 = r1 < R ? soa.off[r1] - 4 : u_end;
+                staged = c1 - c0 <= (int64_t)K3T_STAGE;
+                bytes = (uint32_t)((c1 - c0 + 15) & ~int64_t(15));
+            }
+            const uint32_t s = k % K3T_STAGES;
+            if (k >= K3T_STAGES) k3bar_wait(&s_empty[s], (k / K3T_STAGES - 1) & 1u);
+            if (lane == 0) {
+                s_chunk[s] = K3Chunk{c0, r0, r1, staged ? 1u : 0u, 0u};
+                if (staged) k3bar_copy(&s_full[s], stages + s * K3T_STAGE, u + c0, bytes);
+                else k3bar_arrive(&s_full[s]);
+            }
+            if (r0 >= hi) break;
+            r0 = r1;
+        }
+    } else {
+        for (uint32_t k = 0;; k++) {
+            const uint32_t s = k % K3T_STAGES;
+            k3bar_wait(&s_full[s], (k / K3T_STAGES) & 1u);
+            const K3Chunk ch = s_chunk[s];
+            if (ch.r0 >= ch.r1) break;
+            k3_count_chunk<MINQ>(soa, ch.staged ? stages + s * K3T_STAGE - ch.c0 : u, ch.r0, ch.r1, warp, lane, t0, cnt, minq, sample_sel);
+            __syncwarp();
+            if (lane == 0) k3bar_arrive(&s_empty[s]);
+        }
+    }
+    __syncthreads();
+    k3_flush_tile(cnt, t0, cnt_base, win_len, counts, tid, K3T_THREADS, t0 >= fresh_from);
 }
 
 template <bool MINQ>
```

Measured after the change: 47.48 (median of 6 runs). 3.6% higher.
